# AleoNet/snarkVM

Measured on AMD Instinct MI355X. Metric: BLS12-377 G1 MSM scalar-point pairs/sec (+ Fr NTT elements/sec in ntt_*), higher is better.
Workload: dtype u32 limbs (29-bit radix) modular integer arithmetic, Fq 377-bit / Fr 253-bit; 1 GPU; G1 Pippenger MSM 2^24 (BASELINE.json configs[1]), bases (i+1)G registered in HBM, uniform scalars in HBM; independent instance per GPU; scalars=uniform, lg_ntt=24, window_bits=auto, base_tables=12, table_bits=22, pipelined_batch=True

## Files before the change

### include/snarkvm_hip.h

```cpp
#ifndef SNARKVM_HIP_H
#define SNARKVM_HIP_H

#include <stddef.h>
#include <stdint.h>

#ifdef __cplusplus
extern "C" {
#endif

typedef struct {
    int32_t code;
    char *message;
} RustError;

enum NTTInputOutputOrder { NN = 0, NR = 1, RN = 2, RR = 3 };
enum NTTDirection { Forward = 0, Inverse = 1 };
enum NTTType { Standard = 0, Coset = 1 };


RustError snarkvm_ntt(void *inout, uint32_t lg_domain_size, enum NTTInputOutputOrder ntt_order,
                      enum NTTDirection ntt_direction, enum NTTType ntt_type);

RustError snarkvm_polymul(void *out, size_t pcount, const void *polynomials, const void *plens, size_t ecount,
                          const void *evaluations, const void *elens, uint32_t lg_domain_size);

RustError snarkvm_msm(void *out, const void *points_with_infinity, size_t npoints, const void *scalars,
                      size_t ffi_affine_sz);
RustError snarkvm_hip_set_base_cache(int tables);
RustError snarkvm_hip_set_base_cache_verified(int tables);
void snarkvm_hip_base_cache_stats(uint64_t *out, int reset);


int snarkvm_hip_device_count(void);
int snarkvm_hip_batch_lanes(size_t npoints);
RustError snarkvm_hip_set_devices(const int32_t *ids, size_t n);
RustError snarkvm_hip_set_device(int device);
int snarkvm_hip_num_devices(void);

RustError snarkvm_hip_malloc(void **d_ptr, size_t bytes, int device);
RustError snarkvm_hip_free(void *d_ptr);
RustError snarkvm_hip_memcpy_h2d(void *d_dst, const void *src, size_t bytes);
RustError snarkvm_hip_memcpy_d2h(void *dst, const void *d_src, size_t bytes);
RustError snarkvm_hip_memcpy_d2d(void *d_dst, const void *d_src, size_t bytes);
RustError snarkvm_hip_memset(void *d_dst, int value, size_t bytes);

RustError snarkvm_hip_ntt_device(void *d_inout, uint32_t lg_domain_size, int ntt_order, int ntt_direction,
                                 int ntt_type);
RustError snarkvm_hip_ntt_device_batch(void *const *d_inouts, size_t count, uint32_t lg_domain_size, int ntt_order,
                                       const int *ntt_directions, const int *ntt_types);

RustError snarkvm_hip_scope_begin(const void *d_any);
RustError snarkvm_hip_scope_end(void);
enum { SNARKVM_HIP_SCOPE_ASYNC_MSM = 1, SNARKVM_HIP_SCOPE_STABLE_INPUTS = 2, SNARKVM_HIP_SCOPE_MSM_IN_STREAM = 4 };
RustError snarkvm_hip_scope_begin_ex(const void *d_any, uint32_t flags);
RustError snarkvm_hip_scope_collect(const void *out);
RustError snarkvm_hip_scope_set_flags(uint32_t flags);
void *snarkvm_hip_scope_stream(void);

typedef struct snarkvm_hip_bases snarkvm_hip_bases_t;
RustError snarkvm_hip_register_bases(snarkvm_hip_bases_t **handle, const void *points, size_t npoints,
                                     size_t ffi_affine_sz, int on_device);
RustError snarkvm_hip_register_bases_tables(snarkvm_hip_bases_t **handle, const void *points, size_t npoints,
                                            size_t ffi_affine_sz, int on_device, int tables);
RustError snarkvm_hip_register_bases_windowed(snarkvm_hip_bases_t **handle, const void *points, size_t npoints,
                                              size_t ffi_affine_sz, int on_device, int tables, int window_bits);
void snarkvm_hip_free_bases(snarkvm_hip_bases_t *handle);

RustError snarkvm_hip_register_bases_serialized(snarkvm_hip_bases_t **handle, const void *bytes, size_t npoints,
                                                int compressed, int validate, int tables);
RustError snarkvm_hip_g1_deserialize(void *out_affine, const void *bytes, size_t n, int compressed, int validate);
RustError snarkvm_hip_g1_serialize(void *out_bytes, const void *affine, size_t n, size_t ffi_affine_sz, int compressed);

RustError snarkvm_hip_g2_deserialize(void *out_affine, const void *bytes, size_t n, int validate);
RustError snarkvm_hip_g2_serialize(void *out_bytes, const void *affine, size_t n, size_t ffi_affine_sz);
RustError snarkvm_hip_g2_deserialize_compressed(void *out_affine, const void *bytes, size_t n, int validate);
RustError snarkvm_hip_g2_serialize_compressed(void *out_bytes, const void *affine, size_t n, size_t ffi_affine_sz);

RustError snarkvm_hip_msm_registered(void *out, const snarkvm_hip_bases_t *handle, size_t offset, size_t npoints,
                                     const void *scalars, int scalars_on_device, int window_bits);

RustError snarkvm_hip_msm_registered_ex(void *out, const snarkvm_hip_bases_t *handle, size_t off0, size_t n0,
                                        size_t off1, size_t n1, const void *scalars, int scalars_on_device,
                                        int scalars_montgomery, int window_bits);

RustError snarkvm_hip_msm_registered_batch(void *outs, const snarkvm_hip_bases_t *handle, size_t count,
                                           const size_t *offsets, const size_t *npoints, const void *const *scalars,
                                           int scalars_on_device, int scalars_montgomery, int window_bits);

RustError snarkvm_hip_msm_registered_batch_ex(void *outs, const snarkvm_hip_bases_t *handle, size_t count, const size_t *off0,
                                              const size_t *n0, const size_t *off1, const size_t *n1,
                                              const void *const *scalars, int scalars_on_device, int scalars_montgomery,
                                              int window_bits);

RustError snarkvm_hip_g1_sum(void *out, const void *in_projective, size_t n);

RustError snarkvm_hip_g1_to_affine(void *out_affine, const void *in_projective, size_t n);

RustError snarkvm_hip_msm_g2(void *out, const void *points_with_infinity, size_t npoints, const void *scalars,
                             size_t ffi_affine_sz);

typedef struct snarkvm_hip_bases_g2 snarkvm_hip_bases_g2_t;
RustError snarkvm_hip_register_bases_g2(snarkvm_hip_bases_g2_t **handle, const void *points, size_t npoints,
                                        size_t ffi_affine_sz, int tables, int window_bits);
void snarkvm_hip_free_bases_g2(snarkvm_hip_bases_g2_t *handle);
RustError snarkvm_hip_msm_g2_registered(void *out, const snarkvm_hip_bases_g2_t *handle, size_t offset, size_t npoints,
                                        const void *scalars, int scalars_on_device, int window_bits);
RustError snarkvm_hip_msm_g2_registered_batch(void *outs, const snarkvm_hip_bases_g2_t *handle, size_t count,
                                              const size_t *offsets, const size_t *npoints, const void *const *scalars,
                                              int scalars_on_device, int window_bits);

RustError snarkvm_hip_g1_fixed_base_msm(void *out_projective, const void *g_affine, const void *scalars, size_t n);
RustError snarkvm_hip_g1_group_ntt(void *inout_projective, uint32_t lg_domain_size, int inverse);

RustError snarkvm_hip_fr_mul_device(void *d_out, const void *d_a, const void *d_b, size_t n);
RustError snarkvm_hip_fr_convert_device(void *d_out, const void *d_in, size_t n, int to_bigint);

RustError snarkvm_hip_fr_vec_op(int op, void *out, const void *a, const void *b, const void *c, const void *scalar,
                                size_t n, int on_device);
RustError snarkvm_hip_fr_divide_by_linear(void *quotient, void *remainder, const void *poly, size_t n,
                                          const void *point, int on_device);
RustError snarkvm_hip_fr_batch_inversion_and_mul(void *inout, size_t n, const void *coeff, int on_device);
RustError snarkvm_hip_fr_distribute_powers(void *inout, size_t n, const void *g, const void *c, int on_device);
RustError snarkvm_hip_fr_lagrange_coefficients(void *out, uint32_t lg_domain_size, const void *tau, int on_device);
RustError snarkvm_hip_fr_divide_by_vanishing(void *quotient, void *remainder, const void *poly, size_t len,
                                             size_t domain_size, int on_device);
RustError snarkvm_hip_fr_mul_by_vanishing(void *out, const void *poly, size_t len, size_t domain_size, int on_device);

RustError snarkvm_hip_fr_vec_op_strided(int op, void *out, const void *a, const void *b, const void *c, const void *scalar,
                                        size_t n, size_t count, size_t stride);
RustError snarkvm_hip_fr_divide_by_linear_strided(void *quotients, void *remainders, const void *polys, size_t n,
                                                  const void *point, size_t count, size_t stride);
RustError snarkvm_hip_fr_divide_by_vanishing_strided(void *quotients, void *remainders, const void *polys, size_t len,
                                                     size_t domain_size, size_t count, size_t stride);

RustError snarkvm_hip_g1_generate_bases_device(void *d_out, uint64_t start, size_t npoints);

void snarkvm_hip_set_profiling(int enabled);
int snarkvm_hip_get_phase_count(void);
const char *snarkvm_hip_get_phase_name(int i);
double snarkvm_hip_get_phase_ms(int i);

void snarkvm_hip_coalescer_stats(uint64_t *out, int reset);

void snarkvm_hip_alloc_stats(uint64_t *out, int reset);

RustError snarkvm_hip_synchronize(void);


int snarkvm_hip_selftest_field(int field, int op, const void *a, const void *b, void *out, size_t n);
int snarkvm_hip_selftest_g1_msm_naive(const void *points_with_infinity, size_t npoints, size_t ffi_affine_sz,
                                      const void *scalars, void *out);
int snarkvm_hip_selftest_msm_plan(size_t n, int window_bits, int tables, int table_bits, uint32_t *out);
int snarkvm_hip_selftest_g1_finish(const void *planes_projective, const int32_t *pos, size_t n, void *out);
int snarkvm_hip_selftest_fq_lazy(uint64_t seed, int iters);
int snarkvm_hip_selftest_g1_lazy_tail(uint64_t seed, int iters);
int snarkvm_hip_selftest_fq2_pair(const void *points, size_t npoints, uint64_t seed, int iters);
int snarkvm_hip_selftest_g2_hex(const void *points, size_t npoints, uint64_t seed, int iters);
RustError snarkvm_hip_devtest_g2_tail_repeat(const void *points, size_t npoints, int m, int hb, int threads, int plane_threads,
                                             int hex, int quads, int iters, uint32_t *report);
int snarkvm_hip_selftest_ntt_plan(uint32_t lg, int32_t *out);
int snarkvm_hip_selftest_ntt_twiddle(int kind, uint32_t lg, int pass, int inverse, const uint64_t *x, size_t n, void *out);
int snarkvm_hip_selftest_ntt_index(uint32_t lg, const int32_t *plan, int npass);
int snarkvm_hip_selftest_ntt_host(void *inout, uint32_t lg, const int32_t *plan, int npass, int dir, int type);
RustError snarkvm_hip_devtest_field(int field, int op, const void *a, const void *b, void *out, size_t n);

#ifdef __cplusplus
}
#endif
#endif
```

### rust/snarkvm-algorithms-hip/src/sys.rs

```rust
#![allow(non_camel_case_types, non_snake_case, clippy::too_many_arguments, clippy::missing_safety_doc)]
use super::{Error, NTTDirection, NTTInputOutputOrder, NTTType};
use core::ffi::{c_char, c_void};

#[repr(C)]
pub struct snarkvm_hip_bases_t {
    _private: [u8; 0],
}
#[repr(C)]
pub struct snarkvm_hip_bases_g2_t {
    _private: [u8; 0],
}

pub const SNARKVM_HIP_SCOPE_ASYNC_MSM: u32 = 1;
pub const SNARKVM_HIP_SCOPE_STABLE_INPUTS: u32 = 2;
pub const SNARKVM_HIP_SCOPE_MSM_IN_STREAM: u32 = 4;

extern "C" {
    pub fn snarkvm_ntt(inout: *mut c_void, lg_domain_size: u32, ntt_order: NTTInputOutputOrder, ntt_direction: NTTDirection, ntt_type: NTTType) -> Error;
    pub fn snarkvm_polymul(out: *mut c_void, pcount: usize, polynomials: *const c_void, plens: *const c_void, ecount: usize, evaluations: *const c_void, elens: *const c_void, lg_domain_size: u32) -> Error;
    pub fn snarkvm_msm(out: *mut c_void, points_with_infinity: *const c_void, npoints: usize, scalars: *const c_void, ffi_affine_sz: usize) -> Error;
    pub fn snarkvm_hip_set_base_cache(tables: i32) -> Error;
    pub fn snarkvm_hip_set_base_cache_verified(tables: i32) -> Error;
    pub fn snarkvm_hip_base_cache_stats(out: *mut u64, reset: i32);
    pub fn snarkvm_hip_device_count() -> i32;
    pub fn snarkvm_hip_batch_lanes(npoints: usize) -> i32;
    pub fn snarkvm_hip_set_devices(ids: *const i32, n: usize) -> Error;
    pub fn snarkvm_hip_set_device(device: i32) -> Error;
    pub fn snarkvm_hip_num_devices() -> i32;
    pub fn snarkvm_hip_malloc(d_ptr: *mut *mut c_void, bytes: usize, device: i32) -> Error;
    pub fn snarkvm_hip_free(d_ptr: *mut c_void) -> Error;
    pub fn snarkvm_hip_memcpy_h2d(d_dst: *mut c_void, src: *const c_void, bytes: usize) -> Error;
    pub fn snarkvm_hip_memcpy_d2h(dst: *mut c_void, d_src: *const c_void, bytes: usize) -> Error;
    pub fn snarkvm_hip_memcpy_d2d(d_dst: *mut c_void, d_src: *const c_void, bytes: usize) -> Error;
    pub fn snarkvm_hip_memset(d_dst: *mut c_void, value: i32, bytes: usize) -> Error;
    pub fn snarkvm_hip_ntt_device(d_inout: *mut c_void, lg_domain_size: u32, ntt_order: i32, ntt_direction: i32, ntt_type: i32) -> Error;
    pub fn snarkvm_hip_ntt_device_batch(d_inouts: *const *mut c_void, count: usize, lg_domain_size: u32, ntt_order: i32, ntt_directions: *const i32, ntt_types: *const i32) -> Error;
    pub fn snarkvm_hip_scope_begin(d_any: *const c_void) -> Error;
    pub fn snarkvm_hip_scope_end() -> Error;
    pub fn snarkvm_hip_scope_begin_ex(d_any: *const c_void, flags: u32) -> Error;
    pub fn snarkvm_hip_scope_collect(out: *const c_void) -> Error;
    pub fn snarkvm_hip_scope_set_flags(flags: u32) -> Error;
    pub fn snarkvm_hip_scope_stream() -> *mut c_void;
    pub fn snarkvm_hip_register_bases(handle: *mut *mut snarkvm_hip_bases_t, points: *const c_void, npoints: usize, ffi_affine_sz: usize, on_device: i32) -> Error;
    pub fn snarkvm_hip_register_bases_tables(handle: *mut *mut snarkvm_hip_bases_t, points: *const c_void, npoints: usize, ffi_affine_sz: usize, on_device: i32, tables: i32) -> Error;
    pub fn snarkvm_hip_register_bases_windowed(handle: *mut *mut snarkvm_hip_bases_t, points: *const c_void, npoints: usize, ffi_affine_sz: usize, on_device: i32, tables: i32, window_bits: i32) -> Error;
    pub fn snarkvm_hip_free_bases(handle: *mut snarkvm_hip_bases_t);
    pub fn snarkvm_hip_register_bases_serialized(handle: *mut *mut snarkvm_hip_bases_t, bytes: *const c_void, npoints: usize, compressed: i32, validate: i32, tables: i32) -> Error;
    pub fn snarkvm_hip_g1_deserialize(out_affine: *mut c_void, bytes: *const c_void, n: usize, compressed: i32, validate: i32) -> Error;
    pub fn snarkvm_hip_g1_serialize(out_bytes: *mut c_void, affine: *const c_void, n: usize, ffi_affine_sz: usize, compressed: i32) -> Error;
    pub fn snarkvm_hip_g2_deserialize(out_affine: *mut c_void, bytes: *const c_void, n: usize, validate: i32) -> Error;
    pub fn snarkvm_hip_g2_serialize(out_bytes: *mut c_void, affine: *const c_void, n: usize, ffi_affine_sz: usize) -> Error;
    pub fn snarkvm_hip_g2_deserialize_compressed(out_affine: *mut c_void, bytes: *const c_void, n: usize, validate: i32) -> Error;
    pub fn snarkvm_hip_g2_serialize_compressed(out_bytes: *mut c_void, affine: *const c_void, n: usize, ffi_affine_sz: usize) -> Error;
    pub fn snarkvm_hip_msm_registered(out: *mut c_void, handle: *const snarkvm_hip_bases_t, offset: usize, npoints: usize, scalars: *const c_void, scalars_on_device: i32, window_bits: i32) -> Error;
    pub fn snarkvm_hip_msm_registered_ex(out: *mut c_void, handle: *const snarkvm_hip_bases_t, off0: usize, n0: usize, off1: usize, n1: usize, scalars: *const c_void, scalars_on_device: i32, scalars_montgomery: i32, window_bits: i32) -> Error;
    pub fn snarkvm_hip_msm_registered_batch(outs: *mut c_void, handle: *const snarkvm_hip_bases_t, count: usize, offsets: *const usize, npoints: *const usize, scalars: *const *const c_void, scalars_on_device: i32, scalars_montgomery: i32, window_bits: i32) -> Error;
    pub fn snarkvm_hip_msm_registered_batch_ex(outs: *mut c_void, handle: *const snarkvm_hip_bases_t, count: usize, off0: *const usize, n0: *const usize, off1: *const usize, n1: *const usize, scalars: *const *const c_void, scalars_on_device: i32, scalars_montgomery: i32, window_bits: i32) -> Error;
    pub fn snarkvm_hip_g1_sum(out: *mut c_void, in_projective: *const c_void, n: usize) -> Error;
    pub fn snarkvm_hip_g1_to_affine(out_affine: *mut c_void, in_projective: *const c_void, n: usize) -> Error;
    pub fn snarkvm_hip_msm_g2(out: *mut c_void, points_with_infinity: *const c_void, npoints: usize, scalars: *const c_void, ffi_affine_sz: usize) -> Error;
    pub fn snarkvm_hip_register_bases_g2(handle: *mut *mut snarkvm_hip_bases_g2_t, points: *const c_void, npoints: usize, ffi_affine_sz: usize, tables: i32, window_bits: i32) -> Error;
    pub fn snarkvm_hip_free_bases_g2(handle: *mut snarkvm_hip_bases_g2_t);
    pub fn snarkvm_hip_msm_g2_registered(out: *mut c_void, handle: *const snarkvm_hip_bases_g2_t, offset: usize, npoints: usize, scalars: *const c_void, scalars_on_device: i32, window_bits: i32) -> Error;
    pub fn snarkvm_hip_msm_g2_registered_batch(outs: *mut c_void, handle: *const snarkvm_hip_bases_g2_t, count: usize, offsets: *const usize, npoints: *const usize, scalars: *const *const c_void, scalars_on_device: i32, window_bits: i32) -> Error;
    pub fn snarkvm_hip_g1_fixed_base_msm(out_projective: *mut c_void, g_affine: *const c_void, scalars: *const c_void, n: usize) -> Error;
    pub fn snarkvm_hip_g1_group_ntt(inout_projective: *mut c_void, lg_domain_size: u32, inverse: i32) -> Error;
    pub fn snarkvm_hip_fr_mul_device(d_out: *mut c_void, d_a: *const c_void, d_b: *const c_void, n: usize) -> Error;
    pub fn snarkvm_hip_fr_convert_device(d_out: *mut c_void, d_in: *const c_void, n: usize, to_bigint: i32) -> Error;
    pub fn snarkvm_hip_fr_vec_op(op: i32, out: *mut c_void, a: *const c_void, b: *const c_void, c: *const c_void, scalar: *const c_void, n: usize, on_device: i32) -> Error;
    pub fn snarkvm_hip_fr_divide_by_linear(quotient: *mut c_void, remainder: *mut c_void, poly: *const c_void, n: usize, point: *const c_void, on_device: i32) -> Error;
    pub fn snarkvm_hip_fr_batch_inversion_and_mul(inout: *mut c_void, n: usize, coeff: *const c_void, on_device: i32) -> Error;
    pub fn snarkvm_hip_fr_distribute_powers(inout: *mut c_void, n: usize, g: *const c_void, c: *const c_void, on_device: i32) -> Error;
    pub fn snarkvm_hip_fr_lagrange_coefficients(out: *mut c_void, lg_domain_size: u32, tau: *const c_void, on_device: i32) -> Error;
    pub fn snarkvm_hip_fr_divide_by_vanishing(quotient: *mut c_void, remainder: *mut c_void, poly: *const c_void, len: usize, domain_size: usize, on_device: i32) -> Error;
    pub fn snarkvm_hip_fr_mul_by_vanishing(out: *mut c_void, poly: *const c_void, len: usize, domain_size: usize, on_device: i32) -> Error;
    pub fn snarkvm_hip_fr_vec_op_strided(op: i32, out: *mut c_void, a: *const c_void, b: *const c_void, c: *const c_void, scalar: *const c_void, n: usize, count: usize, stride: usize) -> Error;
    pub fn snarkvm_hip_fr_divide_by_linear_strided(quotients: *mut c_void, remainders: *mut c_void, polys: *const c_void, n: usize, point: *const c_void, count: usize, stride: usize) -> Error;
    pub fn snarkvm_hip_fr_divide_by_vanishing_strided(quotients: *mut c_void, remainders: *mut c_void, polys: *const c_void, len: usize, domain_size: usize, count: usize, stride: usize) -> Error;
    pub fn snarkvm_hip_g1_generate_bases_device(d_out: *mut c_void, start: u64, npoints: usize) -> Error;
    pub fn snarkvm_hip_set_profiling(enabled: i32);
    pub fn snarkvm_hip_get_phase_count() -> i32;
    pub fn snarkvm_hip_get_phase_name(i: i32) -> *const c_char;
    pub fn snarkvm_hip_get_phase_ms(i: i32) -> f64;
    pub fn snarkvm_hip_coalescer_stats(out: *mut u64, reset: i32);
    pub fn snarkvm_hip_alloc_stats(out: *mut u64, reset: i32);
    pub fn snarkvm_hip_synchronize() -> Error;
    pub fn snarkvm_hip_selftest_field(field: i32, op: i32, a: *const c_void, b: *const c_void, out: *mut c_void, n: usize) -> i32;
    pub fn snarkvm_hip_selftest_g1_msm_naive(points_with_infinity: *const c_void, npoints: usize, ffi_affine_sz: usize, scalars: *const c_void, out: *mut c_void) -> i32;
    pub fn snarkvm_hip_selftest_msm_plan(n: usize, window_bits: i32, tables: i32, table_bits: i32, out: *mut u32) -> i32;
    pub fn snarkvm_hip_selftest_g1_finish(planes_projective: *const c_void, pos: *const i32, n: usize, out: *mut c_void) -> i32;
    pub fn snarkvm_hip_selftest_fq_lazy(seed: u64, iters: i32) -> i32;
    pub fn snarkvm_hip_selftest_g1_lazy_tail(seed: u64, iters: i32) -> i32;
    pub fn snarkvm_hip_selftest_fq2_pair(points: *const c_void, npoints: usize, seed: u64, iters: i32) -> i32;
    pub fn snarkvm_hip_selftest_g2_hex(points: *const c_void, npoints: usize, seed: u64, iters: i32) -> i32;
    pub fn snarkvm_hip_devtest_g2_tail_repeat(points: *const c_void, npoints: usize, m: i32, hb: i32, threads: i32, plane_threads: i32, hex: i32, quads: i32, iters: i32, report: *mut u32) -> Error;
    pub fn snarkvm_hip_selftest_ntt_plan(lg: u32, out: *mut i32) -> i32;
    pub fn snarkvm_hip_selftest_ntt_twiddle(kind: i32, lg: u32, pass: i32, inverse: i32, x: *const u64, n: usize, out: *mut c_void) -> i32;
    pub fn snarkvm_hip_selftest_ntt_index(lg: u32, plan: *const i32, npass: i32) -> i32;
    pub fn snarkvm_hip_selftest_ntt_host(inout: *mut c_void, lg: u32, plan: *const i32, npass: i32, dir: i32, type_: i32) -> i32;
    pub fn snarkvm_hip_devtest_field(field: i32, op: i32, a: *const c_void, b: *const c_void, out: *mut c_void, n: usize) -> Error;
}
```

### snarkvm_amd/_lib.py

```python
import ctypes
import os

_HERE = os.path.dirname(os.path.abspath(__file__))
LIB_PATH = os.environ.get("SNARKVM_HIP_LIB") or os.path.join(_HERE, "lib", "libsnarkvm_hip.so")

SYMBOLS = [
    "snarkvm_ntt", "snarkvm_polymul", "snarkvm_msm", "snarkvm_hip_set_base_cache", "snarkvm_hip_set_base_cache_verified", "snarkvm_hip_base_cache_stats",
    "snarkvm_hip_device_count", "snarkvm_hip_batch_lanes", "snarkvm_hip_set_device", "snarkvm_hip_set_devices", "snarkvm_hip_num_devices",
    "snarkvm_hip_malloc", "snarkvm_hip_free", "snarkvm_hip_memcpy_h2d", "snarkvm_hip_memcpy_d2h", "snarkvm_hip_memcpy_d2d", "snarkvm_hip_memset", "snarkvm_hip_ntt_device", "snarkvm_hip_ntt_device_batch",
    "snarkvm_hip_scope_begin", "snarkvm_hip_scope_end", "snarkvm_hip_scope_begin_ex", "snarkvm_hip_scope_collect", "snarkvm_hip_scope_set_flags", "snarkvm_hip_scope_stream", "snarkvm_hip_alloc_stats",
    "snarkvm_hip_register_bases", "snarkvm_hip_register_bases_tables", "snarkvm_hip_register_bases_windowed", "snarkvm_hip_free_bases", "snarkvm_hip_msm_registered", "snarkvm_hip_msm_g2",
    "snarkvm_hip_msm_registered_ex", "snarkvm_hip_msm_registered_batch", "snarkvm_hip_msm_registered_batch_ex", "snarkvm_hip_g1_to_affine",
    "snarkvm_hip_fr_mul_device", "snarkvm_hip_fr_convert_device", "snarkvm_hip_g1_generate_bases_device",
    "snarkvm_hip_fr_vec_op", "snarkvm_hip_fr_divide_by_linear", "snarkvm_hip_fr_batch_inversion_and_mul",
    "snarkvm_hip_fr_distribute_powers", "snarkvm_hip_fr_lagrange_coefficients", "snarkvm_hip_fr_divide_by_vanishing",
    "snarkvm_hip_fr_mul_by_vanishing",
    "snarkvm_hip_fr_vec_op_strided", "snarkvm_hip_fr_divide_by_linear_strided", "snarkvm_hip_fr_divide_by_vanishing_strided",
    "snarkvm_hip_register_bases_serialized", "snarkvm_hip_g1_deserialize", "snarkvm_hip_g1_serialize", "snarkvm_hip_g1_sum", "snarkvm_hip_g2_deserialize", "snarkvm_hip_g2_serialize", "snarkvm_hip_g2_deserialize_compressed", "snarkvm_hip_g2_serialize_compressed",
    "snarkvm_hip_register_bases_g2", "snarkvm_hip_free_bases_g2", "snarkvm_hip_msm_g2_registered", "snarkvm_hip_msm_g2_registered_batch",
    "snarkvm_hip_g1_fixed_base_msm", "snarkvm_hip_g1_group_ntt",
    "snarkvm_hip_set_profiling", "snarkvm_hip_get_phase_count", "snarkvm_hip_get_phase_name",
    "snarkvm_hip_get_phase_ms", "snarkvm_hip_synchronize", "snarkvm_hip_coalescer_stats",
    "snarkvm_hip_selftest_field", "snarkvm_hip_selftest_g1_msm_naive", "snarkvm_hip_selftest_msm_plan", "snarkvm_hip_selftest_g1_finish", "snarkvm_hip_selftest_fq_lazy", "snarkvm_hip_selftest_g1_lazy_tail", "snarkvm_hip_selftest_ntt_plan", "snarkvm_hip_selftest_ntt_twiddle", "snarkvm_hip_selftest_ntt_index", "snarkvm_hip_selftest_ntt_host", "snarkvm_hip_selftest_fq2_pair", "snarkvm_hip_selftest_g2_hex", "snarkvm_hip_devtest_field", "snarkvm_hip_devtest_g2_tail_repeat",
]


class RustError(ctypes.Structure):
    _fields_ = [("code", ctypes.c_int32), ("message", ctypes.c_void_p)]


class HipError(RuntimeError):
    def __init__(self, code, message):
        super().__init__(f"snarkvm_hip error {code}: {message}")
        self.code = code
        self.message = message


_lib = None
_libc = None


def lib():
    global _lib, _libc
    if _lib is None:
        if not os.path.exists(LIB_PATH):
            raise ImportError(
                f"{LIB_PATH} is missing - build it with `python -m snarkvm_amd.build` (hipcc, gfx950). "
                "snarkvm_amd has no CPU fallback.")
        if not os.environ.get("SNARKVM_HIP_NO_TORCH"):
            try:
                import torch
            except ImportError:
                pass
        L = ctypes.CDLL(LIB_PATH)
        err_fns = ["snarkvm_ntt", "snarkvm_polymul", "snarkvm_msm", "snarkvm_hip_set_base_cache", "snarkvm_hip_set_base_cache_verified", "snarkvm_hip_set_device", "snarkvm_hip_set_devices",
                   "snarkvm_hip_malloc", "snarkvm_hip_free", "snarkvm_hip_memcpy_h2d", "snarkvm_hip_memcpy_d2h", "snarkvm_hip_memcpy_d2d", "snarkvm_hip_memset", "snarkvm_hip_ntt_device", "snarkvm_hip_ntt_device_batch",
                   "snarkvm_hip_scope_begin", "snarkvm_hip_scope_end", "snarkvm_hip_scope_begin_ex", "snarkvm_hip_scope_collect", "snarkvm_hip_scope_set_flags",
                   "snarkvm_hip_register_bases", "snarkvm_hip_register_bases_tables", "snarkvm_hip_register_bases_windowed", "snarkvm_hip_msm_registered", "snarkvm_hip_msm_g2", "snarkvm_hip_msm_registered_ex", "snarkvm_hip_msm_registered_batch", "snarkvm_hip_msm_registered_batch_ex", "snarkvm_hip_g1_to_affine", "snarkvm_hip_fr_mul_device",
                   "snarkvm_hip_fr_convert_device", "snarkvm_hip_g1_generate_bases_device", "snarkvm_hip_synchronize",
                   "snarkvm_hip_fr_vec_op", "snarkvm_hip_fr_divide_by_linear", "snarkvm_hip_fr_batch_inversion_and_mul", "snarkvm_hip_fr_distribute_powers", "snarkvm_hip_fr_lagrange_coefficients", "snarkvm_hip_fr_divide_by_vanishing", "snarkvm_hip_fr_mul_by_vanishing",
                   "snarkvm_hip_fr_vec_op_strided", "snarkvm_hip_fr_divide_by_linear_strided", "snarkvm_hip_fr_divide_by_vanishing_strided",
                   "snarkvm_hip_register_bases_serialized", "snarkvm_hip_g1_deserialize", "snarkvm_hip_g1_serialize", "snarkvm_hip_g1_sum", "snarkvm_hip_g2_deserialize", "snarkvm_hip_g2_serialize", "snarkvm_hip_g2_deserialize_compressed", "snarkvm_hip_g2_serialize_compressed",
                   "snarkvm_hip_register_bases_g2", "snarkvm_hip_msm_g2_registered", "snarkvm_hip_msm_g2_registered_batch",
                   "snarkvm_hip_g1_fixed_base_msm", "snarkvm_hip_g1_group_ntt",
                   "snarkvm_hip_devtest_field", "snarkvm_hip_devtest_g2_tail_repeat"]
        for name in err_fns:
            getattr(L, name).restype = RustError
        L.snarkvm_hip_device_count.restype = ctypes.c_int
        L.snarkvm_hip_batch_lanes.restype = ctypes.c_int
        L.snarkvm_hip_num_devices.restype = ctypes.c_int
        L.snarkvm_hip_selftest_g1_finish.restype = ctypes.c_int
        L.snarkvm_hip_selftest_fq_lazy.restype = ctypes.c_int
        L.snarkvm_hip_selftest_g1_lazy_tail.restype = ctypes.c_int
        for name in ("snarkvm_hip_selftest_ntt_plan", "snarkvm_hip_selftest_ntt_twiddle", "snarkvm_hip_selftest_ntt_index", "snarkvm_hip_selftest_ntt_host"):
            getattr(L, name).restype = ctypes.c_int
        L.snarkvm_hip_selftest_fq2_pair.restype = ctypes.c_int
        L.snarkvm_hip_selftest_g2_hex.restype = ctypes.c_int
        L.snarkvm_hip_get_phase_count.restype = ctypes.c_int
        L.snarkvm_hip_get_phase_name.restype = ctypes.c_char_p
        L.snarkvm_hip_get_phase_ms.restype = ctypes.c_double
        L.snarkvm_hip_selftest_field.restype = ctypes.c_int
        L.snarkvm_hip_selftest_g1_msm_naive.restype = ctypes.c_int
        L.snarkvm_hip_selftest_msm_plan.restype = ctypes.c_int
        L.snarkvm_hip_free_bases.restype = None
        L.snarkvm_hip_free_bases_g2.restype = None
        L.snarkvm_hip_set_profiling.restype = None
        L.snarkvm_hip_coalescer_stats.restype = None
        L.snarkvm_hip_base_cache_stats.restype = None
        L.snarkvm_hip_alloc_stats.restype = None
        L.snarkvm_hip_scope_stream.restype = ctypes.c_void_p
        L.snarkvm_hip_scope_begin_ex.argtypes = [ctypes.c_void_p, ctypes.c_uint32]
        L.snarkvm_hip_scope_set_flags.argtypes = [ctypes.c_uint32]
        L.snarkvm_hip_alloc_stats.argtypes = [ctypes.c_void_p, ctypes.c_int]
        L.snarkvm_hip_coalescer_stats.argtypes = [ctypes.c_void_p, ctypes.c_int]
        L.snarkvm_hip_base_cache_stats.argtypes = [ctypes.c_void_p, ctypes.c_int]
        L.snarkvm_hip_malloc.argtypes = [ctypes.POINTER(ctypes.c_void_p), ctypes.c_size_t, ctypes.c_int]
        L.snarkvm_hip_free.argtypes = [ctypes.c_void_p]
        L.snarkvm_hip_memcpy_h2d.argtypes = [ctypes.c_void_p, ctypes.c_void_p, ctypes.c_size_t]
        L.snarkvm_hip_memcpy_d2h.argtypes = [ctypes.c_void_p, ctypes.c_void_p, ctypes.c_size_t]
        L.snarkvm_hip_memcpy_d2d.argtypes = [ctypes.c_void_p, ctypes.c_void_p, ctypes.c_size_t]
        L.snarkvm_hip_memset.argtypes = [ctypes.c_void_p, ctypes.c_int, ctypes.c_size_t]
        _libc = ctypes.CDLL(None)
        _libc.free.argtypes = [ctypes.c_void_p]
        _lib = L
    return _lib


def check(err):
    if err.code != 0:
        msg = ctypes.string_at(err.message).decode(errors="replace") if err.message else ""
        if err.message:
            _libc.free(err.message)
        raise HipError(err.code, msg)


def device_count():
    return lib().snarkvm_hip_device_count()
```

### snarkvm_amd/csrc/api.hip

```cpp
#define SV_TU_G1
#include "runtime.hip.h"
#include "ffl.hip.h"

runtime_t g_rt;
thread_local thread_scope_t g_tl_scope;
thread_scope_t::~thread_scope_t() {
    if (!lane) return;
    pending.clear();
    (void)hipStreamSynchronize(lane->stream);
    for (int i = 0; i < naux; i++) {
        (void)hipStreamSynchronize(aux[i]->stream);
        aux[i]->dev->give(aux[i], true);
    }
    lane->in_scope = false;
    lane->deferred.clear();
    lane->deferred_bytes = 0;
    if (!lane->tw_leases.empty()) ntt_tw_release(lane->dev, lane->tw_leases);
    lane->dev->give(lane, true);
    lane = nullptr;
}
std::atomic<uint64_t> g_co_stats[4];
static std::atomic<uint64_t> g_alloc_stats[5];
void sv_alloc_note(int slot, size_t bytes, double ms) {
    g_alloc_stats[slot].fetch_add(1, std::memory_order_relaxed);
// ... 131 lines not shown
    if (!bytes) return ok();
    API_BEGIN_DEV(device_for(d_src, 1))
    if (!dst || !d_src) throw hip_failure{hipErrorInvalidValue, "snarkvm_hip_memcpy_d2h: null pointer", __LINE__};
    HIP_TRY(hipMemcpyAsync(dst, d_src, bytes, hipMemcpyDeviceToHost, c.stream));
    HIP_TRY(hipStreamSynchronize(c.stream));
    API_END
}
RustError snarkvm_hip_memcpy_d2d(void* d_dst, const void* d_src, size_t bytes) {
    if (!bytes) return ok();
    API_BEGIN_DEV(device_for(d_dst, 1))
    if (!d_dst || !d_src) throw hip_failure{hipErrorInvalidValue, "snarkvm_hip_memcpy_d2d: null pointer", __LINE__};
    const uint8_t *a = (const uint8_t*)d_dst, *b = (const uint8_t*)d_src;
    if (a < b + bytes && b < a + bytes) throw hip_failure{hipErrorInvalidValue, "snarkvm_hip_memcpy_d2d: the ranges overlap", __LINE__};
    if (g_rt.device_of(d_src) < 0) throw hip_failure{hipErrorInvalidValue, "snarkvm_hip_memcpy_d2d: source is not on a device in use", __LINE__};
    HIP_TRY(hipMemcpyAsync(d_dst, d_src, bytes, hipMemcpyDefault, c.stream));
    c.sync_or_defer();
    API_END
}
RustError snarkvm_hip_memset(void* d_dst, int value, size_t bytes) {
    if (!bytes) return ok();
    API_BEGIN_DEV(device_for(d_dst, 1))
    HIP_TRY(hipMemsetAsync(d_dst, value, bytes, c.stream));
    c.sync_or_defer();
    API_END
}

static constexpr uint32_t SCOPE_FLAGS_ALL = SNARKVM_HIP_SCOPE_ASYNC_MSM | SNARKVM_HIP_SCOPE_STABLE_INPUTS | SNARKVM_HIP_SCOPE_MSM_IN_STREAM;
RustError snarkvm_hip_scope_begin_ex(const void* d_any, uint32_t flags) {
    API_TRY
    thread_scope_t& sc = tl_scope();
    if (sc.lane) throw hip_failure{hipErrorInvalidValue, "scope_begin: the calling thread already has an open scope", __LINE__};
    if (flags & ~SCOPE_FLAGS_ALL) throw hip_failure{hipErrorInvalidValue, "scope_begin: unknown flag", __LINE__};
    g_rt.configure();
    const int nd = (int)g_rt.devs.size();
    int dev = device_for(d_any, d_any ? 1 : 0);
    if (dev < 0) dev = (int)(g_rt.rr.fetch_add(1) % (uint32_t)nd);
    device_t* d = g_rt.devs[dev].get();
    int prev = -1;
    if (hipGetDevice(&prev) != hipSuccess) prev = 0;
    lane_t* l = d->take_for_scope(true);
    try {
        HIP_TRY(hipSetDevice(d->physical));
        d->init();
        tu_kernel_attributes(d->logical);
    } catch (...) {
        d->give(l, true);
        (void)hipSetDevice(prev);
        throw;
    }
    l->begin_call();
    l->in_scope = true;
    l->pin_used = 0;
    l->scope_events_used = 0;
    sc = thread_scope_t();
    sc.lane = l;
    sc.prev_device = prev;
    sc.flags = flags;
    API_CATCH
}
RustError snarkvm_hip_scope_begin(const void* d_any) { return snarkvm_hip_scope_begin_ex(d_any, 0); }
void* snarkvm_hip_scope_stream(void) {
    lane_t* l = tl_scope().lane;
    return l ? (void*)l->stream : nullptr;
}
RustError snarkvm_hip_scope_set_flags(uint32_t flags) {
    API_TRY
    thread_scope_t& sc = tl_scope();
    if (!sc.lane) throw hip_failure{hipErrorInvalidValue, "scope_set_flags: the calling thread has no open scope", __LINE__};
    if (flags & ~SCOPE_FLAGS_ALL) throw hip_failure{hipErrorInvalidValue, "scope_set_flags: unknown flag", __LINE__};
    sc.flags = flags;
    API_CATCH
}
RustError snarkvm_hip_scope_collect(const void* out) {
    API_TRY
    scope_collect(out);
    API_CATCH
}
RustError snarkvm_hip_scope_end(void) {
    thread_scope_t& sc = tl_scope();
    lane_t* l = sc.lane;
    if (!l) return ok();
    RustError r = ok();
    try {
        scope_flush();
    } catch (const hip_failure& f) {
        r = from_failure(f);
    } catch (const std::exception& e) {
        r = fail(1, std::string("snarkvm_hip: scope_end: ") + e.what());
    } catch (...) {
        r = fail(1, "snarkvm_hip: scope_end failed");
    }
    l->in_scope = false;
    l->deferred.clear();
    l->deferred_bytes = 0;
    for (int i = 0; i < sc.naux; i++) {
        (void)hipStreamSynchronize(sc.aux[i]->stream);
        sc.aux[i]->dev->give(sc.aux[i], true);
    }
    const int prev = sc.prev_device;
    sc = thread_scope_t();
    l->dev->give(l, true);
    if (prev >= 0) (void)hipSetDevice(prev);
    return r;
}

static void precompute_tables(lane_t& c, snarkvm_hip_bases* h, g1_aff_mem_t* d) { precompute_tables_run<fq_t>(c, d, h->n, h->tables, h->table_bits); }
static void register_bases_impl(snarkvm_hip_bases_t** handle, const void* points, size_t npoints, size_t ffi_affine_sz, int on_device, int tables,
                                int table_bits) {
    if (!handle) throw hip_failure{hipErrorInvalidValue, "register_bases: null handle", __LINE__};
    if (npoints && !points) throw hip_failure{hipErrorInvalidValue, "register_bases: null points", __LINE__};
    if (ffi_affine_sz < 104 || (ffi_affine_sz & 7)) throw hip_failure{hipErrorInvalidValue, "register_bases: bad stride", __LINE__};
    check_tables(tables, table_bits, "register_bases");
    scope_flush();
    const int nd = g_rt.ndev();
    std::unique_ptr<snarkvm_hip_bases> h(new snarkvm_hip_bases());
    h->n = npoints;
    h->tables = tables;
    h->table_bits = table_bits ? table_bits : 256 / tables;
    h->d.assign(nd, nullptr);
    const size_t bytes = (size_t)tables * npoints * sizeof(g1_aff_mem_t);
    try {
        if (npoints) {
            const int owner = on_device ? device_for(points, 1) : -1;
            auto build = [&](int dev) {
                lane_guard lg(dev);
                lane_t& c = lg.c();
                HIP_TRY(hipMalloc((void**)&h->d[dev], bytes));
                const uint8_t* src = (const uint8_t*)points;
                if (!on_device) {
                    c.bases_tmp.ensure(npoints * ffi_affine_sz);
                    HIP_TRY(hipMemcpyAsync(c.bases_tmp.p, points, npoints * ffi_affine_sz, hipMemcpyHostToDevice, c.stream));
                    src = c.bases_tmp.as<uint8_t>();
                }
                convert_bases<fq_t>(c, src, ffi_affine_sz, npoints, h->d[dev]);
                precompute_tables(c, h.get(), h->d[dev]);
                bases_to_lazy_form(c, h->d[dev], (size_t)tables * npoints);
                HIP_TRY(hipStreamSynchronize(c.stream));
            };
            std::vector<int> all;
            for (int d = 0; d < nd; d++) all.push_back(d);
            if (!on_device) {
                for_each_device(all, build);
            } else {
                build(owner);
                for (int d = 0; d < nd; d++) {
                    if (d == owner) continue;
                    lane_guard lg(d);
                    HIP_TRY(hipMalloc((void**)&h->d[d], bytes));
                    HIP_TRY(hipMemcpyPeerAsync(h->d[d], g_rt.devs[d]->physical, h->d[owner], g_rt.devs[owner]->physical, bytes, lg.c().stream));
                    HIP_TRY(hipStreamSynchronize(lg.c().stream));
                }
            }
        }
    } catch (...) {
        h->free_all();
        throw;
    }
    *handle = h.release();
}
RustError snarkvm_hip_register_bases(snarkvm_hip_bases_t** handle, const void* points, size_t npoints, size_t ffi_affine_sz, int on_device) {
    API_TRY
    register_bases_impl(handle, points, npoints, ffi_affine_sz, on_device, 1, 0);
    API_CATCH
}
RustError snarkvm_hip_register_bases_tables(snarkvm_hip_bases_t** handle, const void* points, size_t npoints, size_t ffi_affine_sz, int on_device,
                                            int tables) {
    API_TRY
    register_bases_impl(handle, points, npoints, ffi_affine_sz, on_device, tables, 0);
    API_CATCH
}
RustError snarkvm_hip_register_bases_windowed(snarkvm_hip_bases_t** handle, const void* points, size_t npoints, size_t ffi_affine_sz, int on_device,
                                              int tables, int window_bits) {
    API_TRY
    if (window_bits <= 0) throw hip_failure{hipErrorInvalidValue, "register_bases_windowed: window_bits must be positive", __LINE__};
    register_bases_impl(handle, points, npoints, ffi_affine_sz, on_device, tables, window_bits);
    API_CATCH
}
void snarkvm_hip_free_bases(snarkvm_hip_bases_t* h) {
    if (!h) return;
    h->free_all();
    delete h;
}
}
snarkvm_hip_bases* sv_new_bases_handle(size_t npoints, int tables, int table_bits) {
    snarkvm_hip_bases* h = new snarkvm_hip_bases();
    h->n = npoints;
    h->tables = tables;
    h->table_bits = table_bits;
    h->d.assign(g_rt.ndev(), nullptr);
    return h;
}
void sv_precompute_tables(lane_t& c, snarkvm_hip_bases* h, g1_aff_mem_t* d) { precompute_tables(c, h, d); }
extern "C" {

static void check_window_bits(int window_bits, const char* who) {
    if (window_bits && (window_bits < 2 || window_bits > MSM_C_MAX)) throw std::runtime_error(std::string(who) + ": window_bits must be 0 or 2..23");
}
static void msm_registered_host_scalars(void* out, const snarkvm_hip_bases* h, size_t off0, size_t n0, size_t off1, size_t n1, const void* scalars,
                                        int scalars_montgomery, int window_bits) {
    const size_t n = n0 + n1;
    scope_flush();
    const int nd = g_rt.ndev();
    static const int trace = getenv("SNARKVM_HIP_TRACE") ? atoi(getenv("SNARKVM_HIP_TRACE")) : 0;
    const double t_begin = host_now_ms();
    size_t parts = n / MSM_SPLIT_MIN;
    if (parts > (size_t)nd) parts = (size_t)nd;
    if (parts < 1) parts = 1;
    const size_t chunk = msm_scalar_chunk_pairs();
    if (n >= 2 * chunk && (n + chunk - 1) / chunk > parts) parts = (n + chunk - 1) / chunk;
    std::vector<size_t> bound;
    const int geo = tuning().scalar_geo;
    if (nd == 1 && geo > 1 && tuning().taper != 0 && n >= ((size_t)1 << 22)) {
        parts = n >= ((size_t)1 << 23) ? 3 : 2;
        size_t wsum = 0, w = 1;
        for (size_t i = 0; i < parts; i++, w *= (size_t)geo) wsum += w;
        size_t acc_w = 0;
        w = 1;
        bound.push_back(0);
        for (size_t i = 0; i < parts; i++, w *= (size_t)geo) {
            acc_w += w;
            bound.push_back(i + 1 == parts ? n : (size_t)((unsigned __int128)n * acc_w / wsum));
        }
    } else {
        for (size_t i = 0; i <= parts; i++) bound.push_back(n * i / parts);
    }
    const int ndu = (int)(parts < (size_t)nd ? parts : (size_t)nd);
    std::unique_ptr<msm_accum_t<fq_t>> acc(new msm_accum_t<fq_t>());
    std::mutex acc_mu;
    std::vector<int> devs;
    if (ndu == 1) {
        devs.push_back(-1);
    } else {
        for (int d = 0; d < ndu; d++) devs.push_back(d);
    }
    const size_t slot = msm_plane_bytes<fq_t>();
    for_each_device(devs, [&](int dev) {
        std::vector<size_t> mine;
        for (size_t i = (dev < 0 ? 0 : (size_t)dev); i < parts; i += (size_t)ndu) mine.push_back(i);
        lane_guard lg;
        lg.acquire(dev, mine.size() > 2 ? 3 : (int)mine.size());
        const size_t L = lg.lanes.size();
        size_t max_cnt = 0;
        for (size_t j = 0; j < mine.size(); j++) {
            const size_t cnt = bound[mine[j] + 1] - bound[mine[j]];
            max_cnt = cnt > max_cnt ? cnt : max_cnt;
        }
        const bool use_sink = tuning().taper != 0 && mine.size() >= 2;
        std::vector<msm_pending_t> pend(use_sink ? 1 : mine.size());
        int chunk_c = window_bits;
        msm_bucket_sink_t sink;
        std::vector<hipEvent_t> merged;
        for (size_t l = 0; l < L; l++) {
            lane_t& c = *lg.lanes[l];
            c.begin_call();
            c.scalars_tmp.ensure(max_cnt * 32 + 32);
            c.pin.ensure(slot * (use_sink ? 1 : (mine.size() + L - 1) / L));
        }
        if (use_sink) {
            lane_t& c0 = *lg.lanes[0];
            const msm_plan_t pl = msm_make_plan(max_cnt, window_bits, h->tables, h->table_bits);
            chunk_c = pl.c;
            sink.nbt = (uint32_t)pl.W * pl.nb;
            sink.L = 1;
            const size_t bytes = (size_t)sink.nbt * msm_partial_bytes<fq_t>();
            c0.sink_acc.ensure(bytes);
            sink.acc = c0.sink_acc.p;
            HIP_TRY(hipMemsetAsync(sink.acc, 0, bytes, c0.stream));
            hipEvent_t ready = c0.new_event();
            HIP_TRY(hipEventRecord(ready, c0.stream));
            for (size_t l = 1; l < L; l++) HIP_TRY(hipStreamWaitEvent(lg.lanes[l]->stream, ready, 0));
            for (size_t j = 0; j < mine.size(); j++) merged.push_back(lg.lanes[j % L]->new_event());
        }
        const g1_aff_mem_t* base = h->d[lg.lanes[0]->dev->logical];
        auto upload = [&](size_t j, hipStream_t st) {
            lane_t& c = *lg.lanes[j % L];
            const size_t lo = bound[mine[j]], hi = bound[mine[j] + 1];
            if (hi > lo) HIP_TRY(hipMemcpyAsync(c.scalars_tmp.p, (const uint8_t*)scalars + lo * 32, (hi - lo) * 32, hipMemcpyHostToDevice, st));
        };
        auto compute = [&](size_t j, bool prof) {
            lane_t& c = *lg.lanes[j % L];
            const size_t lo = bound[mine[j]], hi = bound[mine[j] + 1];
            const size_t a0 = lo < n0 ? lo : n0, a1 = hi < n0 ? hi : n0;
            const size_t m0 = a1 - a0;
            const g1_aff_mem_t* b0 = base + off0 + a0;
            const g1_aff_mem_t* b1 = base + off1 + (lo > n0 ? lo - n0 : 0);
            msm_bucket_sink_t mine_sink = sink;
            if (use_sink) {
                mine_sink.after = j ? merged[j - 1] : nullptr;
                mine_sink.done = merged[j];
            }
            const msm_pending_t pd = msm_run<fq_t>(c, m0 ? b0 : b1, c.scalars_tmp.as<uint4>(), hi - lo, c.pin.as<uint8_t>() + (use_sink ? 0 : slot * (j / L)), chunk_c,
                                                   b1, m0 ? m0 : ~(size_t)0, scalars_montgomery, h->tables, h->n, prof, h->table_bits, nullptr,
                                                   use_sink ? &mine_sink : nullptr);
            if (!use_sink) pend[j] = pd;
        };
        if (mine.size() == 1) {
            lane_t& c = *lg.lanes[0];
            c.phase_begin("msm_h2d");
            upload(0, c.stream);
            c.phase_end();
            compute(0, parts == 1);
        } else {
            lane_ring_run(lg, mine.size(), upload, [&](size_t j) { compute(j, false); }, trace, t_begin);
        }
        if (use_sink) {
            lane_t& c0 = *lg.lanes[0];
// ... 556 lines not shown
            g1_xyzz_t t2 = total;
            t2.add(acc);
            t2.add(neg);
            t2.add(acc);
            total = t2;
        } else {
            total.add(acc);
        }
    }
    const g1_jac_t j = total.to_jacobian();
    uint32_t* o = (uint32_t*)out;
    j.x.to_mem_mont().pack(o);
    j.y.to_mem_mont().pack(o + 12);
    j.z.to_mem_mont().pack(o + 24);
    return 0;
}
int snarkvm_hip_selftest_fq_lazy(uint64_t seed, int iters) {
    uint32_t xw[12], yw[12];
    memcpy(xw, G1_GEN_X, 48);
    memcpy(yw, G1_GEN_Y, 48);
    const g1_aff_t g{fq_t::unpack(xw).from_mem_mont(), fq_t::unpack(yw).from_mem_mont()};
    std::vector<g1_aff_t> pool;
    g1_xyzz_t run = g1_xyzz_t::inf();
    for (int k = 0; k < 64; k++) {
        run.add_affine(g);
        const fq_t izzz = run.zzz.inverse();
        const fq_t izz = izzz.sqr() * run.zz.sqr();
        pool.push_back({run.x * izz, run.y * izzz});
    }
    const fq_t c406 = fq_t::from_table(FqLConv::C406), c348 = fq_t::from_table(FqLConv::C348);
    auto next = [&]() {
        seed += 0x9E3779B97F4A7C15ull;
        uint64_t z = seed;
        z = (z ^ (z >> 30)) * 0xBF58476D1CE4E5B9ull;
        z = (z ^ (z >> 27)) * 0x94D049BB133111EBull;
        return z ^ (z >> 31);
    };
    g1_xyzz_t exact = g1_xyzz_t::inf();
    xyzz_lazy_t lazy = xyzz_lazy_t::infinity();
    int prev = -1;
    bool prev_neg = false;
    for (int it = 0; it < iters; it++) {
        const uint64_t r = next();
        int k = (int)(r % 64);
        bool neg = ((r >> 8) & 1) != 0;
        const int mode = (int)((r >> 16) % 16);
        if (mode == 0 && prev >= 0) k = prev, neg = prev_neg;
        if (mode == 1 && prev >= 0) k = prev, neg = !prev_neg;
        if (mode == 2) {
            exact = g1_xyzz_t::inf();
            lazy = xyzz_lazy_t::infinity();
        }
        prev = k;
        prev_neg = neg;
        const g1_aff_t p = pool[k];
        exact.add_affine(p, neg);
        const fql_t px = fql_t::from_limbs(p.x * c406), py = fql_t::from_limbs(p.y * c406);
        if (!lazy.madd(px, py, neg)) {
            g1_xyzz_t e = lazy.to_exact();
            fq_t ex, ey;
            for (int i = 0; i < 13; i++) ex.v[i] = (uint32_t)px.v[i], ey.v[i] = (uint32_t)py.v[i];
            e.add_affine({ex * c348, ey * c348}, neg);
            lazy = xyzz_lazy_t::from_exact(e);
        }
        const g1_xyzz_t got = lazy.to_exact();
        if (got.is_inf() != exact.is_inf()) return it + 1;
        if (!exact.is_inf() && (got.x != exact.x || got.y != exact.y || got.zz != exact.zz || got.zzz != exact.zzz)) return it + 1;
    }
    for (int t = 0; t < 200; t++) {
        fq_t a, b;
        for (int i = 0; i < 13; i++) a.v[i] = (uint32_t)(next() & LIMB_MASK), b.v[i] = (uint32_t)(next() & LIMB_MASK);
        a.v[12] &= 0x00ffffffu;
        b.v[12] &= 0x00ffffffu;
        if (t & 1) for (int i = 0; i < 12; i++) a.v[i] = LIMB_MASK;
        if (t & 2) for (int i = 0; i < 12; i++) b.v[i] = (i & 1) ? LIMB_MASK : 0;
        const fql_t la = fql_t::from_exact(a), lb = fql_t::from_exact(b);
        if (fql_t::mul(la, lb).to_exact() != a * b) return -(4 * t + 1);
        if (fql_t::sqr(la - lb).to_exact() != (a - b).sqr()) return -(4 * t + 2);
        if (fql_t::diff_of_products(la - lb, lb - la, fql_t::from_exact(a * b).normalized(), la).to_exact() != fq_t::diff_of_products(a - b, b - a, a * b, a))
            return -(4 * t + 3);
        if (((la + lb) - (lb + lb)).normalized().to_exact() != (a - b)) return -(4 * t + 4);
        alignas(16) uint32_t raw[12];
        const fql_t wide = (la - lb - lb - lb).normalized();
        wide.store_raw(raw);
        const fql_t back = fql_t::load_raw(raw);
        for (int i = 0; i < 13; i++)
            if (back.v[i] != wide.v[i]) return -(100000 + t);
    }
    return 0;
}
int snarkvm_hip_selftest_g1_lazy_tail(uint64_t seed, int iters) {
    uint32_t xw[12], yw[12];
    memcpy(xw, G1_GEN_X, 48);
    memcpy(yw, G1_GEN_Y, 48);
    const g1_aff_t g{fq_t::unpack(xw).from_mem_mont(), fq_t::unpack(yw).from_mem_mont()};
    std::vector<g1_xyzz_t> pool;
    g1_xyzz_t run = g1_xyzz_t::inf();
    for (int k = 0; k < 48; k++) {
        run.add_affine(g);
        pool.push_back(run);
    }
    auto next = [&]() {
        seed += 0x9E3779B97F4A7C15ull;
        uint64_t z = seed;
        z = (z ^ (z >> 30)) * 0xBF58476D1CE4E5B9ull;
        z = (z ^ (z >> 27)) * 0x94D049BB133111EBull;
        return z ^ (z >> 31);
    };
    auto to_lazy = [](const g1_xyzz_t& p) {
        xyzz_t<fqz_t> r = xyzz_t<fqz_t>::inf();
        if (!p.is_inf()) r = {{fql_t::from_exact(p.x)}, {fql_t::from_exact(p.y)}, {fql_t::from_exact(p.zz)}, {fql_t::from_exact(p.zzz)}};
        return r;
    };
    g1_xyzz_t exact = g1_xyzz_t::inf();
    xyzz_t<fqz_t> lazy = xyzz_t<fqz_t>::inf();
    g1_xyzz_t prev = g1_xyzz_t::inf();
    for (int it = 0; it < iters; it++) {
        const uint64_t r = next();
        g1_xyzz_t p = pool[r % 48];
        fq_t l = fq_t::zero();
        for (int i = 0; i < 12; i++) l.v[i] = (uint32_t)(next() & LIMB_MASK);
        l.v[0] |= 1;
        const fq_t l2 = l.sqr(), l3 = l2 * l;
        p = {p.x * l2, p.y * l3, p.zz * l2, p.zzz * l3};
        if ((r >> 8) & 1) p.y = p.y.neg();
        const int mode = (int)((r >> 16) % 16);
        if (mode == 0) p = prev;
        if (mode == 1) p = {prev.x, prev.y.neg(), prev.zz, prev.zzz};
        if (mode == 2) {
            exact = g1_xyzz_t::inf();
            lazy = xyzz_t<fqz_t>::inf();
        }
        if (mode == 3) p = exact;
        if (mode == 4) {
            exact = exact.dbl();
            lazy = lazy.dbl();
        } else {
            prev = p;
            exact.add(p);
            lazy.add(to_lazy(p));
        }
        if (lazy.is_inf() != exact.is_inf()) return it + 1;
        if (!exact.is_inf() && (lazy.x.to_exact() != exact.x || lazy.y.to_exact() != exact.y || lazy.zz.to_exact() != exact.zz || lazy.zzz.to_exact() != exact.zzz))
            return it + 1;
        xyzz_mem_t<fqz_t> m;
        store_xyzz<fqz_t>(&m, lazy);
        lazy = load_xyzz<fqz_t>(&m);
    }
    fqz_t zq;
    for (int i = 0; i < 13; i++) zq.a.v[i] = FqL::MOD[i];
    if (!zq.is_zero() || !zq.neg().is_zero() || !(zq + zq).is_zero() || (zq + fqz_t::one()).is_zero()) return -1;
    return 0;
}
int snarkvm_hip_selftest_g1_finish(const void* planes_jacobian, const int32_t* pos, size_t n, void* out) {
    try {
        std::unique_ptr<msm_accum_t<fq_t>> acc(new msm_accum_t<fq_t>());
        const uint32_t* src = (const uint32_t*)planes_jacobian;
        for (size_t i = 0; i < n; i++) {
            const g1_jac_t j = {fq_t::from_raw_words(src + 36 * i), fq_t::from_raw_words(src + 36 * i + 12), fq_t::from_raw_words(src + 36 * i + 24)};
            acc->add(pos[i], g1_xyzz_t::from_jacobian(j));
        }
        acc->finish(out);
        return 0;
    } catch (...) {
        return 1;
    }
}

}
```

### snarkvm_amd/csrc/api_serde.hip

```cpp
#include "runtime.hip.h"

snarkvm_hip_bases* sv_new_bases_handle(size_t npoints, int tables, int table_bits);
void sv_precompute_tables(lane_t& c, snarkvm_hip_bases* h, g1_aff_mem_t* d);

static uint32_t g1_deserialize_run(lane_t& c, const void* bytes, size_t n, int compressed, int validate, g1_aff_mem_t* d_native, uint8_t* d_rust) {
    const size_t psz = compressed ? 48 : 96;
    c.bases_tmp.ensure(n * psz);
    c.serde_status.ensure(4);
    HIP_TRY(hipMemcpyAsync(c.bases_tmp.p, bytes, n * psz, hipMemcpyHostToDevice, c.stream));
    HIP_TRY(hipMemsetAsync(c.serde_status.p, 0, 4, c.stream));
    hipLaunchKernelGGL(g1_deserialize_kernel, dim3((unsigned)((n + 63) / 64)), dim3(64), 0, c.stream, c.bases_tmp.as<uint8_t>(), n, compressed, validate,
                       d_native, d_rust, c.serde_status.as<uint32_t>());
    HIP_TRY(hipGetLastError());
    uint32_t st = 0;
    HIP_TRY(hipMemcpyAsync(&st, c.serde_status.p, 4, hipMemcpyDeviceToHost, c.stream));
    HIP_TRY(hipStreamSynchronize(c.stream));
    return st;
}

extern "C" {

RustError snarkvm_hip_register_bases_serialized(snarkvm_hip_bases_t** handle, const void* bytes, size_t npoints, int compressed, int validate,
                                                int tables) {
    API_TRY
    if (!handle || (npoints && !bytes)) throw hip_failure{hipErrorInvalidValue, "register_bases_serialized: null argument", __LINE__};
    check_tables(tables, 0, "register_bases_serialized");
    std::unique_ptr<snarkvm_hip_bases> h(sv_new_bases_handle(npoints, tables, 256 / tables));
    if (npoints) {
        try {
            std::vector<int> all;
            for (int d = 0; d < g_rt.ndev(); d++) all.push_back(d);
            for_each_device(all, [&](int dev) {
                lane_guard lg(dev);
                lane_t& c = lg.c();
                HIP_TRY(hipMalloc((void**)&h->d[dev], (size_t)tables * npoints * sizeof(g1_aff_mem_t)));
                serde_throw_on_status(g1_deserialize_run(c, bytes, npoints, compressed, validate, h->d[dev], nullptr), "register_bases_serialized");
                sv_precompute_tables(c, h.get(), h->d[dev]);
                bases_to_lazy_form(c, h->d[dev], (size_t)tables * npoints);
                HIP_TRY(hipStreamSynchronize(c.stream));
            });
        } catch (...) {
            h->free_all();
            throw;
        }
    }
    *handle = h.release();
    API_CATCH
}
RustError snarkvm_hip_g1_deserialize(void* out_affine, const void* bytes, size_t n, int compressed, int validate) {
    API_BEGIN
    if (n) {
        if (!out_affine || !bytes) throw hip_failure{hipErrorInvalidValue, "g1_deserialize: null argument", __LINE__};
        c.poly[0].ensure(n * 104);
        const uint32_t st = g1_deserialize_run(c, bytes, n, compressed, validate, nullptr, c.poly[0].as<uint8_t>());
        serde_throw_on_status(st, "g1_deserialize");
        HIP_TRY(hipMemcpyAsync(out_affine, c.poly[0].p, n * 104, hipMemcpyDeviceToHost, c.stream));
        HIP_TRY(hipStreamSynchronize(c.stream));
    }
    API_END
}
RustError snarkvm_hip_g1_serialize(void* out_bytes, const void* affine, size_t n, size_t ffi_affine_sz, int compressed) {
    API_BEGIN
    if (n) {
        if (!out_bytes || !affine) throw hip_failure{hipErrorInvalidValue, "g1_serialize: null argument", __LINE__};
        if (ffi_affine_sz < 104 || (ffi_affine_sz & 7)) throw hip_failure{hipErrorInvalidValue, "g1_serialize: bad stride", __LINE__};
        const size_t psz = compressed ? 48 : 96;
        c.bases_tmp.ensure(n * ffi_affine_sz);
        c.poly[0].ensure(n * psz);
        HIP_TRY(hipMemcpyAsync(c.bases_tmp.p, affine, n * ffi_affine_sz, hipMemcpyHostToDevice, c.stream));
        hipLaunchKernelGGL(g1_serialize_kernel, dim3((unsigned)((n + 63) / 64)), dim3(64), 0, c.stream, c.bases_tmp.as<uint8_t>(), ffi_affine_sz, n,
                           compressed, c.poly[0].as<uint8_t>());
        HIP_TRY(hipGetLastError());
        HIP_TRY(hipMemcpyAsync(out_bytes, c.poly[0].p, n * psz, hipMemcpyDeviceToHost, c.stream));
        HIP_TRY(hipStreamSynchronize(c.stream));
    }
    API_END
}

}
```

### snarkvm_amd/csrc/ffl.hip.h

```cpp
#pragma once
#include "ec.hip.h"

namespace sv {

struct FqL {
    static constexpr int N = 13;
    static constexpr int STEPS = 14;
    static constexpr int32_t MOD[13] = {0x00000001, 0x08460000, 0x00000021, 0x16ba8860, 0x14800170, 0x1117dd04, 0x0e3c7bcd,
                                        0x1e601ea2, 0x1b1a22d9, 0x03650a49, 0x118ec170, 0x0f8a21d5, 0x1ae3a461};
    static constexpr int32_t K377[13] = {0x1fffffff, 0x17b9ffff, 0x1fffffde, 0x0945779f, 0x0b7ffe8f, 0x0ee822fb, 0x11c38432,
                                         0x019fe15d, 0x04e5dd26, 0x1c9af5b6, 0x0e713e8f, 0x1075de2a, 0x051c5b9e};
    static constexpr int32_t K435[13] = {0x0677f3e3, 0x01fcf72f, 0x05fc93a0, 0x08eb59fe, 0x0c1a6c3f, 0x122b8005, 0x01c7de9b,
                                         0x0b159718, 0x189a8339, 0x07649107, 0x02e4fa41, 0x13571fee, 0x04eba458};
};
struct FqLConv {
    static constexpr uint32_t C406[13] = {0x19eaf730u, 0x171ffffeu, 0x0d714cf8u, 0x044e31d8u, 0x1eb6e262u, 0x0bfad163u, 0x00d46e9cu,
                                          0x10b6ddbfu, 0x13b9cbddu, 0x075782afu, 0x03bd1d8au, 0x1557cab6u, 0x15742a14u};
    static constexpr uint32_t C399[13] = {0x1fb3d5efu, 0x1759ffffu, 0x161ae2aeu, 0x06bd319fu, 0x15cd6eabu, 0x15c6dfc5u, 0x00a7763du,
                                          0x1e5d80e1u, 0x10d7c95fu, 0x04add573u, 0x1c80b321u, 0x02e104bau, 0x10f92f11u};
    static constexpr uint32_t C348[13] = {0, 0, 0, 0, 0, 0, 0, 0, 0, 0, 0, 0, 1};
};

#if defined(__HIP_DEVICE_COMPILE__)
#define SV_OPAQUE_LIMB(x) asm("" : "+v"(x))
// ... 183 lines not shown
        return r;
    }

    SV_HD fq_t to_exact() const {
        fql_t k;
#pragma unroll
        for (int i = 0; i < N; i++) k.v[i] = FqL::K377[i];
        fql_t t = mul(*this, k);
#pragma unroll 1
        for (int round = 0; round < 3 && t.v[N - 1] < 0; round++) {
            int32_t c = 0;
#pragma unroll
            for (int i = 0; i < N - 1; i++) {
                const int32_t x = t.v[i] + FqL::MOD[i] + c;
                t.v[i] = (int32_t)((uint32_t)x & MASK);
                c = x >> 29;
            }
            t.v[N - 1] += FqL::MOD[N - 1] + c;
        }
        uint32_t w[N];
#pragma unroll
        for (int i = 0; i < N; i++) w[i] = (uint32_t)t.v[i];
        return fq_t::cond_sub(w);
    }
    SV_HD static fql_t from_exact(const fq_t& a) {
        fql_t k;
#pragma unroll
        for (int i = 0; i < N; i++) k.v[i] = FqL::K435[i];
        return mul(from_limbs(a), k);
    }
};

struct alignas(128) g1_lazy_slot_t {
    uint32_t w[32];
    SV_HD void coords(fql_t& px, fql_t& py) const {
#pragma unroll
        for (int i = 0; i < 13; i++) px.v[i] = (int32_t)w[i], py.v[i] = (int32_t)w[13 + i];
        SV_OPAQUE_13(px.v);
        SV_OPAQUE_13(py.v);
    }
    SV_HD static void store(g1_aff_mem_t* slot, const fq_t& x406, const fq_t& y406, bool inf) {
        uint32_t* o = (uint32_t*)slot;
        uint4* q = (uint4*)slot;
        uint32_t t[28];
#pragma unroll
        for (int i = 0; i < 13; i++) t[i] = inf ? 0u : x406.v[i], t[13 + i] = inf ? 0u : y406.v[i];
        t[26] = inf ? 1u : 0u;
        t[27] = 0;
#pragma unroll
        for (int i = 0; i < 7; i++) q[i] = make_uint4(t[4 * i], t[4 * i + 1], t[4 * i + 2], t[4 * i + 3]);
        (void)o;
    }
};
static_assert(sizeof(g1_lazy_slot_t) == sizeof(g1_aff_mem_t), "a lazy base slot overlays the exact one");

struct alignas(16) g1_lazy_partial_t {
    int32_t w[52];
};
struct xyzz_lazy_t {
    fql_t x, y, zz, zzz;
    bool inf;

    SV_HD static xyzz_lazy_t infinity() {
        xyzz_lazy_t r;
        r.x = r.y = r.zz = r.zzz = fql_t::zero();
        r.inf = true;
        return r;
    }
    SV_HD g1_xyzz_t to_exact() const {
        if (inf) return g1_xyzz_t::inf();
        return {x.to_exact(), y.to_exact(), zz.to_exact(), zzz.to_exact()};
    }
    SV_HD void store_raw(g1_lazy_partial_t* p) const {
        uint4* q = (uint4*)p;
        if (inf) {
#pragma unroll
            for (int i = 0; i < 13; i++) q[i] = make_uint4(0, 0, 0, 0);
            return;
        }
        int32_t t[52];
#pragma unroll
        for (int i = 0; i < 13; i++) t[i] = x.v[i], t[13 + i] = y.v[i], t[26 + i] = zz.v[i], t[39 + i] = zzz.v[i];
#pragma unroll
        for (int i = 0; i < 13; i++) q[i] = make_uint4((uint32_t)t[4 * i], (uint32_t)t[4 * i + 1], (uint32_t)t[4 * i + 2], (uint32_t)t[4 * i + 3]);
    }
    SV_HD static g1_xyzz_t exact_from_raw(const g1_lazy_partial_t* p) {
        const uint4* q = (const uint4*)p;
        int32_t t[52];
#pragma unroll
        for (int i = 0; i < 13; i++) {
            const uint4 u = q[i];
            t[4 * i] = (int32_t)u.x, t[4 * i + 1] = (int32_t)u.y, t[4 * i + 2] = (int32_t)u.z, t[4 * i + 3] = (int32_t)u.w;
        }
        fql_t c[4];
#pragma unroll
        for (int k = 0; k < 4; k++)
#pragma unroll
            for (int i = 0; i < 13; i++) c[k].v[i] = t[13 * k + i];
        return {c[0].to_exact(), c[1].to_exact(), c[2].to_exact(), c[3].to_exact()};
    }
    SV_HD static xyzz_lazy_t from_exact(const g1_xyzz_t& p) {
        xyzz_lazy_t r;
        r.inf = p.is_inf();
        if (r.inf) return infinity();
        r.x = fql_t::from_exact(p.x);
        r.y = fql_t::from_exact(p.y);
        r.zz = fql_t::from_exact(p.zz);
        r.zzz = fql_t::from_exact(p.zzz);
        return r;
    }
    SV_HD bool madd(const fql_t& px, const fql_t& py, bool negate) {
        if (inf) {
            x = px;
            y = py.negate_if(negate).normalized();
            zz = zzz = one();
            inf = false;
            return true;
        }
        const fql_t u2 = fql_t::mul(px, zz);
        const fql_t s2 = fql_t::mul(py.negate_if(negate), zzz);
        const fql_t p = u2 - x;
        const fql_t r = s2 - y;
        if ((((uint32_t)p.v[0] + 4u) & fql_t::MASK) <= 5u) return false;
        const fql_t pp = fql_t::sqr(p);
        const fql_t ppp = fql_t::mul(p, pp);
        const fql_t q = fql_t::mul(x, pp);
        const fql_t rr = fql_t::sqr(r);
        fql_t x3;
        {
            int32_t c = 0;
#pragma unroll
            for (int i = 0; i < fql_t::N - 1; i++) {
                const int32_t t = rr.v[i] - ppp.v[i] - 2 * q.v[i] + c;
                x3.v[i] = (int32_t)((uint32_t)t & fql_t::MASK);
                c = t >> 29;
            }
            x3.v[fql_t::N - 1] = rr.v[fql_t::N - 1] - ppp.v[fql_t::N - 1] - 2 * q.v[fql_t::N - 1] + c;
            SV_OPAQUE_13(x3.v);
        }
        y = fql_t::diff_of_products(r, q - x3, y, ppp);
        x = x3;
        zz = fql_t::mul(zz, pp);
        zzz = fql_t::mul(zzz, ppp);
        return true;
    }
    SV_HD static fql_t one() {
        fql_t r;
#pragma unroll
        for (int i = 0; i < fql_t::N; i++) r.v[i] = (int32_t)FqLConv::C406[i];
        return r;
    }
};

struct fqz_t {
    fql_t a;
    struct mem_t {
        uint32_t w[13];
    };
    static constexpr int N = 13;

    SV_HD static fqz_t zero() { return {fql_t::zero()}; }
    SV_HD static fqz_t one() { return {xyzz_lazy_t::one()}; }
    SV_HD static fqz_t load(const mem_t* p) {
        fqz_t r;
#pragma unroll
        for (int i = 0; i < N; i++) r.a.v[i] = (int32_t)p->w[i];
        return r;
    }
    SV_HD void store(mem_t* p) const {
#pragma unroll
        for (int i = 0; i < N; i++) p->w[i] = (uint32_t)a.v[i];
    }
    SV_HD fqz_t operator*(const fqz_t& b) const { return {fql_t::mul(a, b.a)}; }
    SV_HD fqz_t sqr() const { return {fql_t::sqr(a)}; }
    SV_HD fqz_t operator+(const fqz_t& b) const { return {(a + b.a).normalized()}; }
    SV_HD fqz_t operator-(const fqz_t& b) const { return {(a - b.a).normalized()}; }
    SV_HD fqz_t dbl() const { return {(a + a).normalized()}; }
    SV_HD fqz_t neg() const { return {(fql_t::zero() - a).normalized()}; }
    SV_HD static fqz_t diff_of_products(const fqz_t& x, const fqz_t& y, const fqz_t& z, const fqz_t& w) {
        return {fql_t::diff_of_products(x.a, y.a, z.a, w.a)};
    }
    SV_HD fq_t to_exact() const { return a.to_exact(); }
    SV_HD bool is_zero() const {
        int32_t any = 0;
#pragma unroll
        for (int i = 0; i < N; i++) any |= a.v[i];
        if (any == 0) return true;
        if ((((uint32_t)a.v[0] + 8u) & fql_t::MASK) > 16u) return false;
        return a.to_exact().is_zero();
    }
};

}
```

### snarkvm_amd/csrc/msm.hip.h

```cpp
#pragma once
#include <stdlib.h>

#include <type_traits>

#include "ec.hip.h"
#include "ffl.hip.h"
#include "ffl2.hip.h"
#include "hex2.hip.h"
#include "tuning.hip.h"

namespace sv {

struct msm_plan_t {
    size_t n;
    int c;
    int W;
    int J;
    int Wd;
    uint32_t nb;
    uint32_t nbt;
    uint32_t chunk;
    uint32_t nchunks;
    uint32_t S, S2;
    uint32_t L;
// ... 72 lines not shown
    if (p.L > p.nb) p.L = p.nb;
    while (p.nb % p.L) p.L--;
    p.rounds = 0;
    size_t m = ((size_t)p.J * n + p.S - 1) / p.S;
    while (m > 1) {
        m = (m + p.S2 - 1) / p.S2;
        p.rounds++;
    }
    for (int i = 0; i < 10; i++) p.bias[i] = 0;
    for (int w = 0; w < p.Wd; w++) {
        int bit = p.c - 1 + p.c * w;
        if (bit >= MSM_BIAS_BITS) break;
        p.bias[bit / 32] |= 1u << (bit % 32);
    }
    return p;
}

static constexpr int SCAN_TILE = 2048;
static __global__ void scan_tile_kernel(const uint32_t* in, uint32_t* out, uint32_t* block_sums, size_t n) {
    __shared__ uint32_t sh[256];
    const size_t base = (size_t)blockIdx.x * SCAN_TILE + (size_t)threadIdx.x * 8;
    uint32_t v[8], s = 0;
#pragma unroll
    for (int i = 0; i < 8; i++) {
        v[i] = (base + i < n) ? in[base + i] : 0u;
        s += v[i];
    }
    sh[threadIdx.x] = s;
    __syncthreads();
    for (int off = 1; off < 256; off <<= 1) {
        uint32_t t = (threadIdx.x >= (unsigned)off) ? sh[threadIdx.x - off] : 0u;
        __syncthreads();
        sh[threadIdx.x] += t;
        __syncthreads();
    }
    uint32_t run = sh[threadIdx.x] - s;
#pragma unroll
    for (int i = 0; i < 8; i++) {
        if (base + i < n) out[base + i] = run;
        run += v[i];
    }
    if (threadIdx.x == 255 && block_sums) block_sums[blockIdx.x] = sh[255];
}
static __global__ void scan_add_kernel(uint32_t* out, const uint32_t* block_offsets, size_t n) {
    const size_t base = (size_t)blockIdx.x * SCAN_TILE + (size_t)threadIdx.x * 8;
    const uint32_t add = block_offsets[blockIdx.x];
#pragma unroll
    for (int i = 0; i < 8; i++)
        if (base + i < n) out[base + i] += add;
}
static inline size_t scan_tmp_elems(size_t n) {
    size_t tot = 0;
    while (n > 1) {
        n = (n + SCAN_TILE - 1) / SCAN_TILE;
        tot += n + 1;
        if (n == 1) break;
    }
    return tot + 8;
}
static constexpr uint32_t SCAN_ONE_THREADS = 1024, SCAN_ONE_MAX = 33 * SCAN_ONE_THREADS;
static __global__ void __launch_bounds__(1024) scan_one_block_kernel(const uint32_t* in, uint32_t* out, uint32_t n, uint32_t per) {
    extern __shared__ uint32_t scan_sm[];
    __shared__ uint32_t wave_tot[16];
    const uint32_t t = threadIdx.x;
    for (uint32_t i = t; i < n; i += SCAN_ONE_THREADS) scan_sm[i] = in[i];
    __syncthreads();
    const uint32_t lo = t * per, hi = lo + per < n ? lo + per : n;
    uint32_t sum = 0;
    for (uint32_t i = lo; i < hi; i++) sum += scan_sm[i];
    uint32_t incl = sum;
    for (int off = 1; off < 64; off <<= 1) {
        const uint32_t u = (uint32_t)__shfl_up((int)incl, off);
        if ((t & 63) >= (uint32_t)off) incl += u;
    }
    if ((t & 63) == 63) wave_tot[t >> 6] = incl;
    __syncthreads();
    uint32_t base = 0;
    for (uint32_t w = 0; w < (t >> 6); w++) base += wave_tot[w];
    uint32_t run = base + incl - sum;
    for (uint32_t i = lo; i < hi; i++) {
        const uint32_t v = scan_sm[i];
        scan_sm[i] = run;
        run += v;
    }
    __syncthreads();
    for (uint32_t i = t; i < n; i += SCAN_ONE_THREADS) out[i] = scan_sm[i];
}
static inline void exclusive_scan_u32(hipStream_t st, const uint32_t* in, uint32_t* out, size_t n, uint32_t* tmp) {
    if (n == 0) return;
    const int one_launch = tuning().scan1;
    if (one_launch && n > (size_t)SCAN_TILE && n <= (size_t)SCAN_ONE_MAX) {
        const uint32_t per = (uint32_t)((n + SCAN_ONE_THREADS - 1) / SCAN_ONE_THREADS) | 1u;
        hipLaunchKernelGGL(scan_one_block_kernel, dim3(1), dim3(SCAN_ONE_THREADS), (size_t)n * 4, st, in, out, (uint32_t)n, per);
        return;
    }
    const size_t blocks = (n + SCAN_TILE - 1) / SCAN_TILE;
    hipLaunchKernelGGL(scan_tile_kernel, dim3((unsigned)blocks), dim3(256), 0, st, in, out, tmp, n);
    if (blocks > 1) {
        exclusive_scan_u32(st, tmp, tmp, blocks, tmp + blocks + 1);
        hipLaunchKernelGGL(scan_add_kernel, dim3((unsigned)blocks), dim3(256), 0, st, out, tmp, n);
    }
}

template <class F>
SV_HD void store_base_slot(aff_mem_t<F>* slot, const uint32_t* xw, const uint32_t* yw, bool inf, int form406) {
    aff_t<F> a = aff_t<F>::inf();
    if (!inf) {
        a.x = F::from_raw_words(xw);
        a.y = F::from_raw_words(yw);
    }
    store_aff<F>(slot, a);
}
template <>
SV_HD void store_base_slot<fq_t>(aff_mem_t<fq_t>* slot, const uint32_t* xw, const uint32_t* yw, bool inf, int form406) {
    if (form406) {
        const fq_t c = fq_t::from_table(FqLConv::C399);
        g1_lazy_slot_t::store(slot, fq_t::unpack(xw) * c, fq_t::unpack(yw) * c, inf);
        return;
    }
    g1_aff_t a = g1_aff_t::inf();
    if (!inf) {
        a.x = fq_t::from_raw_words(xw);
        a.y = fq_t::from_raw_words(yw);
    }
    store_aff<fq_t>(slot, a);
}
template <>
SV_HD void store_base_slot<fq2_t>(aff_mem_t<fq2_t>* slot, const uint32_t* xw, const uint32_t* yw, bool inf, int form406) {
    if (form406) {
        const fq_t c = fq_t::from_table(FqLConv::C399);
        g2_lazy_slot_t::store(slot, {fq_t::unpack(xw) * c, fq_t::unpack(xw + 12) * c}, {fq_t::unpack(yw) * c, fq_t::unpack(yw + 12) * c}, inf);
        return;
    }
    aff_t<fq2_t> a = aff_t<fq2_t>::inf();
    if (!inf) {
        a.x = fq2_t::from_raw_words(xw);
        a.y = fq2_t::from_raw_words(yw);
    }
    store_aff<fq2_t>(slot, a);
}
static __global__ void g2_bases_to_form406_kernel(aff_mem_t<fq2_t>* slots, size_t n) {
    const size_t i = blockIdx.x * (size_t)blockDim.x + threadIdx.x;
    if (i >= n) return;
    const fq_t c = fq_t::from_table(FqLConv::C406);
    const aff_t<fq2_t> a = load_aff<fq2_t>(&slots[i]);
    g2_lazy_slot_t::store(&slots[i], {a.x.c0 * c, a.x.c1 * c}, {a.y.c0 * c, a.y.c1 * c}, a.is_inf());
}
static __global__ void g1_bases_to_form406_kernel(g1_aff_mem_t* slots, size_t n) {
    const size_t i = blockIdx.x * (size_t)blockDim.x + threadIdx.x;
    if (i >= n) return;
    const fq_t c = fq_t::from_table(FqLConv::C406);
    const g1_aff_t a = g1_load_aff(&slots[i]);
    g1_lazy_slot_t::store(&slots[i], a.x * c, a.y * c, a.is_inf());
}
template <class F>
__global__ void convert_bases_kernel(const uint8_t* in, size_t stride, size_t n, aff_mem_t<F>* out, int form406) {
    size_t i = blockIdx.x * (size_t)blockDim.x + threadIdx.x;
    if (i >= n) return;
    const uint32_t* src = (const uint32_t*)(in + i * stride);
    constexpr int MW = F::MEM_WORDS;
    uint32_t xw[MW], yw[MW];
#pragma unroll
    for (int k = 0; k < MW; k++) {
        xw[k] = src[k];
        yw[k] = src[MW + k];
    }
    const uint32_t inf = src[2 * MW] & 0xffu;
    store_base_slot<F>(&out[i], xw, yw, inf != 0, form406);
}

struct msm_digit_params_t {
    uint32_t bias[10];
    int c, W;
    size_t n;
    int montgomery;
};
template <class DT>
__global__ void __launch_bounds__(256) msm_digits_kernel(const uint4* __restrict__ scalars, DT* __restrict__ digits,
                                                         msm_digit_params_t p) {
    __shared__ uint4 stage[512];
    const size_t nblk = (p.n + 255) / 256;
    for (size_t blk = blockIdx.x; blk < nblk; blk += gridDim.x) {
        const size_t first = blk * 256;
        const size_t cnt = (p.n - first < 256) ? (p.n - first) : 256;
        for (int k = threadIdx.x; k < 512; k += 256)
            if ((size_t)(k >> 1) < cnt) stage[k] = scalars[first * 2 + k];
        __syncthreads();
        if (threadIdx.x < cnt) {
            const uint4 lo = stage[2 * threadIdx.x], hi = stage[2 * threadIdx.x + 1];
            uint32_t s[11] = {lo.x, lo.y, lo.z, lo.w, hi.x, hi.y, hi.z, hi.w, 0u, 0u, 0u};
            if (p.montgomery) {
                fr_t c32 = fr_t::zero();
                c32.v[0] = 32;
                (fr_t::unpack(s) * c32).pack(s);
            }
            uint64_t carry = 0;
#pragma unroll
            for (int k = 0; k < 10; k++) {
                carry += (uint64_t)s[k] + p.bias[k];
                s[k] = (uint32_t)carry;
                carry >>= 32;
            }
            const uint32_t mask = (1u << p.c) - 1;
            const size_t i = first + threadIdx.x;
            for (int w = 0; w < p.W; w++) {
                const int bit = p.c * w, wi = bit >> 5, sh = bit & 31;
                uint64_t two = (uint64_t)s[wi] | ((uint64_t)s[wi + 1] << 32);
                digits[(size_t)w * p.n + i] = (DT)((uint32_t)(two >> sh) & mask);
            }
        }
        __syncthreads();
    }
}

static __global__ void msm_alloc_kernel(const uint32_t* cnt_in, uint32_t* cnt_out, uint32_t nbt, uint32_t S) {
    uint32_t k = blockIdx.x * blockDim.x + threadIdx.x;
    if (k > nbt) return;
    cnt_out[k] = (k == nbt) ? 0u : (cnt_in[k] + S - 1) / S;
}
__device__ __forceinline__ uint32_t find_bucket(const uint32_t* start, uint32_t nbt, uint32_t t) {
    uint32_t lo = 0, hi = nbt;
    while (hi - lo > 1) {
        const uint32_t mid = (lo + hi) >> 1;
        if (start[mid] <= t)
            lo = mid;
        else
            hi = mid;
    }
    return lo;
}
template <class F>
__global__ void __launch_bounds__(256) msm_reduce_kernel(const xyzz_mem_t<F>* __restrict__ in,
                                                         const uint32_t* __restrict__ in_start,
                                                         const uint32_t* __restrict__ in_cnt,
                                                         const uint32_t* __restrict__ out_start,
                                                         xyzz_mem_t<F>* __restrict__ out, uint32_t nbt, uint32_t S2) {
    const uint32_t t = blockIdx.x * blockDim.x + threadIdx.x;
    if (t >= out_start[nbt]) return;
    const uint32_t k = find_bucket(out_start, nbt, t);
    const uint32_t j = t - out_start[k];
    const uint32_t lo = in_start[k] + j * S2;
    uint32_t hi = lo + S2;
    const uint32_t end = in_start[k] + in_cnt[k];
    if (hi > end) hi = end;
    xyzz_t<F> acc = load_xyzz<F>(&in[lo]);
    for (uint32_t pos = lo + 1; pos < hi; pos++) acc.add(load_xyzz<F>(&in[pos]));
    store_xyzz<F>(&out[t], acc);
}

template <class F>
__global__ void __launch_bounds__(256) msm_bucket_merge_kernel(const xyzz_mem_t<F>* __restrict__ part, const uint32_t* __restrict__ start,
                                                               const uint32_t* __restrict__ cnt, xyzz_mem_t<F>* __restrict__ acc, uint32_t nbt, uint32_t L,
                                                               uint32_t slot) {
    const uint32_t k = blockIdx.x * blockDim.x + threadIdx.x;
    if (k >= nbt) return;
    const uint32_t c = cnt[k];
    if (!c) return;
    const uint32_t lo = start[k];
    xyzz_mem_t<F>* dst = &acc[(size_t)k * L + slot];
    xyzz_t<F> a = load_xyzz<F>(dst);
    for (uint32_t i = 0; i < c; i++) a.add(load_xyzz<F>(&part[lo + i]));
    store_xyzz<F>(dst, a);
}
static __global__ void msm_sink_lists_kernel(uint32_t* __restrict__ start, uint32_t* __restrict__ cnt, uint32_t nbt, uint32_t L) {
    const uint32_t k = blockIdx.x * blockDim.x + threadIdx.x;
    if (k > nbt) return;
    start[k] = k * L;
    cnt[k] = k < nbt ? L : 0u;
}

__device__ __forceinline__ fq_t shfl_xor_field(const fq_t& a, int mask) {
    fq_t r;
#pragma unroll
    for (int i = 0; i < fq_t::N; i++) r.v[i] = (uint32_t)__shfl_xor((int)a.v[i], mask);
    return r;
}
__device__ __forceinline__ fq2_t shfl_xor_field(const fq2_t& a, int mask) { return {shfl_xor_field(a.c0, mask), shfl_xor_field(a.c1, mask)}; }
__device__ __forceinline__ fqz_t shfl_xor_field(const fqz_t& a, int mask) {
    fqz_t r;
#pragma unroll
    for (int i = 0; i < fqz_t::N; i++) r.a.v[i] = __shfl_xor(a.a.v[i], mask);
    SV_OPAQUE_13(r.a.v);
    return r;
}
template <class F>
__device__ __forceinline__ xyzz_t<F> shfl_xor_point(const xyzz_t<F>& a, int mask) {
    return {shfl_xor_field(a.x, mask), shfl_xor_field(a.y, mask), shfl_xor_field(a.zz, mask), shfl_xor_field(a.zzz, mask)};
}
template <int CTRL>
__device__ __forceinline__ fq_t quad_perm_field(const fq_t& a) {
    fq_t r;
#pragma unroll
    for (int i = 0; i < fq_t::N; i++) r.v[i] = (uint32_t)__builtin_amdgcn_mov_dpp((int)a.v[i], CTRL, 0xf, 0xf, true);
    return r;
}
template <int CTRL>
__device__ __forceinline__ fq2_t quad_perm_field(const fq2_t& a) {
    return {quad_perm_field<CTRL>(a.c0), quad_perm_field<CTRL>(a.c1)};
}
template <int CTRL>
__device__ __forceinline__ fqz_t quad_perm_field(const fqz_t& a) {
    fqz_t r;
#pragma unroll
    for (int i = 0; i < fqz_t::N; i++) r.a.v[i] = __builtin_amdgcn_mov_dpp(a.a.v[i], CTRL, 0xf, 0xf, true);
    SV_OPAQUE_13(r.a.v);
    return r;
// ... 510 lines not shown
```

### snarkvm_amd/csrc/msm_sort.hip.h

```cpp
#pragma once
#include "ffl.hip.h"
#include "ffl2.hip.h"
#include "ffl2p.hip.h"
#include "msm.hip.h"

namespace sv {

static constexpr int SORT_TILE = 8192;
static constexpr int SORT_THREADS = 256;

struct msm_inst_t {
    const uint4* scalars;
    uint32_t n;
    uint32_t n0;
    uint32_t off0, off1;
    uint32_t pstart;
    uint32_t ptiles;
};
struct msm_radix_params_t {
    size_t n;
    int c, W, J;
    int HB, LB;
    uint32_t nb;
    uint32_t tiles_per_row;
// ... 569 lines not shown
        }
        if (sl == 0) {
            bsize[(size_t)q * B2 + key] = total;
            if (total) atomicMax(&blk_max, total);
        }
    }
    if (q == 0 && threadIdx.x == 0) bsize[(size_t)nbins * B2] = 0;
    __syncthreads();
    if (threadIdx.x == 0 && blk_max > __atomic_load_n(max_size, __ATOMIC_RELAXED)) atomicMax(max_size, blk_max);
}
template <class RIN, class ROUT>
__global__ void __launch_bounds__(SORT_THREADS) radix_scatter2_kernel(const uint32_t* __restrict__ v1, const RIN* __restrict__ l1,
                                                                      const uint32_t* __restrict__ binstart,
                                                                      const uint32_t* __restrict__ tile2_start,
                                                                      const uint32_t* __restrict__ counts2,
                                                                      const uint32_t* __restrict__ off2, const uint32_t* __restrict__ boff,
                                                                      uint32_t* __restrict__ sorted, ROUT* __restrict__ rem_out, uint32_t nbins,
                                                                      int LB, int shift, uint32_t xcd) {
    __shared__ uint32_t lcount[128], lstart[128], cursor[128], gbase[128], wave_tot[4];
    __shared__ uint32_t sv_[SORT_TILE];
    __shared__ uint8_t slow_[SORT_TILE];
    __shared__ ROUT srem_[SORT_TILE];
    const uint32_t ntiles2 = tile2_start[nbins];
    if (blockIdx.x >= ntiles2) return;
    const uint32_t t2 = xcd ? xcd_tile(blockIdx.x, ntiles2) : blockIdx.x;
    const uint32_t B2 = 1u << LB;
    const uint32_t q = find_bucket(tile2_start, nbins, t2);
    const uint32_t lt = t2 - tile2_start[q];
    const uint32_t lo = binstart[q] + lt * SORT_TILE;
    uint32_t hi = lo + SORT_TILE;
    if (hi > binstart[q + 1]) hi = binstart[q + 1];
    {
        const uint32_t i = threadIdx.x;
        const uint32_t cnt = (i < B2) ? counts2[(size_t)t2 * B2 + i] : 0u;
        const uint32_t start = block_excl_scan(cnt, wave_tot);
        if (i < 128) {
            lcount[i] = cnt;
            gbase[i] = (i < B2) ? boff[(q << LB) | i] + off2[(size_t)t2 * B2 + i] : 0u;
            lstart[i] = start;
            cursor[i] = start;
        }
    }
    __syncthreads();
    {
        constexpr int PER = SORT_TILE / SORT_THREADS;
        uint32_t lv[PER];
        uint32_t ll[PER];
#pragma unroll
        for (int k = 0; k < PER; k++) {
            const uint32_t i = lo + threadIdx.x + (uint32_t)k * SORT_THREADS;
            const bool ok = i < hi;
            lv[k] = ok ? v1[i] : 0u;
            ll[k] = ok ? (uint32_t)l1[i] : 0xffffffffu;
        }
        const uint32_t rmask = (1u << shift) - 1;
#pragma unroll
        for (int k = 0; k < PER; k++) {
            if (ll[k] != 0xffffffffu) {
                const uint32_t key = (ll[k] >> shift) & (B2 - 1);
                const uint32_t pos = atomicAdd(&cursor[key], 1u);
                sv_[pos] = lv[k];
                slow_[pos] = (uint8_t)key;
                if (rem_out) srem_[pos] = (ROUT)(ll[k] & rmask);
            }
        }
    }
    __syncthreads();
    const uint32_t total = hi - lo;
#pragma unroll 4
    for (uint32_t pos = threadIdx.x; pos < total; pos += blockDim.x) {
        const uint32_t key = slow_[pos];
        const size_t dst = (size_t)gbase[key] + (pos - lstart[key]);
        sorted[dst] = sv_[pos];
        if (rem_out) rem_out[dst] = srem_[pos];
    }
}

static __global__ void msm_alloc_seg_kernel(const uint32_t* __restrict__ boff, uint32_t* __restrict__ cnt, uint32_t nbt, uint32_t S) {
    const uint32_t k = blockIdx.x * blockDim.x + threadIdx.x;
    if (k > nbt) return;
    uint32_t c = 0;
    if (k < nbt) {
        const uint32_t lo = boff[k], hi = boff[k + 1];
        if (hi > lo) c = (hi - 1) / S - lo / S + 1;
    }
    cnt[k] = c;
}
template <class F, int MINW, bool PREFETCH>
__global__ void __launch_bounds__(256, MINW) msm_accumulate_seg_kernel(const aff_mem_t<F>* __restrict__ bases, const uint32_t* __restrict__ sorted,
                                                                 const uint32_t* __restrict__ boff, const uint32_t* __restrict__ start,
                                                                 xyzz_mem_t<F>* __restrict__ partial, uint32_t nbt, uint32_t S, uint32_t debug_idx_mask) {
    const uint32_t t = blockIdx.x * blockDim.x + threadIdx.x;
    const uint32_t total = boff[nbt];
    const uint64_t lo64 = (uint64_t)t * S;
    if (lo64 >= total) return;
    const uint32_t lo = (uint32_t)lo64;
    const uint32_t hi = (total - lo < S) ? total : lo + S;
    uint32_t k = find_bucket(boff, nbt, lo);
    uint32_t kend = boff[k + 1];
    uint32_t kend2 = boff[k + 2 <= nbt ? k + 2 : nbt];
    uint32_t start_k = start[k];
    uint32_t part_off = t - boff[k] / S;
    xyzz_t<F> acc = xyzz_t<F>::inf();
    auto slot_of = [&](uint32_t e) -> const aff_mem_t<F>* { return &bases[(e & 0x7fffffffu) & debug_idx_mask]; };
    uint32_t e_next = sorted[lo];
    aff_mem_t<F> raw_next;
    if (PREFETCH) raw_next = *slot_of(e_next);
    for (uint32_t pos = lo; pos < hi; pos++) {
        if (pos >= kend) {
            store_xyzz<F>(&partial[start_k + part_off], acc);
            acc = xyzz_t<F>::inf();
            part_off = 0;
            k++;
            kend = kend2;
            while (pos >= kend) {
                k++;
                kend = boff[k + 1];
            }
            kend2 = boff[k + 2 <= nbt ? k + 2 : nbt];
            start_k = start[k];
        }
        const uint32_t e = e_next;
        aff_mem_t<F> raw;
        if (PREFETCH) {
            raw = raw_next;
            if (pos + 1 < hi) {
                e_next = sorted[pos + 1];
                raw_next = *slot_of(e_next);
            }
        } else {
            raw = *slot_of(e);
            if (pos + 1 < hi) e_next = sorted[pos + 1];
        }
        acc.add_affine(load_aff<F>(&raw), (e >> 31) != 0);
    }
    store_xyzz<F>(&partial[start_k + part_off], acc);
}

static __global__ void __launch_bounds__(256) g1_partials_to_exact_kernel(const g1_lazy_partial_t* __restrict__ raw, g1_xyzz_mem_t* __restrict__ partial,
                                                                   const uint32_t* __restrict__ start, uint32_t nbt) {
    const uint32_t i = blockIdx.x * blockDim.x + threadIdx.x;
    if (i >= start[nbt]) return;
    g1_store_xyzz(&partial[i], xyzz_lazy_t::exact_from_raw(&raw[i]));
}
static __device__ __noinline__ void lazy_exceptional_add(xyzz_lazy_t* acc, const fql_t* px, const fql_t* py, bool neg) {
    g1_xyzz_t ex = acc->to_exact();
    const fq_t c348 = fq_t::from_table(FqLConv::C348);
    fq_t bx, by;
#pragma unroll
    for (int i = 0; i < 13; i++) bx.v[i] = (uint32_t)px->v[i], by.v[i] = (uint32_t)py->v[i];
    ex.add_affine({bx * c348, by * c348}, neg);
    *acc = xyzz_lazy_t::from_exact(ex);
}
template <bool PREFETCH>
__global__ void __launch_bounds__(256, 1) msm_accumulate_lazy_kernel(const g1_aff_mem_t* __restrict__ bases, const uint32_t* __restrict__ sorted,
                                                              const uint32_t* __restrict__ boff, const uint32_t* __restrict__ start,
                                                              g1_lazy_partial_t* __restrict__ partial, uint32_t nbt, uint32_t S, uint32_t debug_idx_mask) {
    const uint32_t t = blockIdx.x * blockDim.x + threadIdx.x;
    const uint32_t total = boff[nbt];
    const uint64_t lo64 = (uint64_t)t * S;
    if (lo64 >= total) return;
    const uint32_t lo = (uint32_t)lo64;
    const uint32_t hi = (total - lo < S) ? total : lo + S;
    uint32_t k = find_bucket(boff, nbt, lo);
    uint32_t kend = boff[k + 1];
    uint32_t kend2 = boff[k + 2 <= nbt ? k + 2 : nbt];
    uint32_t start_k = start[k];
    uint32_t part_off = t - boff[k] / S;
    xyzz_lazy_t acc = xyzz_lazy_t::infinity();
    auto slot_of = [&](uint32_t e) -> const g1_lazy_slot_t* { return (const g1_lazy_slot_t*)&bases[(e & 0x7fffffffu) & debug_idx_mask]; };
    uint32_t e_cur = sorted[lo];
    uint32_t e_n1 = lo + 1 < hi ? sorted[lo + 1] : 0u;
    g1_lazy_slot_t raw_next = *slot_of(e_cur);
    for (uint32_t pos = lo;; pos++) {
        const bool end = pos >= hi;
        if (end || pos >= kend) {
            acc.store_raw(&partial[start_k + part_off]);
            if (end) break;
            part_off = 0;
            acc.inf = true;
            k++;
            kend = kend2;
            while (pos >= kend) {
                k++;
                kend = boff[k + 1];
            }
            kend2 = boff[k + 2 <= nbt ? k + 2 : nbt];
            start_k = start[k];
        }
        const uint32_t e = e_cur;
        const g1_lazy_slot_t raw = raw_next;
        if (pos + 1 < hi) raw_next = *slot_of(e_n1);
        e_cur = e_n1;
        if (pos + 2 < hi) e_n1 = sorted[pos + 2];
        if (raw.w[26]) continue;
        const bool neg = (e >> 31) != 0;
        fql_t px, py;
        raw.coords(px, py);
        if (!acc.madd(px, py, neg)) {
            xyzz_lazy_t tmp = acc;
            const fql_t tx = px, ty = py;
            lazy_exceptional_add(&tmp, &tx, &ty, neg);
            acc = tmp;
        }
    }
}

static __global__ void __launch_bounds__(256) g2_pair_partials_to_exact_kernel(const g2_pair_partial_t* __restrict__ raw, xyzz_mem_t<fq2_t>* __restrict__ partial,
                                                                        const uint32_t* __restrict__ start, uint32_t nbt) {
    const uint32_t g = blockIdx.x * blockDim.x + threadIdx.x;
    const uint32_t i = g >> 3, k = g & 7;
    if (i >= start[nbt]) return;
    const uint4* q = (const uint4*)&raw[i].w[16 * k];
    uint32_t t[16];
#pragma unroll
    for (int j = 0; j < 4; j++) {
        const uint4 u = q[j];
        t[4 * j] = u.x, t[4 * j + 1] = u.y, t[4 * j + 2] = u.z, t[4 * j + 3] = u.w;
    }
    fql_t c;
#pragma unroll
    for (int j = 0; j < 13; j++) c.v[j] = (int32_t)t[j];
    c.to_exact().store(&((fq_mem_t*)&partial[i])[k]);
}
template <bool PREFETCH>
__global__ void __launch_bounds__(256, 2) msm_accumulate_pair2_kernel(const aff_mem_t<fq2_t>* __restrict__ bases, const uint32_t* __restrict__ sorted,
                                                               const uint32_t* __restrict__ boff, const uint32_t* __restrict__ start,
                                                               g2_pair_partial_t* __restrict__ partial, uint32_t nbt, uint32_t S, uint32_t debug_idx_mask) {
    const uint32_t gt = blockIdx.x * blockDim.x + threadIdx.x;
    const uint32_t t = gt >> 1;
    const int comp = (int)(gt & 1u);
    const uint32_t total = boff[nbt];
    const uint64_t lo64 = (uint64_t)t * S;
    if (lo64 >= total) return;
    const uint32_t lo = (uint32_t)lo64;
    const uint32_t hi = (total - lo < S) ? total : lo + S;
    uint32_t k = find_bucket(boff, nbt, lo);
    uint32_t kend = boff[k + 1];
    uint32_t start_k = start[k];
    uint32_t part_off = t - boff[k] / S;
    fq2p::xyzz_pair_t<fq2p::xp_dev> acc;
    acc.inf = true;
    auto slot_of = [&](uint32_t e) -> const g2_lazy_slot_t* { return (const g2_lazy_slot_t*)&bases[(e & 0x7fffffffu) & debug_idx_mask]; };
    for (uint32_t pos = lo;; pos++) {
        const bool end = pos >= hi;
        if (end || pos >= kend) {
            uint4* q = (uint4*)&partial[start_k + part_off].w[16 * comp];
            if (acc.inf) {
#pragma unroll
                for (int c4 = 0; c4 < 4; c4++)
#pragma unroll
                    for (int j = 0; j < 4; j++) q[8 * c4 + j] = make_uint4(0, 0, 0, 0);
            } else {
                const fql_t* cs[4] = {&acc.x[0], &acc.y[0], &acc.zz[0], &acc.zzz[0]};
#pragma unroll
                for (int c4 = 0; c4 < 4; c4++) {
                    const int32_t* v = cs[c4]->v;
                    q[8 * c4 + 0] = make_uint4((uint32_t)v[0], (uint32_t)v[1], (uint32_t)v[2], (uint32_t)v[3]);
                    q[8 * c4 + 1] = make_uint4((uint32_t)v[4], (uint32_t)v[5], (uint32_t)v[6], (uint32_t)v[7]);
                    q[8 * c4 + 2] = make_uint4((uint32_t)v[8], (uint32_t)v[9], (uint32_t)v[10], (uint32_t)v[11]);
                    q[8 * c4 + 3] = make_uint4((uint32_t)v[12], 0u, 0u, 0u);
                }
            }
            if (end) break;
            part_off = 0;
            acc.inf = true;
            do {
                k++;
                kend = boff[k + 1];
            } while (pos >= kend);
            start_k = start[k];
        }
        const uint32_t e = sorted[pos];
        const g2_lazy_slot_t* sp = slot_of(e);
        if (sp->w[g2_lazy_slot_t::INF_WORD]) continue;
        fql_t px[1], py[1];
        sp->component(comp, px[0], py[0]);
        acc.madd(px, py, (e >> 31) != 0);
    }
}

}
```

### snarkvm_amd/csrc/runtime.hip.h

```cpp
#pragma once
#include <hip/hip_runtime.h>
#include <stdint.h>
#include <stdio.h>
#include <stdlib.h>
#include <string.h>
#include <time.h>

#include <atomic>
#include <chrono>
#include <condition_variable>
#include <deque>
#include <functional>
#include <exception>
#include <memory>
#include <mutex>
#include <stdexcept>
#include <string>
#include <thread>
#include <utility>
#include <vector>

#include "../../include/snarkvm_hip.h"
#include "ec.hip.h"
#include "ff.hip.h"
#include "msm.hip.h"
#include "msm_sort.hip.h"
#include "ntt.hip.h"
#include "group.hip.h"
#include "poly.hip.h"
#include "serde.hip.h"

using namespace sv;

static RustError ok() { return RustError{0, nullptr}; }
static RustError fail(int code, const std::string& msg) {
    char* m = (char*)malloc(msg.size() + 1);
    if (m) memcpy(m, msg.c_str(), msg.size() + 1);
    return RustError{code ? code : 1, m};
}
struct hip_failure {
    hipError_t e;
    const char* what;
    int line;
};
#define HIP_TRY(x)                                             \
    do {                                                       \
        hipError_t _e = (x);                                   \
        if (_e != hipSuccess) throw hip_failure{_e, #x, __LINE__}; \
    } while (0)
static RustError from_failure(const hip_failure& f) {
    char buf[512];
    snprintf(buf, sizeof buf, "snarkvm_hip: %s failed at api.hip:%d: %s", f.what, f.line, hipGetErrorString(f.e));
    return fail((int)f.e, buf);
}

static double host_now_ms() {
    timespec ts;
    clock_gettime(CLOCK_MONOTONIC, &ts);
    return ts.tv_sec * 1e3 + ts.tv_nsec * 1e-6;
}

void sv_alloc_note(int slot, size_t bytes, double ms);
void sv_defer_free(void* p);
void sv_drain_frees();
struct alloc_timer_t {
    double t0;
    int slot;
    size_t bytes;
    alloc_timer_t(int s, size_t b) : t0(host_now_ms()), slot(s), bytes(b) {}
    ~alloc_timer_t() { sv_alloc_note(slot, bytes, host_now_ms() - t0); }
};
struct dev_buf {
    void* p = nullptr;
    size_t cap = 0;
    void ensure(size_t bytes) {
        if (bytes <= cap) return;
        size_t want = bytes + bytes / 8 + 256;
        alloc_timer_t timer(0, want);
        if (p) sv_defer_free(p);
        p = nullptr;
        cap = 0;
        if (hipMalloc(&p, want) != hipSuccess) {
            (void)hipGetLastError();
            p = nullptr;
            sv_drain_frees();
            const hipError_t e = hipMalloc(&p, want);
            if (e != hipSuccess) {
                (void)hipGetLastError();
                p = nullptr;
                throw hip_failure{e, "hipMalloc", __LINE__};
            }
        }
        cap = want;
    }
    template <class T>
    T* as() const {
        return (T*)p;
    }
};
struct pinned_buf {
    void* p = nullptr;
    size_t cap = 0;
    void ensure(size_t bytes) {
        if (bytes <= cap) return;
        size_t want = bytes + bytes / 8 + 4096;
        alloc_timer_t timer(2, want);
        if (p) HIP_TRY(hipHostFree(p));
        p = nullptr;
        cap = 0;
        HIP_TRY(hipHostMalloc(&p, want, hipHostMallocDefault));
        cap = want;
    }
    template <class T>
    T* as() const {
        return (T*)p;
    }
};

struct phase_rec {
    const char* name;
    hipEvent_t e0, e1;
    double ms;
};
struct device_t;

struct lane_t {
    device_t* dev = nullptr;
    int index = 0;
    hipStream_t stream = nullptr;
    dev_buf scalars, digits, counts, offsets, scan_tmp, sorted, boff, cnt_a, cnt_b, start_a, start_b, part_a, part_b, part_raw, planes;
    dev_buf rv1, rl1, rcounts2, roff2, rbinstart, rntiles, rtstart, rbsize;
    dev_buf rv2, rl2, rmid_size, rmid_boff;
    dev_buf fold_sums;
    dev_buf tail_flags;
    dev_buf sink_acc;
    dev_buf fchunk;
    dev_buf bases_tmp, scalars_tmp, gen_pts, gen_prod;
    dev_buf ntt_data, ntt_scratch, ntt_acc, ntt_alt;
    dev_buf serde_status;
    dev_buf poly[5];
    pinned_buf pin, pin2;
    hipStream_t alt = nullptr;
    hipEvent_t ev[4] = {};
    std::vector<void*> tw_leases;
    bool in_scope = false;
    struct deferred_out_t {
        void* dst;
        size_t off, bytes;
    };
    std::vector<deferred_out_t> deferred;
    size_t deferred_bytes = 0;
    size_t pin_used = 0;
    std::vector<hipEvent_t> scope_events;
    size_t scope_events_used = 0;
    hipEvent_t scope_event() {
        if (scope_events_used == scope_events.size()) {
            hipEvent_t e;
            HIP_TRY(hipEventCreateWithFlags(&e, hipEventDisableTiming));
            scope_events.push_back(e);
        }
        return scope_events[scope_events_used++];
    }
    std::vector<phase_rec> phases;
    std::vector<hipEvent_t> event_pool;
    size_t events_used = 0;

    hipEvent_t new_event() {
        if (events_used == event_pool.size()) {
            hipEvent_t e;
            HIP_TRY(hipEventCreate(&e));
            event_pool.push_back(e);
        }
        return event_pool[events_used++];
    }
    inline ntt_ctx_t ntt_ctx(hipStream_t st = nullptr);
    inline void begin_call();
    inline void phase_begin(const char* name);
    inline void phase_end();
    inline void phase_host(const char* name, double ms);
    inline void end_call();
    void sync_or_defer() {
        if (!in_scope) HIP_TRY(hipStreamSynchronize(stream));
    }
    void host_result(void* dst, const void* d_src, size_t bytes, bool may_defer = true) {
        if (!in_scope || !may_defer) {
            HIP_TRY(hipMemcpyAsync(dst, d_src, bytes, hipMemcpyDeviceToHost, stream));
            return;
        }
        if (deferred_bytes + bytes > pin2.cap) {
            if (!deferred.empty()) flush_scope();
            pin2.ensure(deferred_bytes + bytes > (size_t)1 << 16 ? deferred_bytes + bytes : (size_t)1 << 16);
        }
        HIP_TRY(hipMemcpyAsync(pin2.as<uint8_t>() + deferred_bytes, d_src, bytes, hipMemcpyDeviceToHost, stream));
        deferred.push_back({dst, deferred_bytes, bytes});
        deferred_bytes += (bytes + 15) & ~(size_t)15;
    }
    inline void flush_scope();
};

struct device_t {
    int logical = 0, physical = 0;
    bool ready = false;
    std::mutex init_mu;
    ntt_tables_t tb{};
    dev_buf tables_mem;
    ntt_tw_cache_t tw;
    static constexpr int LANES = 16;
    lane_t lane[LANES];
    std::mutex mu;
    std::condition_variable cv;
    uint32_t busy = 0;
    static constexpr int SCOPE_LANES_MAX = LANES - 4;
    int scope_held = 0;

    void init() {
        std::lock_guard<std::mutex> lk(init_mu);
        if (ready) return;
        for (int l = 0; l < LANES; l++) {
            lane[l].dev = this;
            lane[l].index = l;
            HIP_TRY(hipStreamCreateWithFlags(&lane[l].stream, hipStreamNonBlocking));
            HIP_TRY(hipStreamCreateWithFlags(&lane[l].alt, hipStreamNonBlocking));
            for (auto& e : lane[l].ev) HIP_TRY(hipEventCreateWithFlags(&e, hipEventDisableTiming));
        }
        static_assert(NTT_LG_MAX + 1 <= 32, "size_inv");
        const size_t entries = 8 * NTT_TW_SIZE + 2 * NTT_LOCAL + 4 * NTT_TOP + 32 + 8;
        tables_mem.ensure(entries * sizeof(fr_mem_t));
        fr_mem_t* base = tables_mem.as<fr_mem_t>();
        size_t off = 0;
        auto take = [&](size_t n) {
            fr_mem_t* r = base + off;
            off += n;
            return r;
        };
        for (int d = 0; d < 2; d++) {
            tb.pow_lo[d] = take(NTT_TW_SIZE);
            tb.pow_hi[d] = take(NTT_TW_SIZE);
            tb.g_lo[d] = take(NTT_TW_SIZE);
            tb.g_hi[d] = take(NTT_TW_SIZE);
            tb.local[d] = take(NTT_LOCAL);
            tb.pow_top[d] = take(NTT_TOP);
            tb.g_top[d] = take(NTT_TOP);
        }
        tb.size_inv = take(32);
        tb.consts = take(8);
        hipStream_t st = lane[0].stream;
        hipLaunchKernelGGL(ntt_setup_consts, dim3(1), dim3(64), 0, st, tb);
        hipLaunchKernelGGL(ntt_fill_tables, dim3(NTT_TW_SIZE / 256), dim3(256), 0, st, tb);
        HIP_TRY(hipGetLastError());
        HIP_TRY(hipStreamSynchronize(st));
        ready = true;
    }
    int take(lane_t** out, int want) {
        std::unique_lock<std::mutex> lk(mu);
        cv.wait(lk, [&] { return busy != (1u << LANES) - 1; });
        int got = 0;
        for (int l = 0; l < LANES && got < want; l++)
            if (!(busy & (1u << l))) {
                busy |= 1u << l;
                out[got++] = &lane[l];
            }
        return got;
    }
    bool try_take(lane_t** out) {
        std::lock_guard<std::mutex> lk(mu);
        for (int l = 0; l < LANES; l++)
            if (!(busy & (1u << l))) {
                busy |= 1u << l;
                *out = &lane[l];
                return true;
            }
        return false;
    }
    int try_take_n(lane_t** out, int want) {
        std::lock_guard<std::mutex> lk(mu);
        int got = 0;
        for (int l = 0; l < LANES && got < want; l++)
            if (!(busy & (1u << l))) {
                busy |= 1u << l;
                out[got++] = &lane[l];
            }
        return got;
    }
    lane_t* take_for_scope(bool block) {
        std::unique_lock<std::mutex> lk(mu);
        auto room = [&] { return busy != (1u << LANES) - 1 && scope_held < SCOPE_LANES_MAX; };
        if (block)
            cv.wait(lk, room);
        else if (!room())
            return nullptr;
        for (int i = 0; i < LANES; i++) {
            const int l = block ? i : LANES - 1 - i;
            if (!(busy & (1u << l))) {
                busy |= 1u << l;
                scope_held++;
                return &lane[l];
            }
        }
        return nullptr;
    }
    void give(lane_t* l, bool from_scope = false) {
        {
            std::lock_guard<std::mutex> lk(mu);
            busy &= ~(1u << l->index);
            if (from_scope) scope_held--;
        }
        cv.notify_all();
    }
};

struct runtime_t {
    std::mutex cfg_mu;
    std::vector<int> want;
    std::vector<std::unique_ptr<device_t>> devs;
    bool configured = false;
    std::atomic<uint32_t> rr{0};
    std::atomic<bool> profiling{false};
    std::mutex prof_mu;
    std::vector<std::pair<std::string, double>> last_phases;

    void configure() {
        std::lock_guard<std::mutex> lk(cfg_mu);
        if (configured) return;
        int ndev = 0;
        hipError_t e = hipGetDeviceCount(&ndev);
        if (e != hipSuccess || ndev == 0) throw hip_failure{e == hipSuccess ? hipErrorNoDevice : e, "hipGetDeviceCount (no MI355X visible)", __LINE__};
        std::vector<int> ids = want;
        if (ids.empty()) {
            if (const char* env = getenv("SNARKVM_HIP_DEVICES")) {
                for (const char* p = env; *p;) {
                    char* end = nullptr;
                    long v = strtol(p, &end, 10);
                    if (end == p) break;
                    ids.push_back((int)v);
                    p = (*end == ',') ? end + 1 : end;
                }
            }
        }
        if (ids.empty())
            for (int d = 0; d < ndev; d++) ids.push_back(d);
        for (int id : ids)
            if (id < 0 || id >= ndev) throw hip_failure{hipErrorInvalidDevice, "device index out of range (snarkvm_hip_set_devices / SNARKVM_HIP_DEVICES)", __LINE__};
        for (size_t i = 0; i < ids.size(); i++) {
            devs.emplace_back(new device_t());
            devs.back()->logical = (int)i;
            devs.back()->physical = ids[i];
        }
        configured = true;
    }
    int ndev() {
        configure();
        return (int)devs.size();
    }
    int device_of(const void* ptr) {
        configure();
        hipPointerAttribute_t at;
        if (!ptr || hipPointerGetAttributes(&at, ptr) != hipSuccess) {
            (void)hipGetLastError();
            return -1;
        }
        std::vector<int> match;
        for (auto& d : devs)
            if (d->physical == at.device) match.push_back(d->logical);
        if (match.empty()) return -1;
        return match[rr.fetch_add(1) % match.size()];
    }
};
extern runtime_t g_rt;

static void tu_kernel_attributes(int logical) {
    static std::mutex mu;
    static std::vector<char> done;
    std::lock_guard<std::mutex> lk(mu);
    if ((int)done.size() <= logical) done.resize(logical + 1, 0);
    if (done[logical]) return;
    HIP_TRY(hipFuncSetAttribute((const void*)scan_one_block_kernel, hipFuncAttributeMaxDynamicSharedMemorySize, (int)(SCAN_ONE_MAX * 4)));
#ifdef SV_TU_G1
    HIP_TRY(hipFuncSetAttribute((const void*)msm_accumulate_lazy_kernel<true>, hipFuncAttributeMaxDynamicSharedMemorySize, 128 * 1024));
#endif
#ifdef SV_TU_NTT
    HIP_TRY(hipFuncSetAttribute((const void*)ntt_pass_kernel_v2<false, ntt_arith_u>, hipFuncAttributeMaxDynamicSharedMemorySize, 96 * 1024));
    HIP_TRY(hipFuncSetAttribute((const void*)ntt_pass_kernel_v2<true, ntt_arith_u>, hipFuncAttributeMaxDynamicSharedMemorySize, 96 * 1024));
#endif
    done[logical] = 1;
}

static constexpr int SCOPE_AUX_MAX = 7;
struct scope_pending_t {
    hipEvent_t done;
    std::function<void()> finish;
    const void* tag;
};
struct thread_scope_t {
    lane_t* lane = nullptr;
    int prev_device = -1;
    unsigned flags = 0;
    lane_t* aux[SCOPE_AUX_MAX] = {};
    int naux = 0;
    unsigned aux_rr = 0;
    bool aux_exhausted = false;
    std::vector<scope_pending_t> pending;
    thread_scope_t() = default;
    thread_scope_t(const thread_scope_t&) = default;
    thread_scope_t& operator=(const thread_scope_t&) = default;
    ~thread_scope_t();
};
extern thread_local thread_scope_t g_tl_scope;
static thread_scope_t& tl_scope() { return g_tl_scope; }
static void scope_flush() {
    thread_scope_t& sc = tl_scope();
    if (!sc.lane) return;
    std::exception_ptr err;
    for (scope_pending_t& p : sc.pending) {
        try {
            HIP_TRY(hipEventSynchronize(p.done));
            p.finish();
        } catch (...) {
            if (!err) err = std::current_exception();
        }
    }
    sc.pending.clear();
    try {
        sc.lane->flush_scope();
        for (int i = 0; i < sc.naux; i++) HIP_TRY(hipStreamSynchronize(sc.aux[i]->stream));
    } catch (...) {
        if (!err) err = std::current_exception();
    }
    sc.lane->pin_used = 0;
    sc.lane->scope_events_used = 0;
    for (int i = 0; i < sc.naux; i++) sc.aux[i]->pin_used = 0, sc.aux[i]->scope_events_used = 0;
    if (err) std::rethrow_exception(err);
}
static void scope_collect(const void* tag) {
    thread_scope_t& sc = tl_scope();
    if (!sc.lane) return;
    std::exception_ptr err;
    if (tag) {
        auto ready = [](const scope_pending_t& p) {
            const hipError_t e = hipEventQuery(p.done);
            if (e == hipSuccess) return true;
            (void)hipGetLastError();
            return false;
        };
        auto wanted_ready = [&]() {
            for (const scope_pending_t& p : sc.pending)
                if (p.tag == tag && !ready(p)) return false;
            return true;
        };
        for (size_t i = 0; i < sc.pending.size() && !wanted_ready();) {
            if (sc.pending[i].tag != tag && ready(sc.pending[i])) {
                try {
                    sc.pending[i].finish();
                } catch (...) {
                    if (!err) err = std::current_exception();
                }
                sc.pending.erase(sc.pending.begin() + (ptrdiff_t)i);
            } else {
                i++;
            }
        }
    }
    std::vector<scope_pending_t> keep;
    for (scope_pending_t& p : sc.pending) {
        if (tag && p.tag != tag) {
            keep.push_back(std::move(p));
            continue;
        }
        try {
            HIP_TRY(hipEventSynchronize(p.done));
            p.finish();
        } catch (...) {
            if (!err) err = std::current_exception();
        }
    }
    sc.pending.swap(keep);
    if (sc.pending.empty()) {
        sc.lane->pin_used = 0, sc.lane->scope_events_used = 0;
        for (int i = 0; i < sc.naux; i++) sc.aux[i]->pin_used = 0, sc.aux[i]->scope_events_used = 0;
    }
    if (err) std::rethrow_exception(err);
}
struct lane_guard {
    std::vector<lane_t*> lanes;
    int prev_device = -1;
    bool borrowed = false;
    bool first_borrowed = false;
    lane_guard() {}
    lane_guard(const lane_guard&) = delete;
    explicit lane_guard(int dev) {
        lane_t* sl = tl_scope().lane;
        if (sl && (dev < 0 || (dev < (int)g_rt.devs.size() && g_rt.devs[dev]->physical == sl->dev->physical))) {
            borrowed = true;
            lanes.push_back(sl);
            tu_kernel_attributes(sl->dev->logical);
            return;
        }
        acquire(dev, 1);
    }
    void acquire(int dev, int want) {
        scope_flush();
        g_rt.configure();
        const int nd = (int)g_rt.devs.size();
        if (dev >= nd) throw hip_failure{hipErrorInvalidDevice, "logical device index out of range", __LINE__};
        if (lane_t* sl = tl_scope().lane) {
            if (dev < 0 || g_rt.devs[dev]->physical == sl->dev->physical) {
                lanes.push_back(sl);
                first_borrowed = true;
                tu_kernel_attributes(sl->dev->logical);
                lane_t* more[device_t::LANES];
                const int n = want > 1 ? sl->dev->try_take_n(more, want - 1) : 0;
                for (int i = 0; i < n; i++) lanes.push_back(more[i]);
                return;
            }
        }
        if (prev_device < 0 && hipGetDevice(&prev_device) != hipSuccess) prev_device = 0;
        device_t* d = nullptr;
        lane_t* got[device_t::LANES];
        int n = 0;
        if (dev >= 0) {
            d = g_rt.devs[dev].get();
        } else {
            const uint32_t s = g_rt.rr.fetch_add(1);
            for (int i = 0; i < nd && !d; i++) {
                device_t* cand = g_rt.devs[(s + i) % nd].get();
                if (want == 1) {
                    if (cand->try_take(&got[0])) {
                        d = cand;
                        n = 1;
                    }
                } else {
                    d = cand;
                }
            }
            if (!d) d = g_rt.devs[s % nd].get();
        }
        if (!n) n = d->take(got, want);
        try {
            HIP_TRY(hipSetDevice(d->physical));
            d->init();
            tu_kernel_attributes(d->logical);
        } catch (...) {
            for (int i = 0; i < n; i++) d->give(got[i]);
            if (prev_device >= 0) (void)hipSetDevice(prev_device);
            throw;
        }
        for (int i = 0; i < n; i++) lanes.push_back(got[i]);
    }
    lane_t& c() { return *lanes[0]; }
    ~lane_guard() {
        if (borrowed) return;
        for (size_t i = first_borrowed ? 1 : 0; i < lanes.size(); i++) lanes[i]->dev->give(lanes[i]);
        if (prev_device >= 0) (void)hipSetDevice(prev_device);
    }
};

inline ntt_ctx_t lane_t::ntt_ctx(hipStream_t st) { return ntt_ctx_t{st ? st : stream, &dev->tb, &dev->tw, &tw_leases}; }
inline void lane_t::begin_call() {
    phases.clear();
    events_used = 0;
}
inline void lane_t::phase_begin(const char* name) {
    if (!g_rt.profiling.load(std::memory_order_relaxed)) return;
    phase_rec r{name, new_event(), new_event(), 0.0};
    HIP_TRY(hipEventRecord(r.e0, stream));
    phases.push_back(r);
}
inline void lane_t::phase_end() {
    if (!g_rt.profiling.load(std::memory_order_relaxed) || phases.empty()) return;
    HIP_TRY(hipEventRecord(phases.back().e1, stream));
}
inline void lane_t::phase_host(const char* name, double ms) {
    if (!g_rt.profiling.load(std::memory_order_relaxed)) return;
    phases.push_back(phase_rec{name, nullptr, nullptr, ms});
}
static void ntt_tw_release(device_t* dev, std::vector<void*>& leases) { ntt_tw_release_entries(dev->tw, leases); }
inline void lane_t::flush_scope() {
    HIP_TRY(hipStreamSynchronize(stream));
    for (const deferred_out_t& d : deferred) memcpy(d.dst, pin2.as<uint8_t>() + d.off, d.bytes);
    deferred.clear();
    deferred_bytes = 0;
    if (!tw_leases.empty()) ntt_tw_release(dev, tw_leases);
    sv_drain_frees();
}
inline void lane_t::end_call() {
    if (in_scope) return;
    sv_drain_frees();
    if (!tw_leases.empty()) {
        HIP_TRY(hipStreamSynchronize(stream));
        ntt_tw_release(dev, tw_leases);
    }
    if (phases.empty()) return;
    HIP_TRY(hipStreamSynchronize(stream));
    std::vector<std::pair<std::string, double>> out;
    for (auto& r : phases) {
        if (r.e0) {
            float ms = 0;
            HIP_TRY(hipEventElapsedTime(&ms, r.e0, r.e1));
            r.ms = ms;
        }
        out.emplace_back(r.name, r.ms);
    }
    std::lock_guard<std::mutex> lk(g_rt.prof_mu);
    g_rt.last_phases.swap(out);
}

template <class Fn>
static void for_each_device(const std::vector<int>& devices, Fn fn) {
    if (devices.size() <= 1) {
        for (int d : devices) fn(d);
        return;
    }
    std::vector<std::thread> th;
    std::vector<std::exception_ptr> errs(devices.size());
    for (size_t i = 0; i < devices.size(); i++)
        th.emplace_back([&, i] {
            try {
                fn(devices[i]);
            } catch (...) {
                errs[i] = std::current_exception();
            }
        });
    for (auto& t : th) t.join();
    for (auto& e : errs)
        if (e) std::rethrow_exception(e);
}

struct msm_ticket_t;
template <class F>
struct bases_handle_t {
    std::vector<aff_mem_t<F>*> d;
    size_t n = 0;
    int tables = 1;
    int table_bits = 256;
    mutable std::mutex co_mu;
    mutable std::condition_variable co_cv;
    mutable std::deque<msm_ticket_t*> co_q;
    mutable int co_leaders = 0;
    void free_all() {
        int prev = 0;
        (void)hipGetDevice(&prev);
        for (size_t i = 0; i < d.size(); i++)
            if (d[i]) {
                (void)hipSetDevice(g_rt.devs[i]->physical);
                (void)hipFree(d[i]);
                d[i] = nullptr;
            }
        (void)hipSetDevice(prev);
    }
};
struct snarkvm_hip_bases : bases_handle_t<fq_t> {};

static const uint64_t FQ_R[6] = {202099033278250856ull,  5854854902718660529ull, 11492539364873682930ull,
                                 8885205928937022213ull, 5545221690922665192ull, 39800542322357402ull};
template <class F>
static void write_infinity(void* out) {
    const size_t fb = sizeof(typename F::mem_t);
    memset(out, 0, 3 * fb);
    memcpy((uint8_t*)out + fb, FQ_R, 48);
}

static constexpr int MSM_MAX_POS = 320;
template <class F>
struct msm_accum_t {
    xyzz_t<F> at[MSM_MAX_POS];
    bool used[MSM_MAX_POS];
    int top = -1;
    msm_accum_t() {
        for (int i = 0; i < MSM_MAX_POS; i++) used[i] = false;
    }
    void add(int pos, const xyzz_t<F>& p) {
        if (p.is_inf()) return;
        if (pos < 0 || pos >= MSM_MAX_POS) throw std::runtime_error("msm: bit position out of range");
        if (!used[pos]) {
            at[pos] = p;
            used[pos] = true;
        } else {
            at[pos].add(p);
        }
        if (pos > top) top = pos;
    }
    void finish(void* out) const {
        xyzz_t<F> t = xyzz_t<F>::inf();
        for (int p = top; p >= 0; p--) {
            t = t.dbl();
            if (used[p]) t.add(at[p]);
        }
        const jac_t<F> j = t.to_jacobian();
        uint32_t w[3 * F::MEM_WORDS];
        j.x.to_raw_words(w);
        j.y.to_raw_words(w + F::MEM_WORDS);
        j.z.to_raw_words(w + 2 * F::MEM_WORDS);
        memcpy(out, w, sizeof w);
    }
};
struct msm_pending_t {
    const void* planes = nullptr;
    int nplanes = 0;
    int tail_windows = 0, nbits = 0;
    int c = 0, m = 0;
    bool folded = false;
    int ninst = 0;
    bool lazy = false;
    int pos(int idx) const {
        const int tw = idx / nbits, j = idx % nbits;
        if (ninst) return (tw & 1) * m + j;
        return folded ? c * (tw >> 1) + (tw & 1) * m + j : c * tw + j;
    }
};
template <class F>
static constexpr size_t msm_point_bytes() {
    return sizeof(F) == sizeof(fq_t) && sizeof(xyzz_mem_t<fqz_t>) > sizeof(xyzz_mem_t<F>) ? sizeof(xyzz_mem_t<fqz_t>) : sizeof(xyzz_mem_t<F>);
}
template <class F>
static xyzz_t<F> msm_plane(const msm_pending_t& pd, int i) {
    if constexpr (sizeof(F) == sizeof(fq_t)) {
        if (pd.lazy) {
            const xyzz_t<fqz_t> z = load_xyzz<fqz_t>(&((const xyzz_mem_t<fqz_t>*)pd.planes)[i]);
            if (z.is_inf()) return xyzz_t<F>::inf();
            return {z.x.to_exact(), z.y.to_exact(), z.zz.to_exact(), z.zzz.to_exact()};
        }
    }
    return load_xyzz<F>(&((const xyzz_mem_t<F>*)pd.planes)[i]);
}
template <class F>
static void msm_collect(msm_accum_t<F>& acc, const msm_pending_t& pd) {
    for (int i = 0; i < pd.nplanes; i++) acc.add(pd.pos(i), msm_plane<F>(pd, i));
}
template <class F>
static void msm_collect_inst(msm_accum_t<F>& acc, const msm_pending_t& pd, int inst) {
    const int per = 2 * pd.nbits;
    for (int i = inst * per; i < (inst + 1) * per; i++) acc.add(pd.pos(i), msm_plane<F>(pd, i));
}
struct msm_multi_t {
    const msm_inst_t* d_inst = nullptr;
    uint32_t K = 0;
    size_t npad = 0;
    size_t hn = 0;
    size_t plane_capacity = 0;
};

static size_t msm_acc_lds() {
    const long env = tuning().acc_lds;
    return env < 0 ? 0 : (size_t)env;
}
template <class F>
static bool msm_lazy_on();
template <class F>
static bool msm_lazy_tail_on() {
    return sizeof(F) == sizeof(fq_t) && msm_lazy_on<F>() && tuning().lazy_tail != 0;
}
template <class F>
static size_t msm_partial_bytes() {
    return msm_lazy_tail_on<F>() ? sizeof(xyzz_mem_t<fqz_t>) : sizeof(xyzz_mem_t<F>);
}
struct msm_tail_geom_t {
    int fold_m, fold_hb, tail_windows, nbits;
    bool fold;
};
static msm_tail_geom_t msm_tail_geometry(const msm_plan_t& pl, uint32_t nwin, msm_pending_t& pd, int ninst) {
    msm_tail_geom_t g;
    const int K = pl.c - 1;
    g.fold_m = (K + 1) / 2;
    g.fold_hb = K - g.fold_m;
    g.fold = K >= 11 || (K >= 4 && pl.c * pl.W < 128);
    g.tail_windows = g.fold ? 2 * (int)nwin : (int)nwin;
    g.nbits = g.fold ? g.fold_m + 1 : pl.c;
    pd.tail_windows = g.tail_windows;
    pd.nbits = g.nbits;
    pd.nplanes = g.tail_windows * g.nbits;
    pd.c = pl.c;
    pd.m = g.fold_m;
    pd.folded = g.fold;
    pd.ninst = ninst;
    if ((!ninst && pd.nplanes > MSM_MAX_POS) || pl.c * (pl.W - 1) + (g.fold ? g.fold_m : 0) + g.nbits > MSM_MAX_POS)
        throw hip_failure{hipErrorInvalidValue, "msm: window geometry exceeds the tail's bit-position range", __LINE__};
    return g;
}
template <class F>
static void msm_tail_launch(lane_t& c, const msm_plan_t& pl, const msm_tail_geom_t& g, uint32_t nwin, uint32_t nbt, const xyzz_mem_t<F>* sums,
                            const uint32_t* start, const uint32_t* cnt, const msm_pending_t& pd, void* host_planes) {
    hipStream_t st = c.stream;
    c.planes.ensure((size_t)pd.nplanes * sizeof(xyzz_mem_t<F>));
    const bool is_g2 = sizeof(F) == sizeof(fq2_t);
    const int hex = (is_g2 && tuning().hex2) ? 1 : 0;
    int quads_planes = (tuning().tail_quads >> (is_g2 ? 0 : 2)) & 1, quads_fold = (tuning().tail_quads >> (is_g2 ? 1 : 3)) & 1;
    if (g.fold_m > 8) quads_planes = 0;
    uint32_t* fold_flags = nullptr;
    uint32_t* plane_flags = nullptr;
    if (is_g2) {
        const size_t nslots = g.fold ? ((size_t)nwin << (g.fold_m + 1)) : 0;
        c.tail_flags.ensure((nslots + (size_t)pd.nplanes) * 4);
        fold_flags = c.tail_flags.as<uint32_t>();
        plane_flags = fold_flags + nslots;
    }
    if (g.fold) {
        c.fold_sums.ensure(((size_t)nwin << (g.fold_m + 1)) * sizeof(xyzz_mem_t<F>));
        const unsigned fold_blocks = ((1u << g.fold_m) + (1u << g.fold_hb)) * (unsigned)nwin;
        unsigned fold_threads = (nbt >= (1u << 18) || fold_blocks > 512u) ? 64u : 256u;
        if (sizeof(F) <= 64 && nbt < (1u << 18) && fold_blocks > 512u && fold_blocks <= 1024u && tuning().fold_mid == 128) fold_threads = 128u;
        if (sizeof(F) > 64 && fold_threads == 256u && fold_blocks > 256u && (tuning().fold_threads2 == 128 || tuning().fold_threads2 == 64)) fold_threads = (unsigned)tuning().fold_threads2;
        if (sizeof(F) > 64 && fold_threads == 256u && fold_blocks <= 256u && (tuning().fold_small2 == 128 || tuning().fold_small2 == 64)) fold_threads = (unsigned)tuning().fold_small2;
        if (fold_threads == 64u) quads_fold = 0;
        const dim3 fold_grid((1u << g.fold_m) + (1u << g.fold_hb), (unsigned)nwin);
        hipLaunchKernelGGL((msm_fold_kernel<F>), fold_grid, dim3(fold_threads), 0, st, sums, start, cnt, c.fold_sums.as<xyzz_mem_t<F>>(), g.fold_m, g.fold_hb, hex, quads_fold,
                           fold_flags);
        if constexpr (TAIL_FLAGGED<F>::value)
            hipLaunchKernelGGL((msm_fold_fix_kernel<F>), fold_grid, dim3(64), 0, st, sums, start, cnt, c.fold_sums.as<xyzz_mem_t<F>>(), g.fold_m, g.fold_hb,
                               (const uint32_t*)fold_flags);
        const unsigned plane_threads = quads_planes ? (g.fold_m <= 4 ? 64u : g.fold_m == 5 ? 128u : 256u) : (g.fold_m <= 6 ? 64u : g.fold_m == 7 ? 128u : 256u);
        const dim3 plane_grid((unsigned)g.nbits, (unsigned)g.tail_windows);
        hipLaunchKernelGGL((msm_bitplane_kernel<F, true>), plane_grid, dim3(plane_threads), 0, st, (const xyzz_mem_t<F>*)c.fold_sums.as<xyzz_mem_t<F>>(),
                           (const uint32_t*)nullptr, (const uint32_t*)nullptr, c.planes.as<xyzz_mem_t<F>>(), pl.nb, g.fold_m, g.fold_hb, hex, quads_planes, plane_flags);
        if constexpr (TAIL_FLAGGED<F>::value)
            hipLaunchKernelGGL((msm_bitplane_fix_kernel<F, true>), plane_grid, dim3(64), 0, st, (const xyzz_mem_t<F>*)c.fold_sums.as<xyzz_mem_t<F>>(), (const uint32_t*)nullptr,
                               (const uint32_t*)nullptr, c.planes.as<xyzz_mem_t<F>>(), pl.nb, g.fold_m, g.fold_hb, (const uint32_t*)plane_flags);
    } else {
        const dim3 plane_grid((unsigned)g.nbits, (unsigned)g.tail_windows);
        hipLaunchKernelGGL((msm_bitplane_kernel<F, false>), plane_grid, dim3(256), 0, st, sums, start, cnt, c.planes.as<xyzz_mem_t<F>>(), pl.nb, 0, 0, hex, 0, plane_flags);
        if constexpr (TAIL_FLAGGED<F>::value)
            hipLaunchKernelGGL((msm_bitplane_fix_kernel<F, false>), plane_grid, dim3(64), 0, st, sums, start, cnt, c.planes.as<xyzz_mem_t<F>>(), pl.nb, 0, 0,
                               (const uint32_t*)plane_flags);
    }
    HIP_TRY(hipGetLastError());
    HIP_TRY(hipMemcpyAsync(host_planes, c.planes.p, (size_t)pd.nplanes * sizeof(xyzz_mem_t<F>), hipMemcpyDeviceToHost, st));
}
struct msm_bucket_sink_t {
    void* acc = nullptr;
    uint32_t L = 1, slot = 0, nbt = 0;
    hipEvent_t after = nullptr, done = nullptr;
};
template <class T, class PB, class PE>
static void msm_reduce_and_tail(lane_t& c, const msm_plan_t& pl, const msm_tail_geom_t& tg, uint32_t nwin, uint32_t nbt, int rounds, size_t T0_max, size_t T1_max,
                                const msm_bucket_sink_t* sink, msm_pending_t& pd, void* host_planes, PB&& phase_begin, PE&& phase_end) {
    hipStream_t st = c.stream;
    phase_begin("msm_reduce_partials");
    uint32_t *cnt_in = c.cnt_a.as<uint32_t>(), *cnt_out = c.cnt_b.as<uint32_t>();
    uint32_t *start_in = c.start_a.as<uint32_t>(), *start_out = c.start_b.as<uint32_t>();
    xyzz_mem_t<T> *pin = c.part_a.as<xyzz_mem_t<T>>(), *pout = c.part_b.as<xyzz_mem_t<T>>();
    size_t T_in_max = T0_max;
    for (int r = 0; r < rounds; r++) {
        size_t T_out_max = T_in_max / pl.S2 + nbt + 1;
        if (T_out_max > T1_max) T_out_max = T1_max;
        hipLaunchKernelGGL(msm_alloc_kernel, dim3((nbt + 1 + 255) / 256), dim3(256), 0, st, cnt_in, cnt_out, nbt, pl.S2);
        exclusive_scan_u32(st, cnt_out, start_out, (size_t)nbt + 1, c.scan_tmp.as<uint32_t>());
        hipLaunchKernelGGL((msm_reduce_kernel<T>), dim3((unsigned)((T_out_max + 255) / 256)), dim3(256), 0, st, pin, start_in, cnt_in, start_out, pout, nbt,
                           pl.S2);
        std::swap(cnt_in, cnt_out);
        std::swap(start_in, start_out);
        std::swap(pin, pout);
        T_in_max = T_out_max;
    }
    phase_end();
    if (sink) {
        phase_begin("msm_bucket_merge");
        if (sink->after) HIP_TRY(hipStreamWaitEvent(st, sink->after, 0));
        hipLaunchKernelGGL((msm_bucket_merge_kernel<T>), dim3((nbt + 255) / 256), dim3(256), 0, st, (const xyzz_mem_t<T>*)pin, (const uint32_t*)start_in,
                           (const uint32_t*)cnt_in, (xyzz_mem_t<T>*)sink->acc, nbt, sink->L, sink->slot);
        if (sink->done) HIP_TRY(hipEventRecord(sink->done, st));
        phase_end();
        HIP_TRY(hipGetLastError());
        pd.nplanes = 0;
        return;
    }
    phase_begin("msm_bucket_reduce");
    msm_tail_launch<T>(c, pl, tg, nwin, nbt, pin, start_in, cnt_in, pd, host_planes);
    phase_end();
}
template <class F>
static void msm_launch_accumulate(lane_t& c, const msm_plan_t& pl, const aff_mem_t<F>* vbase, uint32_t* boffp, uint32_t nbt, size_t nthreads, bool one_wave,
                                  bool ltail) {
    hipStream_t st = c.stream;
#ifdef SV_BENCH
    static const uint32_t dbg_mask = getenv("SNARKVM_HIP_DEBUG_IDX_MASK") ? (uint32_t)strtoul(getenv("SNARKVM_HIP_DEBUG_IDX_MASK"), nullptr, 0) : 0xffffffffu;
#else
    constexpr uint32_t dbg_mask = 0xffffffffu;
#endif
    const size_t tmax = nthreads + nbt + 1;
    if constexpr (sizeof(F) == sizeof(fq_t)) {
        if (msm_lazy_on<F>()) {
            if (!ltail) c.part_raw.ensure(tmax * sizeof(g1_lazy_partial_t));
            g1_lazy_partial_t* raw_out = ltail ? c.part_a.as<g1_lazy_partial_t>() : c.part_raw.as<g1_lazy_partial_t>();
            hipLaunchKernelGGL((msm_accumulate_lazy_kernel<true>), dim3((unsigned)((nthreads + 255) / 256)), dim3(256), one_wave || tuning().acc_one_wg ? msm_acc_lds() : 0, st,
                               vbase, c.sorted.as<uint32_t>(), boffp, c.start_a.as<uint32_t>(), raw_out, nbt, pl.S, dbg_mask);
            if (!ltail)
                hipLaunchKernelGGL(g1_partials_to_exact_kernel, dim3((unsigned)((tmax + 255) / 256)), dim3(256), 0, st, (const g1_lazy_partial_t*)raw_out,
                                   c.part_a.as<g1_xyzz_mem_t>(), (const uint32_t*)c.start_a.as<uint32_t>(), nbt);
            return;
        }
    } else {
#ifndef SV_NO_G2
        if (msm_lazy_on<F>()) {
            c.part_raw.ensure(tmax * sizeof(g2_pair_partial_t));
            hipLaunchKernelGGL((msm_accumulate_pair2_kernel<false>), dim3((unsigned)((2 * nthreads + 255) / 256)), dim3(256), 0, st, vbase, c.sorted.as<uint32_t>(),
                               boffp, c.start_a.as<uint32_t>(), c.part_raw.as<g2_pair_partial_t>(), nbt, pl.S, dbg_mask);
            hipLaunchKernelGGL(g2_pair_partials_to_exact_kernel, dim3((unsigned)((8 * tmax + 255) / 256)), dim3(256), 0, st,
                               (const g2_pair_partial_t*)c.part_raw.as<g2_pair_partial_t>(), c.part_a.as<xyzz_mem_t<fq2_t>>(),
                               (const uint32_t*)c.start_a.as<uint32_t>(), nbt);
            return;
        }
#endif
    }
    if (one_wave)
        hipLaunchKernelGGL((msm_accumulate_seg_kernel<F, 1, true>), dim3((unsigned)((nthreads + 255) / 256)), dim3(256), 0, st, vbase, c.sorted.as<uint32_t>(), boffp,
                           c.start_a.as<uint32_t>(), c.part_a.as<xyzz_mem_t<F>>(), nbt, pl.S, dbg_mask);
    else
        hipLaunchKernelGGL((msm_accumulate_seg_kernel<F, 1, false>), dim3((unsigned)((nthreads + 255) / 256)), dim3(256), 0, st, vbase, c.sorted.as<uint32_t>(), boffp,
                           c.start_a.as<uint32_t>(), c.part_a.as<xyzz_mem_t<F>>(), nbt, pl.S, dbg_mask);
}
template <class F>
static size_t msm_plane_bytes() {
    return (size_t)MSM_MAX_POS * msm_point_bytes<F>();
}
template <class F>
static msm_pending_t msm_run(lane_t& c, const aff_mem_t<F>* d_bases, const uint4* d_scalars, size_t n, void* host_planes, int window_bits,
                             const aff_mem_t<F>* d_bases1 = nullptr, size_t n0 = ~(size_t)0, int scalars_montgomery = 0, int tables = 1,
                             size_t table_stride = 0, bool profile = true, int table_bits = 0, const msm_multi_t* mu = nullptr,
                             const msm_bucket_sink_t* sink = nullptr, hipEvent_t scalars_read = nullptr) {
    static const int trace2 = getenv("SNARKVM_HIP_TRACE") ? atoi(getenv("SNARKVM_HIP_TRACE")) : 0;
    const char* cur_phase = "";
    auto phase_begin = [&](const char* name) {
        cur_phase = name;
        if (trace2 >= 2) fprintf(stderr, "[snarkvm_hip] msm n=%zu: %s ...\n", n, name);
        if (profile) c.phase_begin(name);
    };
    auto phase_end = [&]() {
        if (profile) c.phase_end();
        if (trace2 >= 2) {
            const hipError_t e = hipStreamSynchronize(c.stream);
            fprintf(stderr, "[snarkvm_hip] msm n=%zu: %s done (%s)\n", n, cur_phase, hipGetErrorString(e));
        }
    };
    msm_pending_t pd;
    pd.planes = host_planes;
    if (n0 > n) n0 = n;
    if (n == 0) return pd;
    if (n >= ((size_t)1 << 31)) throw hip_failure{hipErrorInvalidValue, "msm: npoints must be < 2^31", __LINE__};
    const msm_plan_t pl = msm_make_plan(n, mu ? table_bits : window_bits, tables, table_bits);
    const bool wide = pl.c > 16;
    if (mu && (wide || pl.W != 1 || pl.c < 12 || (size_t)pl.J * mu->hn >= ((size_t)1 << 31) || n != mu->npad || n % SORT_TILE))
        throw hip_failure{hipErrorInvalidValue, "msm: geometry not eligible for a fused multi-instance run", __LINE__};
    if ((size_t)pl.Wd * n >= ((size_t)1 << 32)) throw hip_failure{hipErrorInvalidValue, "msm: windows * npoints must be < 2^32", __LINE__};
    if ((size_t)pl.J * n >= ((size_t)1 << 31)) throw hip_failure{hipErrorInvalidValue, "msm: tables * npoints must be < 2^31", __LINE__};
    const aff_mem_t<F>* vb1 = d_bases1 ? d_bases1 : d_bases;
    const aff_mem_t<F>* vbase = mu ? d_bases : (vb1 < d_bases ? vb1 : d_bases);
    if (!mu) {
        const size_t top0 = (size_t)(d_bases - vbase) + n0, top1 = (size_t)(vb1 - vbase) + (n - n0);
        if ((size_t)(pl.J - 1) * table_stride + (top0 > top1 ? top0 : top1) >= ((size_t)1 << 31))
            throw hip_failure{hipErrorInvalidValue, "msm: base slots must be addressable in 31 bits (tables * registered points < 2^31)", __LINE__};
    }
    hipStream_t st = c.stream;
    const size_t E_max = (size_t)pl.Wd * n;
    const uint32_t nwin = mu ? mu->K : (uint32_t)pl.W;
    const uint32_t nbt = nwin * pl.nb;

    c.scan_tmp.ensure((scan_tmp_elems((size_t)nbt + 1)) * 4);
    c.boff.ensure(((size_t)nbt + 2) * 4);
    c.cnt_a.ensure(((size_t)nbt + 1) * 4);
    c.cnt_b.ensure(((size_t)nbt + 1) * 4);
    c.start_a.ensure(((size_t)nbt + 1) * 4);
    c.start_b.ensure(((size_t)nbt + 1) * 4);
    const size_t slack = (size_t)nbt / 32 + 64;
    const size_t T0_max = E_max / pl.S + nbt + 1 + slack;
    const size_t T1_max = T0_max / pl.S2 + nbt + 1 + slack;
    const bool ltail = msm_lazy_tail_on<F>();
    pd.lazy = ltail;
    c.part_a.ensure(T0_max * msm_partial_bytes<F>());
    c.part_b.ensure(T1_max * msm_partial_bytes<F>());
    const int K = pl.c - 1;
    const msm_tail_geom_t tg = msm_tail_geometry(pl, nwin, pd, mu ? (int)mu->K : 0);
    if (mu && (size_t)pd.nplanes > mu->plane_capacity) throw hip_failure{hipErrorInvalidValue, "msm: plane staging of the fused group too small", __LINE__};
    if (sink && (mu || sink->nbt != nbt)) throw hip_failure{hipErrorInvalidValue, "msm: bucket sink does not match the plan", __LINE__};
    c.planes.ensure((size_t)pd.nplanes * msm_partial_bytes<F>());

    const int fused_env = tuning().fused;
    const bool fused = !mu && wide && fused_env && pl.c <= 22 && pl.Wd <= FUSED_MAX_ROWS;
    msm_digit_params_t dp;
    memcpy(dp.bias, pl.bias, sizeof dp.bias);
    dp.c = pl.c;
    dp.W = pl.Wd;
    dp.n = n;
    dp.montgomery = scalars_montgomery;
    if (!fused) {
        phase_begin("msm_digits");
        c.digits.ensure(E_max * (wide ? sizeof(uint32_t) : sizeof(uint16_t)));
        size_t blocks = (n + 255) / 256;
        if (mu)
            hipLaunchKernelGGL(msm_digits_multi_kernel, dim3((unsigned)blocks), dim3(256), 0, st, mu->d_inst, mu->K, c.digits.as<uint16_t>(), dp);
        if (blocks > 256 * 16) blocks = 256 * 16;
        if (mu)
            ;
        else if (wide)
            hipLaunchKernelGGL((msm_digits_kernel<uint32_t>), dim3((unsigned)blocks), dim3(256), 0, st, d_scalars, c.digits.as<uint32_t>(), dp);
        else
            hipLaunchKernelGGL((msm_digits_kernel<uint16_t>), dim3((unsigned)blocks), dim3(256), 0, st, d_scalars, c.digits.as<uint16_t>(), dp);
        phase_end();
        if (scalars_read) HIP_TRY(hipEventRecord(scalars_read, st));
    }
    int rounds = 0;
    const bool single_round = mu || (size_t)pl.Wd * n <= ((size_t)1 << 22);
    const bool prefetch_ok = (size_t)pl.Wd * n <= ((size_t)1 << 22);
    {
        msm_radix_params_t rp;
        rp.n = n;
        rp.c = pl.c;
        rp.W = pl.W;
        rp.J = pl.J;
        if (mu) {
            rp.inst = mu->d_inst;
            rp.ninst = mu->K;
            rp.vstride = (uint32_t)mu->hn;
        } else {
            rp.vn0 = (uint32_t)n0;
            rp.vr0 = (uint32_t)(d_bases - vbase);
            rp.vr1 = (uint32_t)(vb1 - vbase);
            rp.vstride = (uint32_t)table_stride;
        }
        const int LBL = K < 7 ? K : 7;
        rp.LB = wide ? 14 : LBL;
        rp.HB = K - rp.LB;
        rp.nb = pl.nb;
        rp.xcd = (uint32_t)tuning().xcd;
        rp.tiles_per_row = fused ? (uint32_t)((n + FUSED_TILE - 1) / FUSED_TILE) : (uint32_t)((n + SORT_TILE - 1) / SORT_TILE);
        rp.TPW = (uint32_t)pl.J * rp.tiles_per_row;
        const uint32_t B1 = 1u << rp.HB;
        const uint32_t nbins = nwin * B1;
        const size_t ncounts1 = (size_t)(mu ? B1 : nbins) * rp.TPW;
        const size_t tiles1 = (size_t)(mu ? 1 : pl.W) * rp.TPW;
        const uint32_t nseg_last = wide ? nbins << 7 : nbins;
        const size_t tiles2_max = E_max / SORT_TILE + nseg_last + 1;
        c.counts.ensure(ncounts1 * 4);
        c.offsets.ensure(ncounts1 * 4);
        c.scan_tmp.ensure(scan_tmp_elems(ncounts1 > (size_t)nbt + 2 ? ncounts1 : (size_t)nbt + 2) * 4);
        c.rv1.ensure(E_max * 4);
        c.rl1.ensure(E_max * (wide ? 2 : 1));
        c.rcounts2.ensure(tiles2_max * 128 * 4);
        c.roff2.ensure(tiles2_max * 128 * 4);
// ... 43 lines not shown
            switch (pl.c) { SV_FUSED_SCATTER(17) SV_FUSED_SCATTER(18) SV_FUSED_SCATTER(19) SV_FUSED_SCATTER(20) SV_FUSED_SCATTER(21) SV_FUSED_SCATTER(22) }
#undef SV_FUSED_SCATTER
            if (scalars_read) HIP_TRY(hipEventRecord(scalars_read, st));
        } else if (wide) {
            phase_begin("msm_sort_level1");
            hipLaunchKernelGGL((radix_hist1_kernel<uint32_t>), dim3((unsigned)tiles1), dim3(SORT_THREADS), 0, st, c.digits.as<uint32_t>(), counts1, rp);
            exclusive_scan_u32(st, counts1, off1, ncounts1, c.scan_tmp.as<uint32_t>());
            hipLaunchKernelGGL((radix_scatter1_kernel<uint32_t, uint16_t>), dim3((unsigned)tiles1), dim3(SORT_THREADS), 0, st, c.digits.as<uint32_t>(),
                               counts1, off1, c.rv1.as<uint32_t>(), c.rl1.as<uint16_t>(), rp);
        } else {
            phase_begin("msm_sort_level1");
            hipLaunchKernelGGL((radix_hist1_kernel<uint16_t>), dim3((unsigned)tiles1), dim3(SORT_THREADS), 0, st, c.digits.as<uint16_t>(), counts1, rp);
            exclusive_scan_u32(st, counts1, off1, ncounts1, c.scan_tmp.as<uint32_t>());
            hipLaunchKernelGGL((radix_scatter1_kernel<uint16_t, uint8_t>), dim3((unsigned)tiles1), dim3(SORT_THREADS), 0, st, c.digits.as<uint16_t>(),
                               counts1, off1, c.rv1.as<uint32_t>(), c.rl1.as<uint8_t>(), rp);
        }
        if (mu)
            hipLaunchKernelGGL(radix_bin_layout_multi_kernel, dim3((nbins + 1 + 255) / 256), dim3(256), 0, st, off1, counts1, ncounts1,
                               c.rbinstart.as<uint32_t>(), nbins, rp);
        else if (!fused)
            hipLaunchKernelGGL(radix_bin_layout_kernel, dim3((nbins + 1 + 255) / 256), dim3(256), 0, st, off1, counts1, ncounts1, c.rbinstart.as<uint32_t>(),
                               nbins, rp.TPW);
        phase_end();
        auto tile_segments = [&](const uint32_t* seg_start, uint32_t nseg) {
            hipLaunchKernelGGL(radix_bin_tiles_kernel, dim3((nseg + 1 + 255) / 256), dim3(256), 0, st, seg_start, c.rntiles.as<uint32_t>(), nseg);
            exclusive_scan_u32(st, c.rntiles.as<uint32_t>(), c.rtstart.as<uint32_t>(), (size_t)nseg + 1, c.scan_tmp.as<uint32_t>());
        };
        auto colscan = [&](uint32_t* sizes, uint32_t nsegs, int bits, uint32_t* dmax) {
            if (nsegs <= 4096)
                hipLaunchKernelGGL(radix_colscan2_seg_kernel, dim3(nsegs), dim3(1024), 0, st, c.rcounts2.as<uint32_t>(), c.roff2.as<uint32_t>(),
                                   c.rtstart.as<uint32_t>(), sizes, nsegs, bits, dmax);
            else
                hipLaunchKernelGGL(radix_colscan2_kernel, dim3(((nsegs << bits) + 1 + 255) / 256), dim3(256), 0, st, c.rcounts2.as<uint32_t>(),
                                   c.roff2.as<uint32_t>(), c.rtstart.as<uint32_t>(), sizes, nsegs, bits, dmax);
        };
        const uint32_t* seg_start = c.rbinstart.as<uint32_t>();
        uint32_t nseg = nbins;
        const uint32_t* v_in = c.rv1.as<uint32_t>();
        if (wide) {
            phase_begin("msm_sort_level2");
            const uint32_t ngroups = nseg << 7;
            const size_t tmax = E_max / SORT_TILE + nseg + 1;
            c.rv2.ensure(E_max * 4);
            c.rl2.ensure(E_max);
            c.rmid_size.ensure(((size_t)ngroups + 3) * 4);
            c.rmid_boff.ensure(((size_t)ngroups + 3) * 4);
            c.scan_tmp.ensure(scan_tmp_elems((size_t)ngroups + 2) * 4);
            uint32_t* msize = c.rmid_size.as<uint32_t>();
            uint32_t* mboff = c.rmid_boff.as<uint32_t>();
            tile_segments(seg_start, nseg);
            hipLaunchKernelGGL((radix_hist2_kernel<uint16_t>), dim3((unsigned)tmax), dim3(SORT_THREADS), 0, st, c.rl1.as<uint16_t>(), seg_start,
                               c.rtstart.as<uint32_t>(), c.rcounts2.as<uint32_t>(), nseg, 7, 7);
            HIP_TRY(hipMemsetAsync(msize + ngroups + 1, 0, 4, st));
            colscan(msize, nseg, 7, msize + ngroups + 1);
            exclusive_scan_u32(st, msize, mboff, (size_t)ngroups + 1, c.scan_tmp.as<uint32_t>());
            hipLaunchKernelGGL((radix_scatter2_kernel<uint16_t, uint8_t>), dim3((unsigned)tmax), dim3(SORT_THREADS), 0, st, v_in, c.rl1.as<uint16_t>(),
                               seg_start, c.rtstart.as<uint32_t>(), c.rcounts2.as<uint32_t>(), c.roff2.as<uint32_t>(), mboff, c.rv2.as<uint32_t>(),
                               c.rl2.as<uint8_t>(), nseg, 7, 7, (uint32_t)tuning().xcd);
            phase_end();
            seg_start = mboff;
            nseg = ngroups;
            v_in = c.rv2.as<uint32_t>();
        }
        phase_begin(wide ? "msm_sort_level3" : "msm_sort_level2");
        tile_segments(seg_start, nseg);
        const uint8_t* rem_last = wide ? c.rl2.as<uint8_t>() : c.rl1.as<uint8_t>();
        hipLaunchKernelGGL((radix_hist2_kernel<uint8_t>), dim3((unsigned)tiles2_max), dim3(SORT_THREADS), 0, st, rem_last, seg_start,
                           c.rtstart.as<uint32_t>(), c.rcounts2.as<uint32_t>(), nseg, LBL, 0);
        HIP_TRY(hipMemsetAsync(d_max, 0, 4, st));
        colscan(bsize, nseg, LBL, d_max);
        exclusive_scan_u32(st, bsize, boffp, (size_t)nbt + 1, c.scan_tmp.as<uint32_t>());
        hipLaunchKernelGGL((radix_scatter2_kernel<uint8_t, uint8_t>), dim3((unsigned)tiles2_max), dim3(SORT_THREADS), 0, st, v_in, rem_last, seg_start,
                           c.rtstart.as<uint32_t>(), c.rcounts2.as<uint32_t>(), c.roff2.as<uint32_t>(), boffp, c.sorted.as<uint32_t>(),
                           (uint8_t*)nullptr, nseg, LBL, 0, (uint32_t)tuning().xcd);
        phase_end();
        phase_begin("msm_accumulate");
        {
            const int env_rounds = tuning().reduce_rounds;
            if (!single_round) rounds = env_rounds < 0 ? 0 : (env_rounds > 8 ? 8 : env_rounds);
            if (mu && tuning().fuse_reduce > 0) rounds = tuning().fuse_reduce > 4 ? 4 : tuning().fuse_reduce;
            if (mu && tuning().fuse_reduce < 0) rounds = mu->K >= 8 ? 1 : 0;
            hipLaunchKernelGGL(msm_alloc_seg_kernel, dim3((nbt + 1 + 255) / 256), dim3(256), 0, st, boffp, c.cnt_a.as<uint32_t>(), nbt, pl.S);
            exclusive_scan_u32(st, c.cnt_a.as<uint32_t>(), c.start_a.as<uint32_t>(), (size_t)nbt + 1, c.scan_tmp.as<uint32_t>());
            msm_launch_accumulate<F>(c, pl, vbase, boffp, nbt, (E_max + pl.S - 1) / pl.S, single_round && prefetch_ok, ltail);
        }
        phase_end();
    }
    if constexpr (sizeof(F) == sizeof(fq_t)) {
        if (ltail) {
            msm_reduce_and_tail<fqz_t>(c, pl, tg, nwin, nbt, rounds, T0_max, T1_max, sink, pd, host_planes, phase_begin, phase_end);
            return pd;
        }
    }
    msm_reduce_and_tail<F>(c, pl, tg, nwin, nbt, rounds, T0_max, T1_max, sink, pd, host_planes, phase_begin, phase_end);
    return pd;
}
template <class F>
static msm_pending_t msm_tail_from_sink(lane_t& c, size_t chunk_n, int window_bits, const msm_bucket_sink_t& sink, void* host_planes, int tables = 1,
                                        int table_bits = 0) {
    msm_pending_t pd;
    pd.planes = host_planes;
    const msm_plan_t pl = msm_make_plan(chunk_n, window_bits, tables, table_bits);
    const uint32_t nwin = (uint32_t)pl.W, nbt = nwin * pl.nb;
    if (nbt != sink.nbt) throw hip_failure{hipErrorInvalidValue, "msm: bucket sink does not match the plan", __LINE__};
    const msm_tail_geom_t tg = msm_tail_geometry(pl, nwin, pd, 0);
    c.start_a.ensure(((size_t)nbt + 1) * 4);
    c.cnt_a.ensure(((size_t)nbt + 1) * 4);
    hipLaunchKernelGGL(msm_sink_lists_kernel, dim3((nbt + 1 + 255) / 256), dim3(256), 0, c.stream, c.start_a.as<uint32_t>(), c.cnt_a.as<uint32_t>(), nbt, sink.L);
    pd.lazy = msm_lazy_tail_on<F>();
    c.phase_begin("msm_bucket_reduce");
    if constexpr (sizeof(F) == sizeof(fq_t)) {
        if (pd.lazy) {
            msm_tail_launch<fqz_t>(c, pl, tg, nwin, nbt, (const xyzz_mem_t<fqz_t>*)sink.acc, c.start_a.as<uint32_t>(), c.cnt_a.as<uint32_t>(), pd, host_planes);
            c.phase_end();
            return pd;
        }
    }
    msm_tail_launch<F>(c, pl, tg, nwin, nbt, (const xyzz_mem_t<F>*)sink.acc, c.start_a.as<uint32_t>(), c.cnt_a.as<uint32_t>(), pd, host_planes);
    c.phase_end();
    return pd;
}
template <class F>
static void msm_run_sync(lane_t& c, const aff_mem_t<F>* d_bases, const uint4* d_scalars, size_t n, void* out, int window_bits,
                         const aff_mem_t<F>* d_bases1 = nullptr, size_t n0 = ~(size_t)0, int scalars_montgomery = 0, int tables = 1,
                         size_t table_stride = 0, int table_bits = 0) {
    if (c.in_scope && c.pin_used) scope_flush();
    c.pin.ensure(msm_plane_bytes<F>());
    const msm_pending_t pd = msm_run<F>(c, d_bases, d_scalars, n, c.pin.p, window_bits, d_bases1, n0, scalars_montgomery, tables, table_stride, true, table_bits);
    HIP_TRY(hipStreamSynchronize(c.stream));
    const double t0 = host_now_ms();
    msm_accum_t<F>* acc = new msm_accum_t<F>();
    std::unique_ptr<msm_accum_t<F>> hold(acc);
    msm_collect<F>(*acc, pd);
    acc->finish(out);
    c.phase_host("msm_host_finish", host_now_ms() - t0);
}

template <class F>
static bool msm_lazy_on() {
    return sizeof(F) == sizeof(fq_t) ? tuning().lazy != 0 : tuning().lazy2 != 0;
}
template <class F>
static void convert_bases(lane_t& c, const uint8_t* d_in, size_t stride, size_t n, aff_mem_t<F>* d_out, hipStream_t st = nullptr, bool for_msm = false) {
    if (!n) return;
    const int form406 = for_msm && msm_lazy_on<F>() ? 1 : 0;
    hipLaunchKernelGGL((convert_bases_kernel<F>), dim3((unsigned)((n + 255) / 256)), dim3(256), 0, st ? st : c.stream, d_in, stride, n, d_out, form406);
    HIP_TRY(hipGetLastError());
}
static void bases_to_lazy_form(lane_t& c, g1_aff_mem_t* d, size_t slots) {
    if (!slots || !msm_lazy_on<fq_t>()) return;
    hipLaunchKernelGGL(g1_bases_to_form406_kernel, dim3((unsigned)((slots + 255) / 256)), dim3(256), 0, c.stream, d, slots);
    HIP_TRY(hipGetLastError());
}
#ifndef SV_NO_G2
static void bases_to_lazy_form(lane_t& c, aff_mem_t<fq2_t>* d, size_t slots) {
    if (!slots || !msm_lazy_on<fq2_t>()) return;
    hipLaunchKernelGGL(g2_bases_to_form406_kernel, dim3((unsigned)((slots + 255) / 256)), dim3(256), 0, c.stream, d, slots);
    HIP_TRY(hipGetLastError());
}
#endif

template <class F>
static void precompute_tables_run(lane_t& c, aff_mem_t<F>* d, size_t n, int tables, int table_bits) {
    if (tables <= 1 || !n) return;
    int run = (int)(n >> 16);
    run = run < 1 ? 1 : (run > PRE_RUN ? PRE_RUN : run);
    const size_t slab = n < PRE_SLAB ? n : PRE_SLAB;
    c.gen_pts.ensure(4 * slab * sizeof(typename F::mem_t));
    for (int j = 1; j < tables; j++)
        for (size_t lo = 0; lo < n; lo += PRE_SLAB) {
            const size_t cnt = n - lo < PRE_SLAB ? n - lo : PRE_SLAB;
            const size_t threads = (cnt + run - 1) / run;
            hipLaunchKernelGGL((precompute_table_kernel<F>), dim3((unsigned)((threads + 255) / 256)), dim3(256), 0, c.stream, d + (size_t)(j - 1) * n + lo,
                               d + (size_t)j * n + lo, cnt, table_bits, run, (typename F::mem_t*)c.gen_pts.p);
        }
    HIP_TRY(hipGetLastError());
}

static int batch_lanes(size_t npoints) {
    const int env = tuning().lanes;
    int l = env > 0 ? env : (npoints >= ((size_t)1 << 20) ? 3 : 8);
    return l < 1 ? 1 : (l > device_t::LANES ? device_t::LANES : l);
}
static constexpr size_t MSM_SPLIT_MIN = (size_t)1 << 18;
static size_t msm_chunk_pairs() {
    const int lg = tuning().msm_chunk_lg;
    return (size_t)1 << (lg < 16 ? 16 : (lg > 30 ? 30 : lg));
}
static size_t msm_scalar_chunk_pairs() {
    const int lg = tuning().scalar_chunk_lg;
    return (size_t)1 << (lg < 18 ? 18 : lg > 30 ? 30 : lg);
}

template <class Upload, class Compute>
static void lane_ring_run(lane_guard& lg, size_t count, Upload&& upload, Compute&& compute, int trace, double t_begin) {
    const size_t L = lg.lanes.size();
    const int phys = lg.lanes[0]->dev->physical;
    std::mutex mu;
    std::condition_variable cv;
    std::vector<char> uploaded(count, 0), enqueued(count, 0);
    std::vector<hipEvent_t> up(count), used(count);
    for (size_t j = 0; j < count; j++) {
        up[j] = lg.lanes[j % L]->new_event();
        used[j] = lg.lanes[j % L]->new_event();
    }
    std::exception_ptr up_err, cp_err;
    std::thread uploader([&] {
        try {
            HIP_TRY(hipSetDevice(phys));
            for (size_t j = 0; j < count; j++) {
                lane_t& c = *lg.lanes[j % L];
                if (j >= L) {
                    char state;
                    {
                        std::unique_lock<std::mutex> lk(mu);
                        cv.wait(lk, [&] { return enqueued[j - L] != 0; });
                        state = enqueued[j - L];
                    }
                    if (state == 2) break;
                    HIP_TRY(hipEventSynchronize(used[j - L]));
                }
                const double t0 = host_now_ms();
                upload(j, c.alt);
                HIP_TRY(hipEventRecord(up[j], c.alt));
                if (trace) fprintf(stderr, "[snarkvm_hip] chunk %zu dev %d lane %d: uploaded t+%.2f .. t+%.2f ms\n", j, c.dev->logical, c.index, t0 - t_begin, host_now_ms() - t_begin);
                {
                    std::lock_guard<std::mutex> lk(mu);
                    uploaded[j] = 1;
                }
                cv.notify_all();
            }
        } catch (...) {
            up_err = std::current_exception();
            std::lock_guard<std::mutex> lk(mu);
            for (auto& u : uploaded) u = 2;
            cv.notify_all();
        }
    });
    try {
        for (size_t j = 0; j < count; j++) {
            lane_t& c = *lg.lanes[j % L];
            {
                std::unique_lock<std::mutex> lk(mu);
                cv.wait(lk, [&] { return uploaded[j] != 0; });
                if (uploaded[j] == 2) break;
            }
            HIP_TRY(hipStreamWaitEvent(c.stream, up[j], 0));
            const double t0 = host_now_ms();
            compute(j);
            HIP_TRY(hipEventRecord(used[j], c.stream));
            if (trace) fprintf(stderr, "[snarkvm_hip] chunk %zu: enqueued t+%.2f .. t+%.2f ms\n", j, t0 - t_begin, host_now_ms() - t_begin);
            {
                std::lock_guard<std::mutex> lk(mu);
                enqueued[j] = 1;
            }
            cv.notify_all();
        }
    } catch (...) {
        cp_err = std::current_exception();
        std::lock_guard<std::mutex> lk(mu);
        for (auto& e : enqueued) e = 2;
        cv.notify_all();
    }
    uploader.join();
    if (cp_err || up_err) {
        for (lane_t* l : lg.lanes) {
            (void)hipStreamSynchronize(l->alt);
            (void)hipStreamSynchronize(l->stream);
        }
        std::rethrow_exception(cp_err ? cp_err : up_err);
    }
}

template <class F>
static void msm_host_chunked(void* out, const void* points, size_t npoints, const void* scalars, size_t stride) {
    const size_t min_stride = 2 * sizeof(typename F::mem_t) + 8;
    if (stride < min_stride || (stride & 7)) throw hip_failure{hipErrorInvalidValue, "msm: bad ffi_affine_sz for this curve", __LINE__};
    scope_flush();
    const int nd = g_rt.ndev();
    static const int trace = getenv("SNARKVM_HIP_TRACE") ? atoi(getenv("SNARKVM_HIP_TRACE")) : 0;
    const double t_begin = host_now_ms();
    size_t nchunks = npoints < 2 * MSM_SPLIT_MIN ? 1 : (npoints + msm_chunk_pairs() - 1) / msm_chunk_pairs();
    if (nchunks == 1 && npoints >= 2 * MSM_SPLIT_MIN && (nd > 1 || npoints >= ((size_t)1 << 20))) nchunks = 2;
    std::vector<size_t> bound;
    for (size_t i = 0; i <= nchunks; i++) bound.push_back(npoints * i / nchunks);
    const bool taper = tuning().taper != 0 && nchunks >= 3 && bound[nchunks] - bound[nchunks - 1] >= MSM_SPLIT_MIN;
    if (taper) {
        const size_t lo = bound[nchunks - 1], len = npoints - lo;
        bound.back() = lo + len / 2;
        bound.push_back(lo + len / 2 + len / 4);
        bound.push_back(npoints);
        nchunks += 2;
    }
    int ramp = tuning().taper != 0 && nchunks >= 2 ? tuning().ramp : 0;
    while (ramp > 0 && (bound[1] >> ramp) < ((size_t)1 << 17)) ramp--;
    if (ramp > 0) {
        const size_t len = bound[1];
        std::vector<size_t> front;
        size_t pos = len >> ramp;
        front.push_back(pos);
        for (int k = ramp; k >= 1; k--) {
            pos += len >> k;
            front.push_back(k == 1 ? len : pos);
        }
        bound.erase(bound.begin() + 1);
        bound.insert(bound.begin() + 1, front.begin(), front.end());
// ... 620 lines not shown
```

### snarkvm_amd/csrc/tuning.hip.h

```cpp
#pragma once
#include <stdio.h>
#include <stdlib.h>
#include <string.h>

namespace sv {

struct tuning_t {
    int lazy = 1, lazy2 = 1, fused = 1;
    long acc_lds = 96 * 1024;
    int acc_one_wg = 0, reduce_rounds = 1, fuse_batch = 1, fuse_max_k = 64, fuse_reduce = -1, coalesce = 1, coalesce_us = 40, lanes = 0;
    int msm_chunk_lg = 20, scalar_chunk_lg = 22, taper = 1, ring_lanes = 3, seg = 0, seg2 = 0, fold_l = 0, scan1 = 1;
    int ntt_min_tiles = 256, ntt_full_tw = 1, ntt_fold = 1, ntt_batch = 1;
    int xcd = 1, fold_threads2 = 128, coalesce_slots = 2, ramp = 3, scalar_geo = 4, lazy_tail = 1, horner2 = 1, hex2 = 1, group_quad = 1, tail_quads = 13, fold_small2 = 256, fold_mid = 128;

    bool set(const char* key, long v) {
#define SV_TUNE_KEY(name)                  \
    if (!strcmp(key, #name)) {             \
        name = (decltype(name))v;          \
        return true;                       \
    }
        SV_TUNE_KEY(lazy) SV_TUNE_KEY(lazy2) SV_TUNE_KEY(fused) SV_TUNE_KEY(acc_lds)
        SV_TUNE_KEY(acc_one_wg) SV_TUNE_KEY(reduce_rounds) SV_TUNE_KEY(fuse_batch) SV_TUNE_KEY(fuse_max_k) SV_TUNE_KEY(fuse_reduce) SV_TUNE_KEY(coalesce)
        SV_TUNE_KEY(coalesce_us) SV_TUNE_KEY(lanes) SV_TUNE_KEY(msm_chunk_lg) SV_TUNE_KEY(scalar_chunk_lg) SV_TUNE_KEY(taper) SV_TUNE_KEY(ring_lanes) SV_TUNE_KEY(seg) SV_TUNE_KEY(seg2)
        SV_TUNE_KEY(fold_l) SV_TUNE_KEY(scan1) SV_TUNE_KEY(ntt_min_tiles) SV_TUNE_KEY(ntt_full_tw) SV_TUNE_KEY(ntt_fold)
        SV_TUNE_KEY(ntt_batch) SV_TUNE_KEY(xcd) SV_TUNE_KEY(fold_threads2) SV_TUNE_KEY(coalesce_slots) SV_TUNE_KEY(ramp) SV_TUNE_KEY(scalar_geo) SV_TUNE_KEY(lazy_tail) SV_TUNE_KEY(horner2) SV_TUNE_KEY(hex2) SV_TUNE_KEY(group_quad) SV_TUNE_KEY(tail_quads) SV_TUNE_KEY(fold_small2) SV_TUNE_KEY(fold_mid)
#undef SV_TUNE_KEY
        return false;
    }
    void parse(const char* s) {
        while (s && *s) {
            while (*s == ',' || *s == ' ') s++;
            const char* eq = strchr(s, '=');
            const char* end = strchr(s, ',');
            if (!end) end = s + strlen(s);
            if (!*s) break;
            char key[32] = {0};
            if (!eq || eq > end || (size_t)(eq - s) >= sizeof key) {
                fprintf(stderr, "[snarkvm_hip] SNARKVM_HIP_TUNING: malformed item at \"%s\" (ignored)\n", s);
            } else {
                memcpy(key, s, (size_t)(eq - s));
                char* num_end = nullptr;
                const long v = strtol(eq + 1, &num_end, 0);
                if (num_end == eq + 1 || !set(key, v)) fprintf(stderr, "[snarkvm_hip] SNARKVM_HIP_TUNING: unknown key or bad value \"%s\" (ignored)\n", key);
            }
            s = end;
        }
    }
    void clamp() {
        auto fix = [](const char* key, auto& v, long lo, long hi) {
            if ((long)v < lo || (long)v > hi) {
                const long was = (long)v;
                v = (decltype(v + 0))((long)v < lo ? lo : hi);
                fprintf(stderr, "[snarkvm_hip] SNARKVM_HIP_TUNING: %s=%ld is out of range [%ld, %ld]; using %ld\n", key, was, lo, hi, (long)v);
            }
        };
        fix("coalesce_slots", coalesce_slots, 1, 8);
        fix("coalesce_us", coalesce_us, 0, 100000);
        fix("fuse_max_k", fuse_max_k, 2, 256);
        fix("fuse_reduce", fuse_reduce, -1, 4);
        fix("reduce_rounds", reduce_rounds, 0, 8);
        fix("lanes", lanes, 0, 8);
        fix("ring_lanes", ring_lanes, 2, 8);
        fix("ntt_min_tiles", ntt_min_tiles, 1, 1 << 20);
        fix("acc_lds", acc_lds, 0, 160 * 1024);
        fix("msm_chunk_lg", msm_chunk_lg, 16, 30);
        fix("scalar_chunk_lg", scalar_chunk_lg, 18, 30);
        fix("ramp", ramp, 0, 6);
        fix("scalar_geo", scalar_geo, 0, 16);
        fix("seg", seg, 0, 4096);
        fix("seg2", seg2, 0, 256);
        fix("fold_l", fold_l, 0, 64);
    }
};
inline const tuning_t& tuning() {
    static const tuning_t t = [] {
        tuning_t v;
        v.parse(getenv("SNARKVM_HIP_TUNING"));
        v.clamp();
        return v;
    }();
    return t;
}

}
```

Measured before the change: 572.3 million pairs/s.

## Accumulate G1 MSM buckets in twisted Edwards coordinates with precomputed base slots

When bases are registered with multiple tables, a twisted Edwards form (Y-X, Y+X, 2dXY) of every base is precomputed on the device and stored in a registry. The bucket accumulation then runs a TE mixed-add kernel, converts the partials back to XYZZ, and runs the existing lazy kernel again in a recompute mode for the cases the TE path flags. The aim is fewer field multiplications per bucket addition, since the extended Edwards mixed add has no exceptional cases. The cost is an extra 160-byte slot per base in HBM, which is more memory traffic per point than the affine form, plus two extra kernel launches per chunk.

Result: slower. 549.5 million pairs/s (-4.0%).

```diff
diff --git a/include/snarkvm_hip.h b/include/snarkvm_hip.h
--- a/include/snarkvm_hip.h
+++ b/include/snarkvm_hip.h
@@ -153,6 +153,8 @@
 int snarkvm_hip_selftest_msm_plan(size_t n, int window_bits, int tables, int table_bits, uint32_t *out);
 int snarkvm_hip_selftest_g1_finish(const void *planes_projective, const int32_t *pos, size_t n, void *out);
 int snarkvm_hip_selftest_fq_lazy(uint64_t seed, int iters);
+int snarkvm_hip_selftest_g1_te(uint64_t seed, int iters);
+RustError snarkvm_hip_g1_te_stats(uint64_t* out);
 int snarkvm_hip_selftest_g1_lazy_tail(uint64_t seed, int iters);
 int snarkvm_hip_selftest_fq2_pair(const void *points, size_t npoints, uint64_t seed, int iters);
 int snarkvm_hip_selftest_g2_hex(const void *points, size_t npoints, uint64_t seed, int iters);
diff --git a/rust/snarkvm-algorithms-hip/src/sys.rs b/rust/snarkvm-algorithms-hip/src/sys.rs
--- a/rust/snarkvm-algorithms-hip/src/sys.rs
+++ b/rust/snarkvm-algorithms-hip/src/sys.rs
@@ -90,6 +90,8 @@
     pub fn snarkvm_hip_selftest_msm_plan(n: usize, window_bits: i32, tables: i32, table_bits: i32, out: *mut u32) -> i32;
     pub fn snarkvm_hip_selftest_g1_finish(planes_projective: *const c_void, pos: *const i32, n: usize, out: *mut c_void) -> i32;
     pub fn snarkvm_hip_selftest_fq_lazy(seed: u64, iters: i32) -> i32;
+    pub fn snarkvm_hip_selftest_g1_te(seed: u64, iters: i32) -> i32;
+    pub fn snarkvm_hip_g1_te_stats(out: *mut u64) -> Error;
     pub fn snarkvm_hip_selftest_g1_lazy_tail(seed: u64, iters: i32) -> i32;
     pub fn snarkvm_hip_selftest_fq2_pair(points: *const c_void, npoints: usize, seed: u64, iters: i32) -> i32;
     pub fn snarkvm_hip_selftest_g2_hex(points: *const c_void, npoints: usize, seed: u64, iters: i32) -> i32;
diff --git a/snarkvm_amd/_lib.py b/snarkvm_amd/_lib.py
--- a/snarkvm_amd/_lib.py
+++ b/snarkvm_amd/_lib.py
@@ -21,7 +21,7 @@
     "snarkvm_hip_g1_fixed_base_msm", "snarkvm_hip_g1_group_ntt",
     "snarkvm_hip_set_profiling", "snarkvm_hip_get_phase_count", "snarkvm_hip_get_phase_name",
     "snarkvm_hip_get_phase_ms", "snarkvm_hip_synchronize", "snarkvm_hip_coalescer_stats",
-    "snarkvm_hip_selftest_field", "snarkvm_hip_selftest_g1_msm_naive", "snarkvm_hip_selftest_msm_plan", "snarkvm_hip_selftest_g1_finish", "snarkvm_hip_selftest_fq_lazy", "snarkvm_hip_selftest_g1_lazy_tail", "snarkvm_hip_selftest_ntt_plan", "snarkvm_hip_selftest_ntt_twiddle", "snarkvm_hip_selftest_ntt_index", "snarkvm_hip_selftest_ntt_host", "snarkvm_hip_selftest_fq2_pair", "snarkvm_hip_selftest_g2_hex", "snarkvm_hip_devtest_field", "snarkvm_hip_devtest_g2_tail_repeat",
+    "snarkvm_hip_selftest_field", "snarkvm_hip_selftest_g1_msm_naive", "snarkvm_hip_selftest_msm_plan", "snarkvm_hip_selftest_g1_finish", "snarkvm_hip_selftest_fq_lazy", "snarkvm_hip_selftest_g1_te", "snarkvm_hip_g1_te_stats", "snarkvm_hip_selftest_g1_lazy_tail", "snarkvm_hip_selftest_ntt_plan", "snarkvm_hip_selftest_ntt_twiddle", "snarkvm_hip_selftest_ntt_index", "snarkvm_hip_selftest_ntt_host", "snarkvm_hip_selftest_fq2_pair", "snarkvm_hip_selftest_g2_hex", "snarkvm_hip_devtest_field", "snarkvm_hip_devtest_g2_tail_repeat",
 ]
 
 
@@ -63,7 +63,7 @@
                    "snarkvm_hip_register_bases_serialized", "snarkvm_hip_g1_deserialize", "snarkvm_hip_g1_serialize", "snarkvm_hip_g1_sum", "snarkvm_hip_g2_deserialize", "snarkvm_hip_g2_serialize", "snarkvm_hip_g2_deserialize_compressed", "snarkvm_hip_g2_serialize_compressed",
                    "snarkvm_hip_register_bases_g2", "snarkvm_hip_msm_g2_registered", "snarkvm_hip_msm_g2_registered_batch",
                    "snarkvm_hip_g1_fixed_base_msm", "snarkvm_hip_g1_group_ntt",
-                   "snarkvm_hip_devtest_field", "snarkvm_hip_devtest_g2_tail_repeat"]
+                   "snarkvm_hip_devtest_field", "snarkvm_hip_devtest_g2_tail_repeat", "snarkvm_hip_g1_te_stats"]
         for name in err_fns:
             getattr(L, name).restype = RustError
         L.snarkvm_hip_device_count.restype = ctypes.c_int
@@ -71,6 +71,7 @@
         L.snarkvm_hip_num_devices.restype = ctypes.c_int
         L.snarkvm_hip_selftest_g1_finish.restype = ctypes.c_int
         L.snarkvm_hip_selftest_fq_lazy.restype = ctypes.c_int
+        L.snarkvm_hip_selftest_g1_te.restype = ctypes.c_int
         L.snarkvm_hip_selftest_g1_lazy_tail.restype = ctypes.c_int
         for name in ("snarkvm_hip_selftest_ntt_plan", "snarkvm_hip_selftest_ntt_twiddle", "snarkvm_hip_selftest_ntt_index", "snarkvm_hip_selftest_ntt_host"):
             getattr(L, name).restype = ctypes.c_int
diff --git a/snarkvm_amd/csrc/api.hip b/snarkvm_amd/csrc/api.hip
--- a/snarkvm_amd/csrc/api.hip
+++ b/snarkvm_amd/csrc/api.hip
@@ -307,6 +307,7 @@
                 }
             }
         }
+        g1_te_attach(h.get());
     } catch (...) {
         h->free_all();
         throw;
@@ -1169,6 +1170,133 @@
     if (!zq.is_zero() || !zq.neg().is_zero() || !(zq + zq).is_zero() || (zq + fqz_t::one()).is_zero()) return -1;
     return 0;
 }
+int snarkvm_hip_selftest_g1_te(uint64_t seed, int iters) {
+    uint32_t xw[12], yw[12];
+    memcpy(xw, G1_GEN_X, 48);
+    memcpy(yw, G1_GEN_Y, 48);
+    const g1_aff_t g{fq_t::unpack(xw).from_mem_mont(), fq_t::unpack(yw).from_mem_mont()};
+    const fq_t one = fq_t::one(), c406 = fq_t::from_table(FqLConv::C406);
+    const fq_t s = fq_t::from_table(FqTE::S377), cc = fq_t::from_table(FqTE::C377), dp = fq_t::from_table(FqTE::DP377);
+    te_bound_violations() = 0;
+    struct slot_t {
+        fql_t b0, b1, b2;
+    };
+    std::vector<g1_aff_t> pool;
+    std::vector<slot_t> slots;
+    g1_xyzz_t run = g1_xyzz_t::inf();
+    for (int k = 0; k < 64; k++) {
+        run.add_affine(g);
+        const fq_t izzz = run.zzz.inverse();
+        const fq_t izz = izzz.sqr() * run.zz.sqr();
+        const g1_aff_t p{run.x * izz, run.y * izzz};
+        pool.push_back(p);
+        const fq_t den = te_base_denominator(p.x, p.y);
+        if (den.is_zero()) return -1;
+        fq_t m, pp, kk;
+        te_base_from_affine(p.x, p.y, den.inverse(), m, pp, kk);
+        const fq_t half = (one + one).inverse();
+        const fq_t X = (pp - m) * half, Y = (pp + m) * half;
+        if (Y.sqr() - X.sqr() != one + dp * X.sqr() * Y.sqr()) return -2;
+        if (kk != (dp + dp) * X * Y) return -3;
+        const fq_t u = (one + Y) * (one - Y).inverse(), v = cc * u * X.inverse();
+        if (u * s.inverse() - one != p.x || v * s.inverse() != p.y) return -4;
+        slots.push_back({fql_t::from_limbs(m * c406), fql_t::from_limbs(pp * c406), fql_t::from_limbs(kk * c406)});
+    }
+    const slot_t inf_slot{fql_t::from_limbs(one * c406), fql_t::from_limbs(one * c406), fql_t::zero()};
+    auto next = [&]() {
+        seed += 0x9E3779B97F4A7C15ull;
+        uint64_t z = seed;
+        z = (z ^ (z >> 30)) * 0xBF58476D1CE4E5B9ull;
+        z = (z ^ (z >> 27)) * 0x94D049BB133111EBull;
+        return z ^ (z >> 31);
+    };
+    auto same_point = [](const te_lazy_t& t, const g1_xyzz_t& e) {
+        alignas(16) g1_lazy_partial_t raw;
+        t.store_raw(&raw);
+        te_lazy_t::raw_to_xyzz(&raw);
+        const g1_xyzz_t got = xyzz_lazy_t::exact_from_raw(&raw);
+        if (got.zz.is_zero() || e.is_inf()) return got.zz.is_zero() && e.is_inf();
+        return got.x * e.zz == e.x * got.zz && got.y * e.zzz == e.y * got.zzz;
+    };
+    g1_xyzz_t exact = g1_xyzz_t::inf();
+    te_lazy_t te = te_lazy_t::neutral();
+    if (!same_point(te, exact)) return -5;
+    int prev = -1;
+    bool prev_neg = false;
+    for (int it = 0; it < iters; it++) {
+        const uint64_t r = next();
+        int k = (int)(r % 64);
+        bool neg = ((r >> 8) & 1) != 0;
+        const int mode = (int)((r >> 16) % 16);
+        if (mode == 0 && prev >= 0) k = prev, neg = prev_neg;
+        if (mode == 1 && prev >= 0) k = prev, neg = !prev_neg;
+        if (mode == 2) {
+            exact = g1_xyzz_t::inf();
+            te = te_lazy_t::neutral();
+        }
+        if (mode == 3) {
+            if (!te.madd(inf_slot.b0, inf_slot.b1, inf_slot.b2, neg)) return it + 1;
+            if (!same_point(te, exact)) return it + 1;
+            continue;
+        }
+        prev = k;
+        prev_neg = neg;
+        exact.add_affine(pool[k], neg);
+        if (!te.madd(slots[k].b0, slots[k].b1, slots[k].b2, neg)) return it + 1;
+        if (!same_point(te, exact)) return it + 1;
+    }
+    for (int k = 0; k < 64; k++)
+        for (int second = 0; second < 2; second++) {
+            exact = g1_xyzz_t::inf();
+            te = te_lazy_t::neutral();
+            exact.add_affine(pool[k], false);
+            exact.add_affine(pool[k], second != 0);
+            if (!te.madd(slots[k].b0, slots[k].b1, slots[k].b2, false) || !te.madd(slots[k].b0, slots[k].b1, slots[k].b2, second != 0)) return -100 - k;
+            if (!same_point(te, exact)) return -100 - k;
+        }
+    {
+        te_lazy_t t2 = te_lazy_t::neutral();
+        t2.y = (fql_t::zero() - t2.y).normalized();
+        alignas(16) g1_lazy_partial_t raw;
+        t2.store_raw(&raw);
+        te_lazy_t::raw_to_xyzz(&raw);
+        const g1_xyzz_t got = xyzz_lazy_t::exact_from_raw(&raw);
+        if (got.zz.is_zero() || got.x != (fq_t::zero() - one) * got.zz || !got.y.is_zero()) return -6;
+    }
+    {
+        te_lazy_t e = te_lazy_t::neutral();
+        e.t = (e.z + e.z).normalized();
+        te_lazy_t e2 = e;
+        if (e.madd(inf_slot.b0, inf_slot.b1, inf_slot.b0, false)) return -7;
+        if (e2.madd(inf_slot.b0, inf_slot.b1, inf_slot.b0, true)) return -8;
+    }
+    if (te_bound_violations() != 0) return -9;
+    return 0;
+}
+RustError snarkvm_hip_g1_te_stats(uint64_t* out) {
+    API_TRY
+    if (!out) throw hip_failure{hipErrorInvalidValue, "g1_te_stats: null argument", __LINE__};
+    g_rt.configure();
+    uint64_t recomputed = 0;
+    int prev = 0;
+    (void)hipGetDevice(&prev);
+    for (auto& d : g_rt.devs) {
+        if (!d->ready) continue;
+        HIP_TRY(hipSetDevice(d->physical));
+        for (auto& l : d->lane) {
+            if (!l.te_state.p) continue;
+            uint32_t w = 0;
+            HIP_TRY(hipStreamSynchronize(l.stream));
+            HIP_TRY(hipMemcpy(&w, l.te_state.as<uint32_t>() + 1, 4, hipMemcpyDeviceToHost));
+            recomputed += w;
+        }
+    }
+    (void)hipSetDevice(prev);
+    out[0] = recomputed;
+    out[1] = te_registry().handles_te.load();
+    out[2] = te_registry().handles_unmappable.load();
+    API_CATCH
+}
 int snarkvm_hip_selftest_g1_finish(const void* planes_jacobian, const int32_t* pos, size_t n, void* out) {
     try {
         std::unique_ptr<msm_accum_t<fq_t>> acc(new msm_accum_t<fq_t>());
diff --git a/snarkvm_amd/csrc/api_serde.hip b/snarkvm_amd/csrc/api_serde.hip
--- a/snarkvm_amd/csrc/api_serde.hip
+++ b/snarkvm_amd/csrc/api_serde.hip
@@ -39,6 +39,7 @@
                 bases_to_lazy_form(c, h->d[dev], (size_t)tables * npoints);
                 HIP_TRY(hipStreamSynchronize(c.stream));
             });
+            g1_te_attach(h.get());
         } catch (...) {
             h->free_all();
             throw;
diff --git a/snarkvm_amd/csrc/ffl.hip.h b/snarkvm_amd/csrc/ffl.hip.h
--- a/snarkvm_amd/csrc/ffl.hip.h
+++ b/snarkvm_amd/csrc/ffl.hip.h
@@ -359,6 +359,191 @@
     }
 };
 
+struct FqTE {
+    static constexpr uint32_t S377[13] = {0x15b06342u, 0x147204a9u, 0x175a8e5fu, 0x1b70ccaeu, 0x191d2c43u, 0x14f44be2u, 0x0c8e35beu,
+                                          0x04244b5fu, 0x03c7e17fu, 0x19c83ffeu, 0x04c75929u, 0x1ebe20cdu, 0x13f11581u};
+    static constexpr uint32_t C377[13] = {0x11d5ac0cu, 0x188710abu, 0x113a9644u, 0x0de71d1cu, 0x09f8a717u, 0x03256d6du, 0x0a20f9a6u,
+                                          0x135c575bu, 0x0d358eb7u, 0x0ade3d8du, 0x08f489cfu, 0x194e6931u, 0x06095b1du};
+    static constexpr uint32_t DP377[13] = {0x0444a707u, 0x08b237f4u, 0x183eaa46u, 0x06e689d0u, 0x10ddfab2u, 0x18dde152u, 0x04a64c49u,
+                                           0x0d517fafu, 0x00a2417cu, 0x1bad5102u, 0x0edd5583u, 0x08bd4a6fu, 0x062f179eu};
+    static constexpr uint32_t K2D377[13] = {0x08894e0eu, 0x11646fe8u, 0x107d548cu, 0x0dcd13a1u, 0x01bbf564u, 0x11bbc2a5u, 0x094c9893u,
+                                            0x1aa2ff5eu, 0x014482f8u, 0x175aa204u, 0x1dbaab07u, 0x117a94deu, 0x0c5e2f3cu};
+    static constexpr int32_t S406[13] = {0x08449ac2, 0x16bc6341, 0x1f27346e, 0x003fa706, 0x16341794, 0x0e03035e, 0x1f0a2ed9,
+                                         0x0c4c0908, 0x1a0645ff, 0x0dd41749, 0x078fb647, 0x1b5db1c4, 0x1660c39d};
+    static constexpr int32_t C406[13] = {0x18d0ec00, 0x19d5ac0b, 0x099a00af, 0x14f3163d, 0x15201f1a, 0x185e2df4, 0x10000b58,
+                                         0x16cc24d5, 0x0cfaac7e, 0x1feb43c4, 0x0f6e64c6, 0x1143d6d9, 0x182ac132};
+};
+
+inline long& te_bound_violations() {
+    static long n = 0;
+    return n;
+}
+inline void te_check_product(const fql_t& a, const fql_t& b) {
+    for (int k = 0; k < 2 * fql_t::N - 1; k++) {
+        unsigned __int128 col = 0;
+        for (int i = 0; i < fql_t::N; i++) {
+            const int j = k - i;
+            if (j < 0 || j >= fql_t::N) continue;
+            const int64_t x = a.v[i], y = b.v[j];
+            col += (unsigned __int128)(uint64_t)(x < 0 ? -x : x) * (uint64_t)(y < 0 ? -y : y);
+        }
+        col += ((unsigned __int128)637 << 58) / 100 + ((unsigned __int128)1 << 34);
+        if (col >> 63) te_bound_violations()++;
+    }
+    const int64_t top = (int64_t)3 << 29;
+    if (a.v[12] > top || a.v[12] < -top || b.v[12] > top || b.v[12] < -top) te_bound_violations()++;
+}
+inline void te_check_limbs(const fql_t& a, int32_t lo, int32_t hi) {
+    for (int i = 0; i < fql_t::N - 1; i++)
+        if (a.v[i] < lo || a.v[i] > hi) te_bound_violations()++;
+}
+#if !defined(__HIP_DEVICE_COMPILE__)
+#define SV_TE_CHECK_PRODUCT(a, b) te_check_product(a, b)
+#define SV_TE_CHECK_LIMBS(a, lo, hi) te_check_limbs(a, lo, hi)
+#else
+#define SV_TE_CHECK_PRODUCT(a, b) ((void)0)
+#define SV_TE_CHECK_LIMBS(a, lo, hi) ((void)0)
+#endif
+
+struct alignas(32) g1_te_slot_t {
+    uint32_t w[40];
+    SV_HD void coords(fql_t& b0, fql_t& b1, fql_t& b2) const {
+#pragma unroll
+        for (int i = 0; i < 13; i++) b0.v[i] = (int32_t)w[i], b1.v[i] = (int32_t)w[13 + i], b2.v[i] = (int32_t)w[26 + i];
+        SV_OPAQUE_13(b0.v);
+        SV_OPAQUE_13(b1.v);
+        SV_OPAQUE_13(b2.v);
+    }
+    SV_HD static void store(g1_te_slot_t* slot, const fq_t& m, const fq_t& p, const fq_t& k) {
+        uint32_t t[40];
+#pragma unroll
+        for (int i = 0; i < 13; i++) t[i] = m.v[i], t[13 + i] = p.v[i], t[26 + i] = k.v[i];
+        t[39] = 0;
+        uint4* q = (uint4*)slot;
+#pragma unroll
+        for (int i = 0; i < 10; i++) q[i] = make_uint4(t[4 * i], t[4 * i + 1], t[4 * i + 2], t[4 * i + 3]);
+    }
+};
+static_assert(sizeof(g1_te_slot_t) == 160, "three 13-limb coordinates in ten 16-byte words");
+
+SV_HD fq_t te_base_denominator(const fq_t& x, const fq_t& y) {
+    const fq_t s = fq_t::from_table(FqTE::S377);
+    const fq_t u = s * (x + fq_t::one()), v = s * y;
+    return v * (u + fq_t::one());
+}
+SV_HD void te_base_from_affine(const fq_t& x, const fq_t& y, const fq_t& inv, fq_t& m, fq_t& p, fq_t& k) {
+    const fq_t s = fq_t::from_table(FqTE::S377), c = fq_t::from_table(FqTE::C377), k2d = fq_t::from_table(FqTE::K2D377);
+    const fq_t u = s * (x + fq_t::one()), v = s * y, u1 = u + fq_t::one();
+    const fq_t X = c * u * u1 * inv, Y = (u - fq_t::one()) * v * inv;
+    m = Y - X;
+    p = Y + X;
+    k = k2d * X * Y;
+}
+
+struct te_lazy_t {
+    fql_t x, y, z, t;
+
+    SV_HD static te_lazy_t neutral() {
+        te_lazy_t r;
+        r.x = r.t = fql_t::zero();
+        r.y = r.z = xyzz_lazy_t::one();
+        return r;
+    }
+    SV_HD static bool equals_multiple_of_q(const fql_t& v, int32_t k) {
+        fql_t m;
+#pragma unroll
+        for (int i = 0; i < fql_t::N; i++) m.v[i] = k * FqL::MOD[i];
+        m = m.normalized();
+        int32_t d = 0;
+#pragma unroll
+        for (int i = 0; i < fql_t::N; i++) d |= m.v[i] ^ v.v[i];
+        return d == 0;
+    }
+    SV_HD static bool is_zero_mod_q(const fql_t& v) {
+        const uint32_t f = ((uint32_t)v.v[0] + 3u) & fql_t::MASK;
+        if (f > 6u) return false;
+        return equals_multiple_of_q(v, (int32_t)f - 3);
+    }
+    SV_HD bool madd(const fql_t& b0, const fql_t& b1, const fql_t& b2, bool negate) {
+        fql_t m0, m1;
+#pragma unroll
+        for (int i = 0; i < fql_t::N; i++) m0.v[i] = negate ? b1.v[i] : b0.v[i], m1.v[i] = negate ? b0.v[i] : b1.v[i];
+        const fql_t k = b2.negate_if(negate);
+        const fql_t ymx = y - x, ypx = (y + x).normalized();
+        SV_TE_CHECK_LIMBS(ymx, -(int32_t)fql_t::MASK, (int32_t)fql_t::MASK);
+        SV_TE_CHECK_PRODUCT(ymx, m0);
+        SV_TE_CHECK_PRODUCT(ypx, m1);
+        SV_TE_CHECK_PRODUCT(t, k);
+        const fql_t a = fql_t::mul(ymx, m0);
+        const fql_t b = fql_t::mul(ypx, m1);
+        const fql_t c = fql_t::mul(t, k);
+        const fql_t d = z + z;
+        const fql_t e = b - a;
+        const fql_t f = (d - c).normalized(), g = (d + c).normalized(), h = (b + a).normalized();
+        SV_TE_CHECK_LIMBS(e, -(int32_t)fql_t::MASK, (int32_t)fql_t::MASK);
+        SV_TE_CHECK_LIMBS(f, 0, (int32_t)fql_t::MASK);
+        SV_TE_CHECK_LIMBS(g, 0, (int32_t)fql_t::MASK);
+        SV_TE_CHECK_LIMBS(h, 0, (int32_t)fql_t::MASK);
+        SV_TE_CHECK_PRODUCT(e, f);
+        SV_TE_CHECK_PRODUCT(g, h);
+        SV_TE_CHECK_PRODUCT(e, h);
+        SV_TE_CHECK_PRODUCT(f, g);
+        bool ok = true;
+        if ((((uint32_t)f.v[0] + 3u) & fql_t::MASK) <= 6u || (((uint32_t)g.v[0] + 3u) & fql_t::MASK) <= 6u)
+            ok = !(is_zero_mod_q(f) || is_zero_mod_q(g));
+        x = fql_t::mul(e, f);
+        y = fql_t::mul(g, h);
+        t = fql_t::mul(e, h);
+        z = fql_t::mul(f, g);
+        return ok;
+    }
+    SV_HD void store_raw(g1_lazy_partial_t* p) const {
+        uint4* q = (uint4*)p;
+        int32_t w[52];
+#pragma unroll
+        for (int i = 0; i < 13; i++) w[i] = x.v[i], w[13 + i] = y.v[i], w[26 + i] = z.v[i], w[39 + i] = t.v[i];
+#pragma unroll
+        for (int i = 0; i < 13; i++) q[i] = make_uint4((uint32_t)w[4 * i], (uint32_t)w[4 * i + 1], (uint32_t)w[4 * i + 2], (uint32_t)w[4 * i + 3]);
+    }
+    SV_HD static void raw_to_xyzz(g1_lazy_partial_t* p) {
+        uint4* q = (uint4*)p;
+        int32_t w[52];
+#pragma unroll
+        for (int i = 0; i < 13; i++) {
+            const uint4 u = q[i];
+            w[4 * i] = (int32_t)u.x, w[4 * i + 1] = (int32_t)u.y, w[4 * i + 2] = (int32_t)u.z, w[4 * i + 3] = (int32_t)u.w;
+        }
+        fql_t X, Y, Z, s, c;
+#pragma unroll
+        for (int i = 0; i < 13; i++) X.v[i] = w[i], Y.v[i] = w[13 + i], Z.v[i] = w[26 + i], s.v[i] = FqTE::S406[i], c.v[i] = FqTE::C406[i];
+        const fql_t zmy = Z - Y, zpy = (Z + Y).normalized();
+        fql_t xn, yn, zz, zzz;
+        if (is_zero_mod_q(X)) {
+            if (is_zero_mod_q(zmy.normalized())) {
+                xn = yn = zz = zzz = fql_t::zero();
+            } else {
+                xn = (fql_t::zero() - xyzz_lazy_t::one()).normalized();
+                yn = fql_t::zero();
+                zz = zzz = xyzz_lazy_t::one();
+            }
+        } else {
+            SV_TE_CHECK_PRODUCT(zmy, s);
+            const fql_t W = fql_t::mul(zmy, s);
+            const fql_t D = fql_t::mul(W, X);
+            zz = fql_t::mul(D, D);
+            zzz = fql_t::mul(zz, D);
+            SV_TE_CHECK_PRODUCT(zpy - W, X);
+            xn = fql_t::mul(fql_t::mul(zpy - W, X), D);
+            SV_TE_CHECK_PRODUCT(zpy, c);
+            yn = fql_t::mul(fql_t::mul(fql_t::mul(zpy, c), Z), zz);
+        }
+#pragma unroll
+        for (int i = 0; i < 13; i++) w[i] = xn.v[i], w[13 + i] = yn.v[i], w[26 + i] = zz.v[i], w[39 + i] = zzz.v[i];
+#pragma unroll
+        for (int i = 0; i < 13; i++) q[i] = make_uint4((uint32_t)w[4 * i], (uint32_t)w[4 * i + 1], (uint32_t)w[4 * i + 2], (uint32_t)w[4 * i + 3]);
+    }
+};
+
 struct fqz_t {
     fql_t a;
     struct mem_t {
diff --git a/snarkvm_amd/csrc/msm.hip.h b/snarkvm_amd/csrc/msm.hip.h
--- a/snarkvm_amd/csrc/msm.hip.h
+++ b/snarkvm_amd/csrc/msm.hip.h
@@ -248,6 +248,52 @@
     const fq_t c = fq_t::from_table(FqLConv::C406);
     const g1_aff_t a = g1_load_aff(&slots[i]);
     g1_lazy_slot_t::store(&slots[i], a.x * c, a.y * c, a.is_inf());
+}
+static constexpr int TE_BATCH = 8;
+static __global__ void __launch_bounds__(256) g1_bases_to_te_kernel(const g1_aff_mem_t* __restrict__ sw, g1_te_slot_t* __restrict__ te, size_t n,
+                                                             uint32_t* __restrict__ unmappable) {
+    const size_t first = ((size_t)blockIdx.x * blockDim.x + threadIdx.x) * TE_BATCH;
+    if (first >= n) return;
+    const fq_t c348 = fq_t::from_table(FqLConv::C348), c406 = fq_t::from_table(FqLConv::C406);
+    fq_t x[TE_BATCH], y[TE_BATCH], den[TE_BATCH], pre[TE_BATCH];
+    bool neutral[TE_BATCH];
+    bool bad = false;
+    fq_t run = fq_t::one();
+#pragma unroll 1
+    for (int j = 0; j < TE_BATCH; j++) {
+        neutral[j] = true;
+        den[j] = fq_t::one();
+        if (first + j < n) {
+            const g1_lazy_slot_t* s = (const g1_lazy_slot_t*)&sw[first + j];
+            if (!s->w[26]) {
+                fq_t bx, by;
+#pragma unroll
+                for (int i = 0; i < 13; i++) bx.v[i] = s->w[i], by.v[i] = s->w[13 + i];
+                x[j] = bx * c348;
+                y[j] = by * c348;
+                const fq_t d = te_base_denominator(x[j], y[j]);
+                if (d.is_zero()) {
+                    bad = true;
+                } else {
+                    den[j] = d;
+                    neutral[j] = false;
+                }
+            }
+        }
+        pre[j] = run;
+        run = run * den[j];
+    }
+    fq_t inv = run.inverse();
+#pragma unroll 1
+    for (int j = TE_BATCH - 1; j >= 0; j--) {
+        const fq_t inv_j = inv * pre[j];
+        inv = inv * den[j];
+        if (first + j >= n) continue;
+        fq_t m = fq_t::one(), p = fq_t::one(), k = fq_t::zero();
+        if (!neutral[j]) te_base_from_affine(x[j], y[j], inv_j, m, p, k);
+        g1_te_slot_t::store(&te[first + j], m * c406, p * c406, k * c406);
+    }
+    if (bad) atomicOr(unmappable, 1u);
 }
 template <class F>
 __global__ void convert_bases_kernel(const uint8_t* in, size_t stride, size_t n, aff_mem_t<F>* out, int form406) {
diff --git a/snarkvm_amd/csrc/msm_sort.hip.h b/snarkvm_amd/csrc/msm_sort.hip.h
--- a/snarkvm_amd/csrc/msm_sort.hip.h
+++ b/snarkvm_amd/csrc/msm_sort.hip.h
@@ -745,10 +745,15 @@
     ex.add_affine({bx * c348, by * c348}, neg);
     *acc = xyzz_lazy_t::from_exact(ex);
 }
-template <bool PREFETCH>
+template <bool PREFETCH, bool GUARDED = false>
 __global__ void __launch_bounds__(256, 1) msm_accumulate_lazy_kernel(const g1_aff_mem_t* __restrict__ bases, const uint32_t* __restrict__ sorted,
                                                               const uint32_t* __restrict__ boff, const uint32_t* __restrict__ start,
-                                                              g1_lazy_partial_t* __restrict__ partial, uint32_t nbt, uint32_t S, uint32_t debug_idx_mask) {
+                                                              g1_lazy_partial_t* __restrict__ partial, uint32_t nbt, uint32_t S, uint32_t debug_idx_mask,
+                                                              uint32_t* __restrict__ te_state = nullptr) {
+    if constexpr (GUARDED) {
+        if (te_state[2] == 0) return;
+        if (blockIdx.x == 0 && threadIdx.x == 0) atomicAdd(&te_state[1], 1u);
+    }
     const uint32_t t = blockIdx.x * blockDim.x + threadIdx.x;
     const uint32_t total = boff[nbt];
     const uint64_t lo64 = (uint64_t)t * S;
@@ -799,6 +804,66 @@
     }
 }
 
+template <bool PREFETCH>
+__global__ void __launch_bounds__(256, 1) msm_accumulate_te_kernel(const g1_te_slot_t* __restrict__ bases, const uint32_t* __restrict__ sorted,
+                                                            const uint32_t* __restrict__ boff, const uint32_t* __restrict__ start,
+                                                            g1_lazy_partial_t* __restrict__ partial, uint32_t nbt, uint32_t S, uint32_t debug_idx_mask,
+                                                            uint32_t* __restrict__ te_state) {
+    const uint32_t t = blockIdx.x * blockDim.x + threadIdx.x;
+    const uint32_t total = boff[nbt];
+    const uint64_t lo64 = (uint64_t)t * S;
+    if (lo64 >= total) return;
+    const uint32_t lo = (uint32_t)lo64;
+    const uint32_t hi = (total - lo < S) ? total : lo + S;
+    uint32_t k = find_bucket(boff, nbt, lo);
+    uint32_t kend = boff[k + 1];
+    uint32_t kend2 = boff[k + 2 <= nbt ? k + 2 : nbt];
+    uint32_t start_k = start[k];
+    uint32_t part_off = t - boff[k] / S;
+    te_lazy_t acc = te_lazy_t::neutral();
+    bool ok = true;
+    auto slot_of = [&](uint32_t e) -> const g1_te_slot_t* { return &bases[(e & 0x7fffffffu) & debug_idx_mask]; };
+    uint32_t e_cur = sorted[lo];
+    uint32_t e_n1 = lo + 1 < hi ? sorted[lo + 1] : 0u;
+    g1_te_slot_t raw_next = *slot_of(e_cur);
+    for (uint32_t pos = lo;; pos++) {
+        const bool end = pos >= hi;
+        if (end || pos >= kend) {
+            acc.store_raw(&partial[start_k + part_off]);
+            if (end) break;
+            part_off = 0;
+            acc = te_lazy_t::neutral();
+            k++;
+            kend = kend2;
+            while (pos >= kend) {
+                k++;
+                kend = boff[k + 1];
+            }
+            kend2 = boff[k + 2 <= nbt ? k + 2 : nbt];
+            start_k = start[k];
+        }
+        const uint32_t e = e_cur;
+        const g1_te_slot_t raw = raw_next;
+        if (pos + 1 < hi) raw_next = *slot_of(e_n1);
+        e_cur = e_n1;
+        if (pos + 2 < hi) e_n1 = sorted[pos + 2];
+        fql_t b0, b1, b2;
+        raw.coords(b0, b1, b2);
+        ok &= acc.madd(b0, b1, b2, (e >> 31) != 0);
+    }
+    if (!ok) atomicOr(&te_state[0], 1u);
+}
+static __global__ void __launch_bounds__(256) g1_te_partials_to_xyzz_kernel(g1_lazy_partial_t* __restrict__ raw, const uint32_t* __restrict__ start, uint32_t nbt,
+                                                                     uint32_t* __restrict__ te_state) {
+    const uint32_t i = blockIdx.x * blockDim.x + threadIdx.x;
+    if (i == 0) {
+        te_state[2] = te_state[0];
+        te_state[0] = 0;
+    }
+    if (i >= start[nbt]) return;
+    te_lazy_t::raw_to_xyzz(&raw[i]);
+}
+
 static __global__ void __launch_bounds__(256) g2_pair_partials_to_exact_kernel(const g2_pair_partial_t* __restrict__ raw, xyzz_mem_t<fq2_t>* __restrict__ partial,
                                                                         const uint32_t* __restrict__ start, uint32_t nbt) {
     const uint32_t g = blockIdx.x * blockDim.x + threadIdx.x;
diff --git a/snarkvm_amd/csrc/runtime.hip.h b/snarkvm_amd/csrc/runtime.hip.h
--- a/snarkvm_amd/csrc/runtime.hip.h
+++ b/snarkvm_amd/csrc/runtime.hip.h
@@ -133,6 +133,7 @@
     dev_buf rv2, rl2, rmid_size, rmid_boff;
     dev_buf fold_sums;
     dev_buf tail_flags;
+    dev_buf te_state;
     dev_buf sink_acc;
     dev_buf fchunk;
     dev_buf bases_tmp, scalars_tmp, gen_pts, gen_prod;
@@ -377,6 +378,8 @@
     HIP_TRY(hipFuncSetAttribute((const void*)scan_one_block_kernel, hipFuncAttributeMaxDynamicSharedMemorySize, (int)(SCAN_ONE_MAX * 4)));
 #ifdef SV_TU_G1
     HIP_TRY(hipFuncSetAttribute((const void*)msm_accumulate_lazy_kernel<true>, hipFuncAttributeMaxDynamicSharedMemorySize, 128 * 1024));
+    HIP_TRY(hipFuncSetAttribute((const void*)msm_accumulate_lazy_kernel<true, true>, hipFuncAttributeMaxDynamicSharedMemorySize, 128 * 1024));
+    HIP_TRY(hipFuncSetAttribute((const void*)msm_accumulate_te_kernel<true>, hipFuncAttributeMaxDynamicSharedMemorySize, 128 * 1024));
 #endif
 #ifdef SV_TU_NTT
     HIP_TRY(hipFuncSetAttribute((const void*)ntt_pass_kernel_v2<false, ntt_arith_u>, hipFuncAttributeMaxDynamicSharedMemorySize, 96 * 1024));
@@ -625,10 +628,44 @@
         if (e) std::rethrow_exception(e);
 }
 
+struct te_registry_t {
+    struct entry_t {
+        const uint8_t *lo, *hi;
+        const uint8_t* te;
+    };
+    std::mutex mu;
+    std::vector<entry_t> v;
+    std::atomic<uint64_t> handles_te{0}, handles_unmappable{0};
+    void add(const void* sw, size_t slots, const void* te) {
+        std::lock_guard<std::mutex> lk(mu);
+        v.push_back({(const uint8_t*)sw, (const uint8_t*)sw + slots * sizeof(g1_aff_mem_t), (const uint8_t*)te});
+    }
+    void remove(const void* sw) {
+        std::lock_guard<std::mutex> lk(mu);
+        for (size_t i = 0; i < v.size(); i++)
+            if (v[i].lo == (const uint8_t*)sw) {
+                v.erase(v.begin() + (long)i);
+                return;
+            }
+    }
+    const g1_te_slot_t* find(const void* vbase) {
+        std::lock_guard<std::mutex> lk(mu);
+        const uint8_t* p = (const uint8_t*)vbase;
+        for (const entry_t& e : v)
+            if (p >= e.lo && p < e.hi) return (const g1_te_slot_t*)(e.te + (size_t)(p - e.lo) / sizeof(g1_aff_mem_t) * sizeof(g1_te_slot_t));
+        return nullptr;
+    }
+};
+inline te_registry_t& te_registry() {
+    static te_registry_t r;
+    return r;
+}
+
 struct msm_ticket_t;
 template <class F>
 struct bases_handle_t {
     std::vector<aff_mem_t<F>*> d;
+    std::vector<void*> te;
     size_t n = 0;
     int tables = 1;
     int table_bits = 256;
@@ -642,6 +679,11 @@
         for (size_t i = 0; i < d.size(); i++)
             if (d[i]) {
                 (void)hipSetDevice(g_rt.devs[i]->physical);
+                if (i < te.size() && te[i]) {
+                    te_registry().remove(d[i]);
+                    (void)hipFree(te[i]);
+                    te[i] = nullptr;
+                }
                 (void)hipFree(d[i]);
                 d[i] = nullptr;
             }
@@ -880,8 +922,24 @@
         if (msm_lazy_on<F>()) {
             if (!ltail) c.part_raw.ensure(tmax * sizeof(g1_lazy_partial_t));
             g1_lazy_partial_t* raw_out = ltail ? c.part_a.as<g1_lazy_partial_t>() : c.part_raw.as<g1_lazy_partial_t>();
-            hipLaunchKernelGGL((msm_accumulate_lazy_kernel<true>), dim3((unsigned)((nthreads + 255) / 256)), dim3(256), one_wave || tuning().acc_one_wg ? msm_acc_lds() : 0, st,
-                               vbase, c.sorted.as<uint32_t>(), boffp, c.start_a.as<uint32_t>(), raw_out, nbt, pl.S, dbg_mask);
+            const dim3 grid((unsigned)((nthreads + 255) / 256));
+            const size_t lds = one_wave || tuning().acc_one_wg ? msm_acc_lds() : 0;
+            if (const g1_te_slot_t* te = te_registry().find(vbase)) {
+                if (!c.te_state.p) {
+                    c.te_state.ensure(16);
+                    HIP_TRY(hipMemsetAsync(c.te_state.p, 0, 16, st));
+                }
+                uint32_t* te_state = c.te_state.as<uint32_t>();
+                hipLaunchKernelGGL((msm_accumulate_te_kernel<true>), grid, dim3(256), lds, st, te, c.sorted.as<uint32_t>(), boffp, c.start_a.as<uint32_t>(), raw_out, nbt,
+                                   pl.S, dbg_mask, te_state);
+                hipLaunchKernelGGL(g1_te_partials_to_xyzz_kernel, dim3((unsigned)((tmax + 255) / 256)), dim3(256), 0, st, raw_out, (const uint32_t*)c.start_a.as<uint32_t>(),
+                                   nbt, te_state);
+                hipLaunchKernelGGL((msm_accumulate_lazy_kernel<true, true>), grid, dim3(256), lds, st, vbase, c.sorted.as<uint32_t>(), boffp, c.start_a.as<uint32_t>(), raw_out,
+                                   nbt, pl.S, dbg_mask, te_state);
+            } else {
+                hipLaunchKernelGGL((msm_accumulate_lazy_kernel<true>), grid, dim3(256), lds, st, vbase, c.sorted.as<uint32_t>(), boffp, c.start_a.as<uint32_t>(), raw_out, nbt,
+                                   pl.S, dbg_mask, (uint32_t*)nullptr);
+            }
             if (!ltail)
                 hipLaunchKernelGGL(g1_partials_to_exact_kernel, dim3((unsigned)((tmax + 255) / 256)), dim3(256), 0, st, (const g1_lazy_partial_t*)raw_out,
                                    c.part_a.as<g1_xyzz_mem_t>(), (const uint32_t*)c.start_a.as<uint32_t>(), nbt);
@@ -1231,6 +1289,44 @@
     hipLaunchKernelGGL(g1_bases_to_form406_kernel, dim3((unsigned)((slots + 255) / 256)), dim3(256), 0, c.stream, d, slots);
     HIP_TRY(hipGetLastError());
 }
+static void g1_te_attach(bases_handle_t<fq_t>* h) {
+    if (!tuning().g1_te || !tuning().lazy || h->tables < 2 || !h->n) return;
+    const size_t slots = (size_t)h->tables * h->n;
+    h->te.assign(h->d.size(), nullptr);
+    bool unmappable = false;
+    for (size_t dev = 0; dev < h->d.size() && !unmappable; dev++) {
+        if (!h->d[dev]) continue;
+        lane_guard lg((int)dev);
+        lane_t& c = lg.c();
+        HIP_TRY(hipMalloc(&h->te[dev], slots * sizeof(g1_te_slot_t)));
+        c.serde_status.ensure(4);
+        HIP_TRY(hipMemsetAsync(c.serde_status.p, 0, 4, c.stream));
+        const size_t threads = (slots + TE_BATCH - 1) / TE_BATCH;
+        hipLaunchKernelGGL(g1_bases_to_te_kernel, dim3((unsigned)((threads + 255) / 256)), dim3(256), 0, c.stream, (const g1_aff_mem_t*)h->d[dev],
+                           (g1_te_slot_t*)h->te[dev], slots, c.serde_status.as<uint32_t>());
+        HIP_TRY(hipGetLastError());
+        uint32_t bad = 0;
+        HIP_TRY(hipMemcpyAsync(&bad, c.serde_status.p, 4, hipMemcpyDeviceToHost, c.stream));
+        HIP_TRY(hipStreamSynchronize(c.stream));
+        unmappable = bad != 0;
+    }
+    if (unmappable) {
+        int prev = 0;
+        (void)hipGetDevice(&prev);
+        for (size_t dev = 0; dev < h->te.size(); dev++)
+            if (h->te[dev]) {
+                (void)hipSetDevice(g_rt.devs[dev]->physical);
+                (void)hipFree(h->te[dev]);
+            }
+        (void)hipSetDevice(prev);
+        h->te.clear();
+        te_registry().handles_unmappable++;
+        return;
+    }
+    for (size_t dev = 0; dev < h->d.size(); dev++)
+        if (h->d[dev]) te_registry().add(h->d[dev], slots, h->te[dev]);
+    te_registry().handles_te++;
+}
 #ifndef SV_NO_G2
 static void bases_to_lazy_form(lane_t& c, aff_mem_t<fq2_t>* d, size_t slots) {
     if (!slots || !msm_lazy_on<fq2_t>()) return;
diff --git a/snarkvm_amd/csrc/tuning.hip.h b/snarkvm_amd/csrc/tuning.hip.h
--- a/snarkvm_amd/csrc/tuning.hip.h
+++ b/snarkvm_amd/csrc/tuning.hip.h
@@ -6,7 +6,7 @@
 namespace sv {
 
 struct tuning_t {
-    int lazy = 1, lazy2 = 1, fused = 1;
+    int lazy = 1, lazy2 = 1, fused = 1, g1_te = 1;
     long acc_lds = 96 * 1024;
     int acc_one_wg = 0, reduce_rounds = 1, fuse_batch = 1, fuse_max_k = 64, fuse_reduce = -1, coalesce = 1, coalesce_us = 40, lanes = 0;
     int msm_chunk_lg = 20, scalar_chunk_lg = 22, taper = 1, ring_lanes = 3, seg = 0, seg2 = 0, fold_l = 0, scan1 = 1;
@@ -19,7 +19,7 @@
         name = (decltype(name))v;          \
         return true;                       \
     }
-        SV_TUNE_KEY(lazy) SV_TUNE_KEY(lazy2) SV_TUNE_KEY(fused) SV_TUNE_KEY(acc_lds)
+        SV_TUNE_KEY(lazy) SV_TUNE_KEY(g1_te) SV_TUNE_KEY(lazy2) SV_TUNE_KEY(fused) SV_TUNE_KEY(acc_lds)
         SV_TUNE_KEY(acc_one_wg) SV_TUNE_KEY(reduce_rounds) SV_TUNE_KEY(fuse_batch) SV_TUNE_KEY(fuse_max_k) SV_TUNE_KEY(fuse_reduce) SV_TUNE_KEY(coalesce)
         SV_TUNE_KEY(coalesce_us) SV_TUNE_KEY(lanes) SV_TUNE_KEY(msm_chunk_lg) SV_TUNE_KEY(scalar_chunk_lg) SV_TUNE_KEY(taper) SV_TUNE_KEY(ring_lanes) SV_TUNE_KEY(seg) SV_TUNE_KEY(seg2)
         SV_TUNE_KEY(fold_l) SV_TUNE_KEY(scan1) SV_TUNE_KEY(ntt_min_tiles) SV_TUNE_KEY(ntt_full_tw) SV_TUNE_KEY(ntt_fold)
```
